# OFA-Sys/ONE-PEACE

Hardware: AMD Instinct MI355X
Metric: pretrain samples/s (tri-modal global batch) ONE-PEACE-4B (higher is better)
Workload: dtype bf16

## Files before the change

### include/onepeace_hip.h

```cpp
#ifndef ONEPEACE_HIP_H
#define ONEPEACE_HIP_H

#include <stdint.h>

#ifdef __cplusplus
extern "C" {
#endif

int op_abi_version(void);
const char* op_last_error(void);

int op_prof_enable(int on);
int op_prof_reserve(int events);
int op_prof_collect(double* ms, int64_t* count, double* work, int n_families);

int op_layernorm_fwd(const void* x, const void* w, const void* b, void* y, float* mean, float* rstd, int64_t rows,
                     int64_t cols, float eps, int act_gelu, int dtype, const int* x_rows, void* stream);
int64_t op_layernorm_bwd_workspace_bytes(int64_t rows, int64_t cols);
int op_layernorm_bwd(const void* dy, const void* x, const void* w, const void* b, const float* mean, const float* rstd,
                     const void* add, void* dx, void* dw, void* db, void* workspace, int64_t rows, int64_t cols,
                     int act_gelu, int accumulate, int dtype, const int* x_rows, void* stream);

int op_gemm_nt(const void* A, int64_t lda, const void* B0, const void* B1, const void* B2, int64_t ldb, int64_t n_seg,
               const void* bias0, const void* bias1, const void* bias2, void* C, int64_t ldc, void* h0, void* h1,
               const void* resid, int64_t ldr, const void* gamma, const float* rowscale, int64_t rows_per_sample,
               const float* alpha, int64_t M, int64_t N, int64_t K, int epilogue, void* workspace, int64_t workspace_bytes,
               int64_t tune, const int* resid_rows, int64_t resid_rows_total, void* stream);
int op_gemm_tn(const void* A, int64_t lda, const void* B, int64_t ldb, void* C, int64_t ldc, int64_t M, int64_t N, int64_t K,
               int accumulate, void* workspace, int64_t workspace_bytes, int64_t tune, void* stream);
int op_gemm_nt_grouped(int64_t nprob, const void* const* A, const int64_t* M, int64_t lda, const void* const* B, int64_t ldb,
                       const void* const* bias, void* const* C, int64_t ldc, void* const* h0, void* const* h1,
                       const void* const* resid, int64_t ldr, const void* const* gamma, const float* const* rowscale,
                       const int64_t* rows_per_sample, int64_t N, int64_t K, int epilogue, int64_t tune, const int* const* resid_rows,
                       int64_t resid_rows_total, void* stream);
int op_gemm_nt_batched(const void* A, int64_t lda, int64_t stride_a, const void* W, int64_t ldb, int64_t stride_b, const void* bias,
                       int64_t stride_bias, void* C, int64_t ldc, int64_t stride_c, int64_t M, int64_t N, int64_t K, int64_t batch,
                       void* stream);
int op_audio_conv1_ln_gelu_fwd(const void* wav, int64_t stride, const void* w0, const void* b0, const void* lnw, const void* lnb, void* y,
                               float* mean, float* rstd, int64_t rows, int64_t C, float eps, void* stream);
int64_t op_audio_conv1_ln_gelu_bwd_workspace_bytes(int64_t C);
int op_audio_conv1_ln_gelu_bwd(const void* dy, const void* wav, int64_t stride, const void* w0, const void* b0, const void* lnw, const void* lnb,
                               const float* mean, const float* rstd, void* dw0, void* db0, void* dlnw, void* dlnb, void* workspace,
                               int64_t rows, int64_t C, int accumulate, void* stream);
int64_t op_gemm_tn_grouped_counter_bytes(void);
int64_t op_gemm_tn_grouped_plan(int64_t nprob, const int64_t* M, const int64_t* N, const int64_t* K, int64_t workgroups, int64_t tune,
                                int32_t* out, int64_t cap);
int op_gemm_tn_grouped(int64_t nprob, const void* const* A, const int64_t* lda, const void* const* B, const int64_t* ldb, void* const* C,
                       const int64_t* ldc, const int64_t* M, const int64_t* N, const int64_t* K, const int32_t* accumulate,
                       const void* const* W, const int64_t* ldw, float* const* rowdot, const void* const* rscale, void* counters,
                       int64_t tune, void* stream);
int op_gemm_plan(int64_t M, int64_t N, int64_t K, int epilogue, int has_bias, int64_t workspace_bytes, int64_t tune, int* plan);

int op_quant_fp8_rows(const void* x, int64_t ldx, void* q, int64_t ldq, float* scale, int64_t rows, int64_t cols, void* stream);
int op_layernorm_fwd_q8(const void* x, const void* w, const void* b, void* y, float* mean, float* rstd, void* q8, float* q8_scale,
                        int64_t rows, int64_t cols, float eps, void* stream);
int op_ln_geglu_fwd_q8(const void* h0, const void* h1, int64_t ldh, const void* w, const void* b, void* y, float* mean, float* rstd, void* q8,
                       float* q8_scale, int64_t rows, int64_t cols, float eps, void* stream);
int op_gemm_nt_fp8(const void* A8, int64_t lda, const float* sa, const void* B0, const void* B1, int64_t ldb, const float* sb0,
                   const float* sb1, const void* bias, void* C, int64_t ldc, void* h0, void* h1, const void* resid, int64_t ldr,
                   const void* gamma, const float* rowscale, int64_t rows_per_sample, int64_t M, int64_t N, int64_t K, int epilogue,
                   int64_t tune, void* stream);

int op_attn_fwd(const void* q, const void* k, const void* v, int64_t ld, const void* bias, int64_t bias_batch_stride,
                const void* bias_frag, const void* key_pad, void* out, int64_t ldo, float* lse, int64_t lse_ld, int64_t B,
                int64_t S, int64_t Spad, int64_t heads, int64_t head_dim, float scale, int64_t tune, void* stream);
int64_t op_attn_bias_frag_elems(int64_t n_img, int64_t S);
int op_attn_bias_pack(const void* src, void* dst, int64_t n_img, int64_t S, int64_t Spad, void* stream);
int op_attn_bwd_delta(const void* dout, const void* out, int64_t ldo, float* delta, int64_t B, int64_t S, int64_t Spad,
                      int64_t heads, void* stream);
int64_t op_attn_bwd_dbias_slabs(int64_t B, int64_t S, int64_t heads, int64_t tune);
int op_attn_bwd(const void* q, const void* k, const void* v, int64_t ld, const void* dout, const void* out, int64_t ldo,
                const void* bias, const void* biasT, const void* bias_frag, int64_t bias_batch_stride, const void* key_pad,
                const float* lse, float* delta, void* dq,
                void* dk, void* dv, int64_t ldg, float* dbias, int64_t B, int64_t S, int64_t Spad, int64_t heads,
                int64_t head_dim, float scale, int64_t tune, void* stream);

int op_relpos_bias_build(const void* table, const int* bucket, int64_t bucket_ld, void* out, int64_t heads, int64_t S,
                         int64_t Spad, int transposed, void* stream);
int op_relpos_bias_bwd(const float* dbias, int64_t S, int64_t Spad, const int* pos, const int* seg, int64_t nseg, const int* bucket_seg,
                       int64_t num_rel, float* partial_ws, float* dtable, int64_t heads, void* stream);
int op_relpos_bias_build_ids(const void* table, const int* bucket, int64_t bucket_ld, const int* ids, void* out, int64_t B,
                             int64_t heads, int64_t K, int64_t Kpad, int transposed, void* stream);
int op_relpos_bias_fold_ids(const float* dbias, const int* ids, float* dense_ws, int64_t Sfull, int64_t B, int64_t heads, int64_t K,
                            int64_t Kpad, void* stream);

int op_transpose(const void* in, void* out, int64_t rows, int64_t cols, int64_t ld_in, int64_t ld_out, void* stream);
int op_transpose_scaled(const void* in, void* out, int64_t rows, int64_t cols, int64_t ld_in, int64_t ld_out, const void* scale,
                        void* stream);
int op_transpose_batched(const void* table, int64_t n, int64_t total_tiles, void* stream);
int64_t op_transpose_desc_bytes(void);
int64_t op_colsum_workspace_bytes(int64_t N);
int op_colsum_segments(const void* x, void* out0, void* out1, void* out2, void* workspace, int64_t M, int64_t n_seg,
                       int64_t seg_cols, int accumulate, void* stream);
int64_t op_resid_bwd_workspace_bytes(int64_t N);
int op_resid_bwd(const void* dout, const void* y, const void* gamma, const float* rowscale, int64_t rows_per_sample,
                 void* dbranch, void* dgamma, void* dbias, float* g0, void* workspace, int64_t M, int64_t N, int accumulate,
                 const int* dout_rows, void* stream);
int op_gamma_grad_finish(const float* rowdot, int64_t slots, const void* b0, const float* g00, const void* b1, const float* g01,
                         const void* b2, const float* g02, void* dgamma, int64_t N, int accumulate, void* stream);
int op_ln_geglu_bwd(const void* dy, const void* h0, const void* h1, const void* w, const float* mean, const float* rstd,
                    void* dh0, void* dh1, int64_t ldd, int64_t ldh, void* dw, void* db, void* workspace, int64_t rows,
                    int64_t cols, int accumulate, void* stream);
int op_ln_geglu_fwd(const void* h0, const void* h1, int64_t ldh, const void* w, const void* b, void* y, float* mean, float* rstd,
                    int64_t rows, int64_t cols, float eps, void* stream);
int op_colsum(const void* x, const void* y, const float* rowscale, int64_t rows_per_sample, const void* mul, void* out,
              void* workspace, int64_t M, int64_t N, int accumulate, int out_dtype, void* stream);
int op_geglu_bwd(const void* dg, const void* h0, const void* h1, void* dh0, void* dh1, int64_t numel, void* stream);
int op_scale_rows(const void* dout, const void* gamma, const float* rowscale, int64_t rows_per_sample, void* dbranch,
                  int64_t M, int64_t N, void* stream);

int op_l2norm_fwd(const void* x, void* y, float* inv_norm, int64_t rows, int64_t cols, float eps, int out_dtype, void* stream);
int op_l2norm_bwd(const void* dy, const void* y, const float* inv_norm, void* dx, int64_t rows, int64_t cols, int y_dtype,
                  void* stream);
int op_infonce_rows(float* sim, int64_t rows, int64_t n, int64_t ld, int64_t target0, float label_smoothing, float gscale,
                    float* row_loss, float* row_hit, float* row_dot, int write_grad, void* stream);

int op_adamw_step(void* p, const void* g, float* m, float* v, int64_t numel, float lr, float beta1, float beta2, float eps,
                  float weight_decay, int64_t step, float grad_scale, const float* grad_sqnorm, float clip_norm,
                  void* stream);
int op_adamw_step_groups(void* p, const void* g, float* m, float* v, int64_t numel, const int64_t* group_end8,
                         const float* group_lr_scale, const float* group_weight_decay, int64_t n_groups, float lr, float beta1,
                         float beta2, float eps, int64_t step, float grad_scale, const float* grad_sqnorm, float clip_norm,
                         void* stream);
int op_sqnorm(const void* x, int64_t numel, float* workspace, float* out, void* stream);

int op_rows_gather(const void* src, void* dst, const int* list, int64_t nseg, const int64_t* src_row0, const int64_t* dst_row0,
                   const int64_t* S, const int64_t* n_kept, const int64_t* dst_rows, const int64_t* n_samples, const int64_t* list_off,
                   int64_t dst_total, int64_t cols, void* stream);
int op_rows_merge(const void* base, const void* upd, void* out, const int* list, int64_t nseg, const int64_t* src_row0,
                  const int64_t* dst_row0, const int64_t* S, const int64_t* n_kept, const int64_t* dst_rows, const int64_t* n_samples,
                  const int64_t* list_off, int64_t total, int64_t cols, void* stream);
int op_rows_map(int* map, const int* list, int64_t nseg, const int64_t* src_row0, const int64_t* dst_row0, const int64_t* S,
                const int64_t* n_kept, const int64_t* dst_rows, const int64_t* n_samples, const int64_t* list_off, int64_t dst_total,
                void* stream);

int64_t op_sim_topk_splits(int64_t M, int64_t N, int64_t splits);
int64_t op_sim_topk_workspace_bytes(int64_t M, int64_t N, int64_t k, int64_t splits);
int op_sim_topk(const void* Q, int64_t ldq, const void* G, int64_t ldg, int64_t M, int64_t N, int64_t D, int64_t k, float* vals, int* idx,
                void* workspace, int64_t workspace_bytes, int64_t splits, void* stream);

int op_image_resize_normalize(const void* src, int64_t src_bytes, const int64_t* desc, const int64_t* desc_host, int64_t B,
                              const int* coef, int64_t coef_count, int64_t S, const float* mean, const float* stdev, void* out,
                              int out_dtype, void* workspace, int64_t workspace_bytes, void* stream);

int op_audio_normalize_pad(const void* src, int64_t src_bytes, const int64_t* desc, const int64_t* desc_host, int64_t B, int64_t max_len,
                           int64_t min_len, void* out, int64_t T, int out_dtype, void* workspace, int64_t workspace_bytes, void* stream);

#ifdef __cplusplus
}
#endif
#endif
```

### one-peace_amd/csrc/elementwise.hip

```cpp
#include "common.h"
#include <string.h>

namespace {

constexpr int CS_MAX_PARTS = 256;

__device__ __forceinline__ void transpose_tile(int bx, int by, const bf16_t* __restrict__ in, bf16_t* __restrict__ out,
                                                        int rows, int cols, int64_t ld_in, int64_t ld_out,
                                                        const bf16_t* __restrict__ scale = nullptr) {
  __shared__ bf16_t tile[64][64 + 2];
  const int r0 = by * 64, c0 = bx * 64;
  const int tx = threadIdx.x & 15, ty = threadIdx.x >> 4;
#pragma unroll
  for (int k = 0; k < 4; ++k) {
    const int r = r0 + ty + k * 16, c = c0 + tx * 4;
    if (r < rows) {
      const float sc = scale ? (float)scale[r] : 1.f;
      if (c + 3 < cols && (ld_in & 3) == 0) {
        bf16x4 v = *reinterpret_cast<const bf16x4*>(in + (int64_t)r * ld_in + c);
#pragma unroll
        for (int j = 0; j < 4; ++j) tile[ty + k * 16][tx * 4 + j] = scale ? (bf16_t)(sc * (float)v[j]) : v[j];
      } else {
        for (int j = 0; j < 4; ++j)
          if (c + j < cols) tile[ty + k * 16][tx * 4 + j] = scale ? (bf16_t)(sc * (float)in[(int64_t)r * ld_in + c + j]) : in[(int64_t)r * ld_in + c + j];
      }
    }
  }
  __syncthreads();
#pragma unroll
  for (int k = 0; k < 4; ++k) {
    const int c = c0 + ty + k * 16, r = r0 + tx * 4;
    if (c < cols) {
      if (r + 3 < rows && (ld_out & 3) == 0) {
        bf16x4 v;
#pragma unroll
        for (int j = 0; j < 4; ++j) v[j] = tile[tx * 4 + j][ty + k * 16];
        *reinterpret_cast<bf16x4*>(out + (int64_t)c * ld_out + r) = v;
      } else {
        for (int j = 0; j < 4; ++j)
          if (r + j < rows) out[(int64_t)c * ld_out + r + j] = tile[tx * 4 + j][ty + k * 16];
      }
    }
  }
}


__global__ __launch_bounds__(256) void transpose_kernel(const bf16_t* __restrict__ in, bf16_t* __restrict__ out, int rows, int cols,
                                                        int64_t ld_in, int64_t ld_out, const bf16_t* __restrict__ scale) {
  transpose_tile(blockIdx.x, blockIdx.y, in, out, rows, cols, ld_in, ld_out, scale);
}

struct TransposeDesc { const bf16_t* in; bf16_t* out; int rows, cols; int64_t ld_in, ld_out; int tile0, tiles_x; const bf16_t* scale; };
__global__ __launch_bounds__(256) void transpose_batched_kernel(const TransposeDesc* __restrict__ table, int n) {
  const int b = blockIdx.x;
  int lo = 0, hi = n - 1;
  while (lo < hi) {
    const int mid = (lo + hi + 1) >> 1;
    if (table[mid].tile0 <= b) lo = mid; else hi = mid - 1;
  }
  const TransposeDesc d = table[lo];
  const int local = b - d.tile0;
  transpose_tile(local % d.tiles_x, local / d.tiles_x, d.in, d.out, d.rows, d.cols, d.ld_in, d.ld_out, d.scale);
}

__global__ __launch_bounds__(256) void colsum_partial_kernel(const bf16_t* __restrict__ x, const bf16_t* __restrict__ y,
                                                             const float* __restrict__ rowscale, int rps,
                                                             float* __restrict__ part, int64_t M, int N, int64_t ld) {
  __shared__ float red[4][512];
  const int lane = threadIdx.x & 63, wid = threadIdx.x >> 6;
  const int c = blockIdx.x * 512 + lane * 8;
  float a[8] = {0, 0, 0, 0, 0, 0, 0, 0};
  if (c < N) {
    const int64_t m0 = (int64_t)blockIdx.y * 4 + wid, step = (int64_t)gridDim.y * 4;
    if (!y && !rowscale) {
      int64_t m = m0;
      for (; m + 3 * step < M; m += 4 * step) {
        typename Vec8<bf16_t>::raw_t r0 = Vec8<bf16_t>::ldraw(x + m * ld + c), r1 = Vec8<bf16_t>::ldraw(x + (m + step) * ld + c),
                                     r2 = Vec8<bf16_t>::ldraw(x + (m + 2 * step) * ld + c), r3 = Vec8<bf16_t>::ldraw(x + (m + 3 * step) * ld + c);
        float v0[8], v1[8], v2[8], v3[8];
        Vec8<bf16_t>::cvt(r0, v0);
        Vec8<bf16_t>::cvt(r1, v1);
        Vec8<bf16_t>::cvt(r2, v2);
        Vec8<bf16_t>::cvt(r3, v3);
#pragma unroll
        for (int j = 0; j < 8; ++j) a[j] = (((a[j] + v0[j]) + v1[j]) + v2[j]) + v3[j];
      }
      for (; m < M; m += step) {
        float xv[8];
        Vec8<bf16_t>::load(x + m * ld + c, xv);
#pragma unroll
        for (int j = 0; j < 8; ++j) a[j] += xv[j];
      }
    } else {
      for (int64_t m = m0; m < M; m += step) {
        float xv[8];
        Vec8<bf16_t>::load(x + m * ld + c, xv);
        float s = rowscale ? rowscale[m / rps] : 1.f;
        if (y) {
          float yv[8];
          Vec8<bf16_t>::load(y + m * ld + c, yv);
#pragma unroll
          for (int j = 0; j < 8; ++j) a[j] += s * xv[j] * yv[j];
        } else {
#pragma unroll
          for (int j = 0; j < 8; ++j) a[j] += s * xv[j];
        }
      }
    }
  }
#pragma unroll
  for (int j = 0; j < 8; ++j) red[wid][lane * 8 + j] = a[j];
  __syncthreads();
  for (int i = threadIdx.x; i < 512; i += 256) {
    const int cc = blockIdx.x * 512 + i;
    if (cc < N) part[(int64_t)blockIdx.y * N + cc] = red[0][i] + red[1][i] + red[2][i] + red[3][i];
  }
}

__global__ __launch_bounds__(256) void gamma_grad_finish_kernel(const float* __restrict__ rowdot, int slots,
                                                                const bf16_t* __restrict__ b0, const float* __restrict__ g00,
                                                                const bf16_t* __restrict__ b1, const float* __restrict__ g01,
                                                                const bf16_t* __restrict__ b2, const float* __restrict__ g02,
                                                                bf16_t* __restrict__ dgamma, int N, int accumulate) {
  __shared__ float part[4][64];
  const int lane = threadIdx.x & 63, w = threadIdx.x >> 6;
  const int n = blockIdx.x * 64 + lane;
  float a0 = 0.f, a1 = 0.f, a2 = 0.f, a3 = 0.f;
  if (n < N) {
    int s = w;
    for (; s + 12 < slots; s += 16) {
      a0 += rowdot[(int64_t)s * N + n];
      a1 += rowdot[(int64_t)(s + 4) * N + n];
      a2 += rowdot[(int64_t)(s + 8) * N + n];
      a3 += rowdot[(int64_t)(s + 12) * N + n];
    }
    for (; s < slots; s += 4) a0 += rowdot[(int64_t)s * N + n];
  }
  part[w][lane] = (a0 + a1) + (a2 + a3);
  __syncthreads();
  if (w != 0 || n >= N) return;
  float t = (part[0][lane] + part[1][lane]) + (part[2][lane] + part[3][lane]);
  if (g00) t += (b0 ? (float)b0[n] : 0.f) * g00[n];
  if (g01) t += (b1 ? (float)b1[n] : 0.f) * g01[n];
  if (g02) t += (b2 ? (float)b2[n] : 0.f) * g02[n];
  dgamma[n] = (bf16_t)(t + (accumulate ? (float)dgamma[n] : 0.f));
}

__global__ __launch_bounds__(256) void resid_bwd_kernel(const bf16_t* __restrict__ dout, const bf16_t* __restrict__ y,
                                                        const bf16_t* __restrict__ gamma, const float* __restrict__ rowscale,
                                                        int rps, bf16_t* __restrict__ dbranch, float* __restrict__ part,
                                                        int64_t M, int N, const int* __restrict__ rows) {
  __shared__ float red[4][512];
  const int lane = threadIdx.x & 63, wid = threadIdx.x >> 6;
  const int c = blockIdx.x * 512 + lane * 8;
  float ag[8] = {0, 0, 0, 0, 0, 0, 0, 0}, ab[8] = {0, 0, 0, 0, 0, 0, 0, 0};
  float gv[8] = {1, 1, 1, 1, 1, 1, 1, 1};
  if (c < N) {
    if (gamma) Vec8<bf16_t>::load(gamma + c, gv);
    const int64_t step = (int64_t)gridDim.y * 4;
    const int64_t mfirst = (int64_t)blockIdx.y * 4 + wid;
    int64_t e0 = (rows && mfirst < M) ? rows[mfirst] : mfirst, e1 = (rows && mfirst + step < M) ? rows[mfirst + step] : mfirst + step;
    for (int64_t m = mfirst; m < M; m += 2 * step) {
      const int64_t m2 = m + step;
      const bool two = m2 < M;
      const int64_t s0 = e0, s1 = two ? e1 : -1;
      const int64_t mn = m + 2 * step;
      if (rows) {
        if (mn < M) e0 = rows[mn];
        if (mn + step < M) e1 = rows[mn + step];
      } else {
        e0 = mn;
        e1 = mn + step;
      }
      const bf16x8 zero8 = {(bf16_t)0.f, (bf16_t)0.f, (bf16_t)0.f, (bf16_t)0.f, (bf16_t)0.f, (bf16_t)0.f, (bf16_t)0.f, (bf16_t)0.f};
      bf16x8 d0 = s0 >= 0 ? Vec8<bf16_t>::ldraw(dout + s0 * N + c) : zero8, d1, y0, y1;
      if (y) y0 = Vec8<bf16_t>::ldraw(y + m * N + c);
      if (two) {
        d1 = s1 >= 0 ? Vec8<bf16_t>::ldraw(dout + s1 * N + c) : zero8;
        if (y) y1 = Vec8<bf16_t>::ldraw(y + m2 * N + c);
      }
#pragma unroll
      for (int h = 0; h < 2; ++h) {
        if (h == 1 && !two) break;
        const int64_t mm = h == 0 ? m : m2;
        float d[8], o[8];
        Vec8<bf16_t>::cvt(h == 0 ? d0 : d1, d);
        const float sc = rowscale ? rowscale[mm / rps] : 1.f;
        if (y) {
          float yv[8];
          Vec8<bf16_t>::cvt(h == 0 ? y0 : y1, yv);
#pragma unroll
          for (int j = 0; j < 8; ++j) ag[j] += sc * d[j] * yv[j];
        }
#pragma unroll
        for (int j = 0; j < 8; ++j) {
          const float t = sc * d[j];
          ab[j] += t;
          o[j] = t * gv[j];
        }
        Vec8<bf16_t>::store(dbranch + mm * N + c, o);
      }
    }
  }
  if (part == nullptr) return;
#pragma unroll
  for (int pass = 0; pass < 2; ++pass) {
    if (pass == 0 && y == nullptr) continue;
    __syncthreads();
#pragma unroll
    for (int j = 0; j < 8; ++j) red[wid][lane * 8 + j] = pass == 0 ? ag[j] : ab[j];
    __syncthreads();
    float* dst = part + ((int64_t)pass * gridDim.y + blockIdx.y) * N;
    for (int i = threadIdx.x; i < 512; i += 256) {
      const int cc = blockIdx.x * 512 + i;
      if (cc < N) dst[cc] = red[0][i] + red[1][i] + red[2][i] + red[3][i];
    }
  }
}

__global__ __launch_bounds__(256) void geglu_bwd_kernel(const bf16_t* __restrict__ dg, const bf16_t* __restrict__ h0,
                                                        const bf16_t* __restrict__ h1, bf16_t* __restrict__ dh0,
                                                        bf16_t* __restrict__ dh1, int64_t n8) {
  for (int64_t i = (int64_t)blockIdx.x * 256 + threadIdx.x; i < n8; i += (int64_t)gridDim.x * 256) {
    float g[8], a[8], b[8], o0[8], o1[8];
    Vec8<bf16_t>::load(dg + i * 8, g);
    Vec8<bf16_t>::load(h0 + i * 8, a);
    Vec8<bf16_t>::load(h1 + i * 8, b);
#pragma unroll
    for (int j = 0; j < 8; ++j) {
      float cdf, pdf;
      gelu_parts(a[j], cdf, pdf);
      o0[j] = g[j] * b[j] * (cdf + a[j] * pdf);
      o1[j] = g[j] * a[j] * cdf;
    }
    Vec8<bf16_t>::store(dh0 + i * 8, o0);
    Vec8<bf16_t>::store(dh1 + i * 8, o1);
  }
}

__global__ __launch_bounds__(256) void scale_rows_kernel(const bf16_t* __restrict__ dout, const bf16_t* __restrict__ gamma,
                                                         const float* __restrict__ rowscale, int rps,
                                                         bf16_t* __restrict__ dbranch, int64_t M, int N) {
  const int n8 = N / 8;
  const int64_t total = M * n8;
  for (int64_t i = (int64_t)blockIdx.x * 256 + threadIdx.x; i < total; i += (int64_t)gridDim.x * 256) {
    const int64_t m = i / n8;
    const int c = (int)(i - m * n8) * 8;
    float d[8], gv[8];
    Vec8<bf16_t>::load(dout + m * N + c, d);
    const float s = rowscale ? rowscale[m / rps] : 1.f;
    if (gamma) {
      Vec8<bf16_t>::load(gamma + c, gv);
#pragma unroll
      for (int j = 0; j < 8; ++j) d[j] *= s * gv[j];
    } else {
#pragma unroll
      for (int j = 0; j < 8; ++j) d[j] *= s;
    }
    Vec8<bf16_t>::store(dbranch + m * N + c, d);
  }
}

template <typename TO>
__global__ __launch_bounds__(256) void l2norm_fwd_kernel(const bf16_t* __restrict__ x, TO* __restrict__ y,
                                                         float* __restrict__ inv_norm, int rows, int cols, float eps) {
  const int lane = threadIdx.x & 63;
  const int row = blockIdx.x * 4 + (threadIdx.x >> 6);
  if (row >= rows) return;
  float ss = 0.f;
  for (int c = lane * 8; c < cols; c += 512) {
    float v[8];
    Vec8<bf16_t>::load(x + (int64_t)row * cols + c, v);
#pragma unroll
    for (int j = 0; j < 8; ++j) ss += v[j] * v[j];
  }
  ss = wave_sum(ss);
  const float nrm = sqrtf(ss);
  const float inv = 1.f / fmaxf(nrm, eps);
  for (int c = lane * 8; c < cols; c += 512) {
    float v[8];
    Vec8<bf16_t>::load(x + (int64_t)row * cols + c, v);
#pragma unroll
    for (int j = 0; j < 8; ++j) v[j] *= inv;
    Vec8<TO>::store(y + (int64_t)row * cols + c, v);
  }
  if (lane == 0 && inv_norm) inv_norm[row] = nrm < eps ? -inv : inv;
}

template <typename TY>
__global__ __launch_bounds__(256) void l2norm_bwd_kernel(const TY* __restrict__ dy, const TY* __restrict__ y,
                                                         const float* __restrict__ inv_norm, bf16_t* __restrict__ dx,
                                                         int rows, int cols) {
  const int lane = threadIdx.x & 63;
  const int row = blockIdx.x * 4 + (threadIdx.x >> 6);
  if (row >= rows) return;
  float dot = 0.f;
  for (int c = lane * 8; c < cols; c += 512) {
    float a[8], b[8];
// ... 284 lines not shown
#pragma unroll
    for (int i = 0; i < 4; ++i) {
      if (i < d.nseg && rc >= d.seg[i].dst_row0 && rc < d.seg[i].dst_row0 + d.seg[i].dst_rows) {
        const int local = (int)(rc - d.seg[i].dst_row0);
        const int j = local / d.seg[i].S;
        if (j < d.seg[i].n_kept) from = d.seg[i].src_row0 + (int64_t)list[d.seg[i].list_off + j] * d.seg[i].S + (local - j * d.seg[i].S);
      }
    }
    bf16x8* o = reinterpret_cast<bf16x8*>(dst + rc * cols);
    if (from >= 0) {
      const bf16x8* in = reinterpret_cast<const bf16x8*>(src + from * cols);
      for (int c = lane; c < n8; c += 64) o[c] = in[c];
    } else {
      bf16x8 z;
#pragma unroll
      for (int k = 0; k < 8; ++k) z[k] = (bf16_t)0.f;
      for (int c = lane; c < n8; c += 64) o[c] = z;
    }
  }
}

__global__ __launch_bounds__(256) void rows_merge_kernel(const bf16_t* __restrict__ base, const bf16_t* __restrict__ upd,
                                                         bf16_t* __restrict__ out, const int* __restrict__ list, const RowsSegs d,
                                                         int64_t total, int cols) {
  const int lane = threadIdx.x & 63;
  const int n8 = cols / 8;
  for (int64_t r = (int64_t)blockIdx.x * 4 + (threadIdx.x >> 6); r < total; r += (int64_t)gridDim.x * 4) {
    int64_t from = -1;
#pragma unroll
    for (int i = 0; i < 4; ++i) {
      if (i < d.nseg && r >= d.seg[i].src_row0 && r < d.seg[i].src_row0 + (int64_t)d.seg[i].n_samples * d.seg[i].S) {
        const int local = (int)(r - d.seg[i].src_row0);
        const int smp = local / d.seg[i].S;
        const int j = list[d.seg[i].list_off + smp];
        if (j >= 0) from = d.seg[i].dst_row0 + (int64_t)j * d.seg[i].S + (local - smp * d.seg[i].S);
      }
    }
    if (from < 0 && out == base) continue;
    if (from >= 0 && upd == nullptr) continue;
    const bf16x8* in = reinterpret_cast<const bf16x8*>(from >= 0 ? upd + from * cols : base + r * cols);
    bf16x8* o = reinterpret_cast<bf16x8*>(out + r * cols);
    for (int c = lane; c < n8; c += 64) o[c] = in[c];
  }
}

__global__ __launch_bounds__(256) void rows_map_kernel(int* __restrict__ map, const int* __restrict__ list, const RowsSegs d, int64_t dst_total) {
  const int64_t rc = (int64_t)blockIdx.x * 256 + threadIdx.x;
  if (rc >= dst_total) return;
  int64_t from = -1;
#pragma unroll
  for (int i = 0; i < 4; ++i) {
    if (i < d.nseg && rc >= d.seg[i].dst_row0 && rc < d.seg[i].dst_row0 + d.seg[i].dst_rows) {
      const int local = (int)(rc - d.seg[i].dst_row0);
      const int j = local / d.seg[i].S;
      if (j < d.seg[i].n_kept) from = d.seg[i].src_row0 + (int64_t)list[d.seg[i].list_off + j] * d.seg[i].S + (local - j * d.seg[i].S);
    }
  }
  map[rc] = (int)from;
}

}

extern "C" {

int op_transpose_scaled(const void* in, void* out, int64_t rows, int64_t cols, int64_t ld_in, int64_t ld_out, const void* scale,
                        void* stream) {
  OP_CHECK_ARG(in && out && rows >= 0 && cols >= 0, "transpose: bad args");
  if (rows == 0 || cols == 0) return OP_OK;
  dim3 grid(ceil_div(cols, 64), ceil_div(rows, 64));
  hipLaunchKernelGGL(transpose_kernel, grid, dim3(256), 0, (hipStream_t)stream, (const bf16_t*)in, (bf16_t*)out, (int)rows,
                     (int)cols, ld_in, ld_out, (const bf16_t*)scale);
  OP_LAUNCH_CHECK();
  return OP_OK;
}
int op_transpose(const void* in, void* out, int64_t rows, int64_t cols, int64_t ld_in, int64_t ld_out, void* stream) {
  return op_transpose_scaled(in, out, rows, cols, ld_in, ld_out, nullptr, stream);
}

int op_transpose_batched(const void* table, int64_t n, int64_t total_tiles, void* stream) {
  OP_CHECK_ARG(table && n > 0 && total_tiles > 0, "transpose_batched: bad args");
  hipLaunchKernelGGL(transpose_batched_kernel, dim3((unsigned)total_tiles), dim3(256), 0, (hipStream_t)stream,
                     (const TransposeDesc*)table, (int)n);
  OP_LAUNCH_CHECK();
  return OP_OK;
}
int64_t op_transpose_desc_bytes(void) { return (int64_t)sizeof(TransposeDesc); }

int64_t op_colsum_workspace_bytes(int64_t N) { return (int64_t)CS_MAX_PARTS * N * (int64_t)sizeof(float); }

int op_colsum(const void* x, const void* y, const float* rowscale, int64_t rows_per_sample, const void* mul, void* out,
              void* workspace, int64_t M, int64_t N, int accumulate, int out_dtype, void* stream) {
  OP_CHECK_ARG(x && out && workspace, "colsum: null pointer");
  OP_CHECK_ARG(N > 0 && N % 8 == 0, "colsum: N must be a multiple of 8");
  hipStream_t s = (hipStream_t)stream;
  int parts = (int)((M + 63) / 64);
  if (parts > CS_MAX_PARTS) parts = CS_MAX_PARTS;
  if (parts < 1) parts = 1;
  dim3 grid(ceil_div(N, 512), parts);
  hipLaunchKernelGGL(colsum_partial_kernel, grid, dim3(256), 0, s, (const bf16_t*)x, (const bf16_t*)y, rowscale,
                     (int)(rows_per_sample > 0 ? rows_per_sample : 1), (float*)workspace, M, (int)N, N);
  OP_LAUNCH_CHECK();
  if (out_dtype == OP_DT_BF16)
    hipLaunchKernelGGL((partials_reduce_kernel<bf16_t>), dim3(ceil_div(N, 32)), dim3(256), 0, s, (const float*)workspace, parts,
                       N, (int)N, (const bf16_t*)mul, (bf16_t*)out, accumulate);
  else
    hipLaunchKernelGGL((partials_reduce_kernel<float>), dim3(ceil_div(N, 32)), dim3(256), 0, s, (const float*)workspace, parts,
                       N, (int)N, (const bf16_t*)mul, (float*)out, accumulate);
  OP_LAUNCH_CHECK();
  return OP_OK;
}

int64_t op_resid_bwd_workspace_bytes(int64_t N) { return 2 * (int64_t)CS_MAX_PARTS * N * (int64_t)sizeof(float); }

int op_resid_bwd(const void* dout, const void* y, const void* gamma, const float* rowscale, int64_t rows_per_sample,
                 void* dbranch, void* dgamma, void* dbias, float* g0, void* workspace, int64_t M, int64_t N, int accumulate,
                 const int* dout_rows, void* stream) {
  OP_CHECK_ARG(dout && dbranch, "resid_bwd: null pointer");
  OP_CHECK_ARG(N > 0 && N % 8 == 0, "resid_bwd: N must be a multiple of 8");
  OP_CHECK_ARG(!dgamma || y, "resid_bwd: dgamma needs y");
  OP_CHECK_ARG(!(dgamma && g0), "resid_bwd: g0 (dbranch without gamma) and dgamma (from y) are alternatives");
  OP_CHECK_ARG(!(dgamma || dbias || g0) || workspace, "resid_bwd: dgamma/dbias/g0 requested without workspace");
  if (M == 0) {
    if (g0) (void)hipMemsetAsync(g0, 0, (size_t)N * sizeof(float), (hipStream_t)stream);
    return OP_OK;
  }
  hipStream_t s = (hipStream_t)stream;
  int parts = (int)((M + 63) / 64);
  if (parts > CS_MAX_PARTS) parts = CS_MAX_PARTS;
  if (parts < 1) parts = 1;
  float* ws = (dgamma || dbias || g0) ? (float*)workspace : nullptr;
  hipLaunchKernelGGL(resid_bwd_kernel, dim3(ceil_div(N, 512), parts), dim3(256), 0, s, (const bf16_t*)dout,
                     (const bf16_t*)(dgamma ? y : nullptr), (const bf16_t*)(g0 ? nullptr : gamma), rowscale,
                     (int)(rows_per_sample > 0 ? rows_per_sample : 1), (bf16_t*)dbranch, ws, M, (int)N, dout_rows);
  OP_LAUNCH_CHECK();
  if (ws) {
    hipLaunchKernelGGL((partials_reduce3_kernel<bf16_t>), dim3(ceil_div(N, 32), g0 ? 3 : 2), dim3(256), 0, s, ws,
                       ws + (int64_t)parts * N, ws + (int64_t)parts * N, (const bf16_t*)nullptr, (const bf16_t*)gamma,
                       (const bf16_t*)nullptr, (bf16_t*)dgamma, (bf16_t*)dbias, (bf16_t*)nullptr, parts, N, (int)N,
                       accumulate, g0);
    OP_LAUNCH_CHECK();
  }
  return OP_OK;
}

int op_gamma_grad_finish(const float* rowdot, int64_t slots, const void* b0, const float* g00, const void* b1, const float* g01,
                         const void* b2, const float* g02, void* dgamma, int64_t N, int accumulate, void* stream) {
  OP_CHECK_ARG(rowdot && dgamma && N > 0 && slots > 0, "gamma_grad_finish: null pointer");
  hipLaunchKernelGGL(gamma_grad_finish_kernel, dim3(ceil_div(N, 64)), dim3(256), 0, (hipStream_t)stream, rowdot, (int)slots,
                     (const bf16_t*)b0, g00, (const bf16_t*)b1, g01, (const bf16_t*)b2, g02, (bf16_t*)dgamma, (int)N, accumulate);
  OP_LAUNCH_CHECK();
  return OP_OK;
}

int op_colsum_segments(const void* x, void* out0, void* out1, void* out2, void* workspace, int64_t M, int64_t n_seg,
                       int64_t seg_cols, int accumulate, void* stream) {
  OP_CHECK_ARG(x && workspace, "colsum_segments: null pointer");
  OP_CHECK_ARG(n_seg >= 1 && n_seg <= 3 && seg_cols > 0 && seg_cols % 8 == 0, "colsum_segments: bad segments");
  hipStream_t s = (hipStream_t)stream;
  const int64_t N = n_seg * seg_cols;
  int parts = (int)((M + 63) / 64);
  if (parts > CS_MAX_PARTS) parts = CS_MAX_PARTS;
  if (parts < 1) parts = 1;
  void* outs[3] = {out0, out1, out2};
  const float* ws = (const float*)workspace;
  for (int i = 0; i < (int)n_seg; ++i) {
    if (outs[i] == nullptr) continue;
    hipLaunchKernelGGL(colsum_partial_kernel, dim3(ceil_div(seg_cols, 512), parts), dim3(256), 0, s,
                       (const bf16_t*)x + i * seg_cols, (const bf16_t*)nullptr, (const float*)nullptr, 1,
                       (float*)workspace + (int64_t)i * parts * seg_cols, M, (int)seg_cols, N);
    OP_LAUNCH_CHECK();
  }
  const int64_t st = (int64_t)parts * seg_cols;
  hipLaunchKernelGGL((partials_reduce3_kernel<bf16_t>), dim3(ceil_div(seg_cols, 32), (int)n_seg), dim3(256), 0, s, ws, ws + st,
                     ws + 2 * st, (const bf16_t*)nullptr, (const bf16_t*)nullptr, (const bf16_t*)nullptr, (bf16_t*)out0,
                     (bf16_t*)out1, (bf16_t*)out2, parts, seg_cols, (int)seg_cols, accumulate);
  OP_LAUNCH_CHECK();
  return OP_OK;
}

int op_geglu_bwd(const void* dg, const void* h0, const void* h1, void* dh0, void* dh1, int64_t numel, void* stream) {
  OP_CHECK_ARG(dg && h0 && h1 && dh0 && dh1, "geglu_bwd: null pointer");
  OP_CHECK_ARG(numel % 8 == 0, "geglu_bwd: numel must be a multiple of 8");
  if (numel == 0) return OP_OK;
  hipLaunchKernelGGL(geglu_bwd_kernel, dim3(ew_grid(numel / 8)), dim3(256), 0, (hipStream_t)stream, (const bf16_t*)dg,
                     (const bf16_t*)h0, (const bf16_t*)h1, (bf16_t*)dh0, (bf16_t*)dh1, numel / 8);
  OP_LAUNCH_CHECK();
  return OP_OK;
}

int op_scale_rows(const void* dout, const void* gamma, const float* rowscale, int64_t rows_per_sample, void* dbranch,
                  int64_t M, int64_t N, void* stream) {
  OP_CHECK_ARG(dout && dbranch, "scale_rows: null pointer");
  OP_CHECK_ARG(N % 8 == 0, "scale_rows: N must be a multiple of 8");
  if (M == 0) return OP_OK;
  hipLaunchKernelGGL(scale_rows_kernel, dim3(ew_grid(M * (N / 8))), dim3(256), 0, (hipStream_t)stream, (const bf16_t*)dout,
                     (const bf16_t*)gamma, rowscale, (int)(rows_per_sample > 0 ? rows_per_sample : 1), (bf16_t*)dbranch, M,
                     (int)N);
  OP_LAUNCH_CHECK();
  return OP_OK;
}

int op_l2norm_fwd(const void* x, void* y, float* inv_norm, int64_t rows, int64_t cols, float eps, int out_dtype, void* stream) {
  OP_CHECK_ARG(x && y && cols % 8 == 0, "l2norm_fwd: bad args");
  if (rows == 0) return OP_OK;
  if (out_dtype == OP_DT_BF16)
    hipLaunchKernelGGL((l2norm_fwd_kernel<bf16_t>), dim3(ceil_div(rows, 4)), dim3(256), 0, (hipStream_t)stream,
                       (const bf16_t*)x, (bf16_t*)y, inv_norm, (int)rows, (int)cols, eps);
  else
    hipLaunchKernelGGL((l2norm_fwd_kernel<float>), dim3(ceil_div(rows, 4)), dim3(256), 0, (hipStream_t)stream,
                       (const bf16_t*)x, (float*)y, inv_norm, (int)rows, (int)cols, eps);
  OP_LAUNCH_CHECK();
  return OP_OK;
}

int op_l2norm_bwd(const void* dy, const void* y, const float* inv_norm, void* dx, int64_t rows, int64_t cols, int y_dtype,
                  void* stream) {
  OP_CHECK_ARG(dy && y && inv_norm && dx && cols % 8 == 0, "l2norm_bwd: bad args");
  if (rows == 0) return OP_OK;
  if (y_dtype == OP_DT_BF16)
    hipLaunchKernelGGL((l2norm_bwd_kernel<bf16_t>), dim3(ceil_div(rows, 4)), dim3(256), 0, (hipStream_t)stream,
                       (const bf16_t*)dy, (const bf16_t*)y, inv_norm, (bf16_t*)dx, (int)rows, (int)cols);
  else
    hipLaunchKernelGGL((l2norm_bwd_kernel<float>), dim3(ceil_div(rows, 4)), dim3(256), 0, (hipStream_t)stream,
                       (const float*)dy, (const float*)y, inv_norm, (bf16_t*)dx, (int)rows, (int)cols);
  OP_LAUNCH_CHECK();
  return OP_OK;
}

int op_infonce_rows(float* sim, int64_t rows, int64_t n, int64_t ld, int64_t target0, float label_smoothing, float gscale,
                    float* row_loss, float* row_hit, float* row_dot, int write_grad, void* stream) {
  OP_CHECK_ARG(sim && row_loss && row_hit && row_dot, "infonce_rows: null pointer");
  OP_CHECK_ARG(n >= 2 && target0 >= 0 && target0 + rows <= n, "infonce_rows: targets out of range");
  if (rows == 0) return OP_OK;
  hipLaunchKernelGGL(infonce_rows_kernel, dim3((int)rows), dim3(256), 0, (hipStream_t)stream, sim, (int)n, ld, (int)target0,
                     label_smoothing, gscale, row_loss, row_hit, row_dot, write_grad);
  OP_LAUNCH_CHECK();
  return OP_OK;
}

int op_sqnorm(const void* x, int64_t numel, float* workspace, float* out, void* stream) {
  OP_CHECK_ARG(x && workspace && out && numel % 8 == 0, "sqnorm: bad args");
  hipStream_t s = (hipStream_t)stream;
  hipLaunchKernelGGL(sqnorm_partial_kernel, dim3(1024), dim3(256), 0, s, (const bf16_t*)x, numel / 8, workspace);
  OP_LAUNCH_CHECK();
  hipLaunchKernelGGL(sqnorm_final_kernel, dim3(1), dim3(256), 0, s, (const float*)workspace, 1024, out);
  OP_LAUNCH_CHECK();
  return OP_OK;
}

int op_adamw_step(void* p, const void* g, float* m, float* v, int64_t numel, float lr, float beta1, float beta2, float eps,
                  float weight_decay, int64_t step, float grad_scale, const float* grad_sqnorm, float clip_norm,
                  void* stream) {
  OP_CHECK_ARG(p && g && m && v, "adamw: null pointer");
  OP_CHECK_ARG(numel % 8 == 0 && step >= 1, "adamw: numel must be a multiple of 8 and step >= 1");
  if (numel == 0) return OP_OK;
  const double bc1 = 1.0 - pow((double)beta1, (double)step);
  const double bc2 = 1.0 - pow((double)beta2, (double)step);
  const float step_size = (float)((double)lr * sqrt(bc2) / bc1);
  const float decay_mul = 1.f - weight_decay * lr;
  hipLaunchKernelGGL(adamw_kernel, dim3(ew_grid(numel / 8)), dim3(256), 0, (hipStream_t)stream, (bf16_t*)p, (const bf16_t*)g,
                     m, v, numel / 8, beta1, beta2, eps, step_size, decay_mul, grad_scale, grad_sqnorm, clip_norm);
  OP_LAUNCH_CHECK();
  return OP_OK;
}

int op_adamw_step_groups(void* p, const void* g, float* m, float* v, int64_t numel, const int64_t* group_end8,
                         const float* group_lr_scale, const float* group_weight_decay, int64_t n_groups, float lr, float beta1,
                         float beta2, float eps, int64_t step, float grad_scale, const float* grad_sqnorm, float clip_norm,
                         void* stream) {
  OP_CHECK_ARG(p && g && m && v && group_end8 && group_lr_scale && group_weight_decay, "adamw_groups: null pointer");
  OP_CHECK_ARG(numel % 8 == 0 && step >= 1 && n_groups >= 1 && n_groups <= ADAM_MAX_GROUPS,
               "adamw_groups: numel %% 8 == 0, step >= 1, 1 <= n_groups <= %d required", ADAM_MAX_GROUPS);
  if (numel == 0) return OP_OK;
  const double bc1 = 1.0 - pow((double)beta1, (double)step);
  const double bc2 = 1.0 - pow((double)beta2, (double)step);
  hipLaunchKernelGGL(adamw_groups_kernel, dim3(ew_grid(numel / 8)), dim3(256), 0, (hipStream_t)stream, (bf16_t*)p,
                     (const bf16_t*)g, m, v, numel / 8, group_end8, group_lr_scale, group_weight_decay, (int)n_groups, lr, beta1,
                     beta2, eps, (float)(sqrt(bc2) / bc1), grad_scale, grad_sqnorm, clip_norm);
  OP_LAUNCH_CHECK();
  return OP_OK;
}

int op_relpos_bias_build(const void* table, const int* bucket, int64_t bucket_ld, void* out, int64_t heads, int64_t S,
                         int64_t Spad, int transposed, void* stream) {
  OP_CHECK_ARG(table && bucket && out && Spad >= S && Spad % 8 == 0, "relpos_bias_build: bad args");
  hipLaunchKernelGGL(relpos_build_kernel, dim3(ew_grid(S * Spad)), dim3(256), 0, (hipStream_t)stream, (const bf16_t*)table,
                     bucket, bucket_ld, (bf16_t*)out, (int)heads, (int)S, (int)Spad, transposed);
  OP_LAUNCH_CHECK();
  return OP_OK;
}

int op_relpos_bias_build_ids(const void* table, const int* bucket, int64_t bucket_ld, const int* ids, void* out, int64_t B,
                             int64_t heads, int64_t K, int64_t Kpad, int transposed, void* stream) {
  OP_CHECK_ARG(table && bucket && ids && out && B > 0 && K > 0 && Kpad >= K && Kpad % 8 == 0, "relpos_bias_build_ids: bad args");
  hipLaunchKernelGGL(relpos_build_ids_kernel, dim3(ew_grid(B * K * Kpad)), dim3(256), 0, (hipStream_t)stream, (const bf16_t*)table,
                     bucket, bucket_ld, ids, (bf16_t*)out, (int)B, (int)heads, (int)K, (int)Kpad, transposed);
  OP_LAUNCH_CHECK();
  return OP_OK;
}

int op_relpos_bias_fold_ids(const float* dbias, const int* ids, float* dense_ws, int64_t Sfull, int64_t B, int64_t heads, int64_t K,
                            int64_t Kpad, void* stream) {
  OP_CHECK_ARG(dbias && ids && dense_ws && B > 0 && K > 0 && Sfull > 0, "relpos_bias_fold_ids: bad args");
  hipLaunchKernelGGL(relpos_fold_ids_kernel, dim3(ew_grid(B * heads * K * K)), dim3(256), 0, (hipStream_t)stream, dbias, ids, dense_ws,
                     (int)B, (int)heads, (int)K, (int)Kpad, (int)Sfull);
  OP_LAUNCH_CHECK();
// ... 75 lines not shown
```

### one-peace_amd/csrc/layernorm.hip

```cpp
#include "common.h"

namespace {

constexpr int LN_MAX_BLOCKS = 4096;
constexpr int g_ln_blocks_fwd = 512, g_ln_blocks_bwd = 512;
#ifndef OP_LN_GEGLU_BLOCKS_FWD
#define OP_LN_GEGLU_BLOCKS_FWD 2048
#endif
#ifndef OP_LN_GEGLU_BLOCKS_BWD
#define OP_LN_GEGLU_BLOCKS_BWD 512
#endif

template <int NW>
__device__ __forceinline__ float group_sum(float v, float* red) {
  v = wave_sum(v);
  if (NW == 1) return v;
  const int wid = threadIdx.x >> 6;
  __syncthreads();
  if ((threadIdx.x & 63) == 0) red[wid] = v;
  __syncthreads();
  float t = 0.f;
#pragma unroll
  for (int i = 0; i < NW; ++i) t += red[i];
  return t;
// ... 97 lines not shown
    }
    const float rstd = rsqrtf(group_sum<NW>(ss, red) * inv + eps);
    T* yr = y + row * (int64_t)cols;
    int amax = 0;
#pragma unroll
    for (int i = 0; i < CH; ++i) {
      const int c = (tig + G * i) * 8;
      if (c < cols) {
        float o[8];
#pragma unroll
        for (int j = 0; j < 8; ++j) {
          float t = (v[i][j] - mean) * rstd * wv[i][j] + bv[i][j];
          o[j] = GELU ? gelu_erf(t) : t;
        }
        store_sel<T, NT>(yr + c, o);
        if constexpr (Q8) {
#pragma unroll
          for (int j = 0; j < 8; ++j) { v[i][j] = (float)(T)o[j]; amax = fp8_amax_acc(amax, v[i][j]); }
        }
      }
    }
    if constexpr (Q8) {
      float qinv;
      const float sc = fp8_row_scale(group_amax<NW>(amax, red), qinv);
      uint8_t* qr = q8 + row * (int64_t)cols;
#pragma unroll
      for (int i = 0; i < CH; ++i) {
        const int c = (tig + G * i) * 8;
        if (c < cols) *reinterpret_cast<u32x2*>(qr + c) = fp8_pack8(v[i], qinv);
      }
      if (tig == 0) q8_scale[row] = sc;
    }
    if (tig == 0) {
      if (mean_out) mean_out[row] = mean;
      if (rstd_out) rstd_out[row] = rstd;
    }
#pragma unroll
    for (int i = 0; i < CH; ++i) cur[i] = nxt[i];
  }
}

template <int CH, int NW, bool Q8 = false>
__global__ __launch_bounds__(NW == 1 ? 256 : 64 * NW) void ln_geglu_fwd_kernel(const bf16_t* __restrict__ h0, const bf16_t* __restrict__ h1,
                                                           int64_t ldh, const bf16_t* __restrict__ w, const bf16_t* __restrict__ b,
                                                           bf16_t* __restrict__ y, float* __restrict__ mean_out,
                                                           float* __restrict__ rstd_out, int64_t rows, int cols, float eps,
                                                           uint8_t* __restrict__ q8 = nullptr, float* __restrict__ q8_scale = nullptr) {
  __shared__ float red[4];
  constexpr int G = 64 * NW;
  const int tig = (NW == 1) ? (threadIdx.x & 63) : threadIdx.x;
  const int64_t row0 = (NW == 1) ? ((int64_t)blockIdx.x * 4 + (threadIdx.x >> 6)) : blockIdx.x;
  const int64_t rstep = (NW == 1) ? (int64_t)gridDim.x * 4 : gridDim.x;
  const float inv = 1.0f / (float)cols;
  float wv[CH][8], bv[CH][8];
#pragma unroll
  for (int i = 0; i < CH; ++i) {
    const int c = (tig + G * i) * 8;
#pragma unroll
    for (int j = 0; j < 8; ++j) { wv[i][j] = 1.f; bv[i][j] = 0.f; }
    if (c < cols) {
      if (w) Vec8<bf16_t>::load(w + c, wv[i]);
      if (b) Vec8<bf16_t>::load(b + c, bv[i]);
    }
  }
  bf16x8 c0[CH], c1[CH], n0[CH], n1[CH];
  if (row0 < rows) {
#pragma unroll
    for (int i = 0; i < CH; ++i) {
      const int c = (tig + G * i) * 8;
      if (c < cols) {
        c0[i] = Vec8<bf16_t>::ldraw_nt(h0 + row0 * ldh + c);
        c1[i] = Vec8<bf16_t>::ldraw_nt(h1 + row0 * ldh + c);
      }
    }
  }
  for (int64_t row = row0; row < rows; row += rstep) {
    const int64_t nrow = row + rstep;
    if (nrow < rows) {
#pragma unroll
      for (int i = 0; i < CH; ++i) {
        const int c = (tig + G * i) * 8;
        if (c < cols) {
          n0[i] = Vec8<bf16_t>::ldraw_nt(h0 + nrow * ldh + c);
          n1[i] = Vec8<bf16_t>::ldraw_nt(h1 + nrow * ldh + c);
        }
      }
    }
    float v[CH][8];
    float s = 0.f;
#pragma unroll
    for (int i = 0; i < CH; ++i) {
      const int c = (tig + G * i) * 8;
      if (c < cols) {
        float a[8], bb[8];
        Vec8<bf16_t>::cvt(c0[i], a);
        Vec8<bf16_t>::cvt(c1[i], bb);
#pragma unroll
        for (int j = 0; j < 8; ++j) {
          v[i][j] = (float)(bf16_t)(gelu_erf(a[j]) * bb[j]);
          s += v[i][j];
        }
      } else {
#pragma unroll
        for (int j = 0; j < 8; ++j) v[i][j] = 0.f;
      }
    }
    const float mean = group_sum<NW>(s, red) * inv;
    float ss = 0.f;
#pragma unroll
    for (int i = 0; i < CH; ++i) {
      const int c = (tig + G * i) * 8;
      if (c < cols) {
#pragma unroll
        for (int j = 0; j < 8; ++j) { const float d = v[i][j] - mean; ss += d * d; }
      }
    }
    const float rstd = rsqrtf(group_sum<NW>(ss, red) * inv + eps);
    bf16_t* yr = y + row * (int64_t)cols;
    int amax = 0;
#pragma unroll
    for (int i = 0; i < CH; ++i) {
      const int c = (tig + G * i) * 8;
      if (c < cols) {
        float o[8];
#pragma unroll
        for (int j = 0; j < 8; ++j) o[j] = (v[i][j] - mean) * rstd * wv[i][j] + bv[i][j];
        Vec8<bf16_t>::store_nt(yr + c, o);
        if constexpr (Q8) {
#pragma unroll
          for (int j = 0; j < 8; ++j) { v[i][j] = (float)(bf16_t)o[j]; amax = fp8_amax_acc(amax, v[i][j]); }
        }
      }
    }
    if constexpr (Q8) {
      float qinv;
      const float sc = fp8_row_scale(group_amax<NW>(amax, red), qinv);
      uint8_t* qr = q8 + row * (int64_t)cols;
#pragma unroll
      for (int i = 0; i < CH; ++i) {
        const int c = (tig + G * i) * 8;
        if (c < cols) *reinterpret_cast<u32x2*>(qr + c) = fp8_pack8(v[i], qinv);
      }
      if (tig == 0) q8_scale[row] = sc;
    }
    if (tig == 0) {
      if (mean_out) mean_out[row] = mean;
      if (rstd_out) rstd_out[row] = rstd;
    }
#pragma unroll
    for (int i = 0; i < CH; ++i) { c0[i] = n0[i]; c1[i] = n1[i]; }
  }
}

template <typename T, int CH, int NW, bool GELU, bool NT>
__global__ __launch_bounds__(256) void ln_bwd_kernel(const T* __restrict__ dy, const T* __restrict__ x,
                                                     const T* __restrict__ w, const T* __restrict__ b,
                                                     const float* __restrict__ mean_in,
                                                     const float* __restrict__ rstd_in, const T* __restrict__ add,
                                                     T* __restrict__ dx, float* __restrict__ ws, int64_t rows, int cols,
                                                     const int* __restrict__ xmap = nullptr) {
  extern __shared__ __attribute__((aligned(16))) float smem[];
  float* red = smem;
  constexpr int G = 64 * NW;
  const int tig = (NW == 1) ? (threadIdx.x & 63) : threadIdx.x;
  const int wid = threadIdx.x >> 6;
  const int64_t row0 = (NW == 1) ? ((int64_t)blockIdx.x * 4 + wid) : blockIdx.x;
  const int64_t rstep = (NW == 1) ? (int64_t)gridDim.x * 4 : gridDim.x;
  const float inv = 1.0f / (float)cols;

  float wv[CH][8], bv[CH][8], dwa[CH][8], dba[CH][8];
#pragma unroll
  for (int i = 0; i < CH; ++i) {
    const int c = (tig + G * i) * 8;
#pragma unroll
    for (int j = 0; j < 8; ++j) { wv[i][j] = 1.f; bv[i][j] = 0.f; dwa[i][j] = 0.f; dba[i][j] = 0.f; }
    if (c < cols) {
      if (w) Vec8<T>::load(w + c, wv[i]);
      if (GELU && b) Vec8<T>::load(b + c, bv[i]);
    }
  }
  typedef typename Vec8<T>::raw_t raw_t;
  raw_t curx[CH], curg[CH], nxtx[CH], nxtg[CH], addv[CH];
  int64_t src = row0 < rows ? (xmap ? (int64_t)xmap[row0] : row0) : -1;
  int64_t nsrc = row0 + rstep < rows ? (xmap ? (int64_t)xmap[row0 + rstep] : row0 + rstep) : -1, nnsrc = -1;
  if (row0 < rows) {
#pragma unroll
    for (int i = 0; i < CH; ++i) {
      const int c = (tig + G * i) * 8;
      if (c < cols) {
        if (src >= 0) curx[i] = ldraw_sel<T, NT>(x + src * (int64_t)cols + c);
        else curx[i] = raw_t{};
        curg[i] = ldraw_sel<T, NT>(dy + row0 * (int64_t)cols + c);
      }
    }
  }
  for (int64_t row = row0; row < rows; row += rstep) {
    const float mean = mean_in[row], rstd = rstd_in[row];
    const int64_t nrow = row + rstep, nnrow = nrow + rstep;
    if (nnrow < rows) nnsrc = xmap ? (int64_t)xmap[nnrow] : nnrow;
#pragma unroll
    for (int i = 0; i < CH; ++i) {
      const int c = (tig + G * i) * 8;
      if (c < cols) {
        if (add && src >= 0) addv[i] = ldraw_sel<T, NT>(add + src * (int64_t)cols + c);
        if (nrow < rows) {
          if (nsrc >= 0) nxtx[i] = ldraw_sel<T, NT>(x + nsrc * (int64_t)cols + c);
          else nxtx[i] = raw_t{};
          nxtg[i] = ldraw_sel<T, NT>(dy + nrow * (int64_t)cols + c);
        }
      }
    }
    float xh[CH][8], g[CH][8];
    float s1 = 0.f, s2 = 0.f;
#pragma unroll
    for (int i = 0; i < CH; ++i) {
      const int c = (tig + G * i) * 8;
      if (c < cols) {
        Vec8<T>::cvt(curx[i], xh[i]);
        Vec8<T>::cvt(curg[i], g[i]);
#pragma unroll
        for (int j = 0; j < 8; ++j) {
          xh[i][j] = (xh[i][j] - mean) * rstd;
          if (GELU) g[i][j] *= gelu_erf_grad(xh[i][j] * wv[i][j] + bv[i][j]);
          dwa[i][j] += g[i][j] * xh[i][j];
          dba[i][j] += g[i][j];
          const float gw = g[i][j] * wv[i][j];
          g[i][j] = gw;
          s1 += gw;
          s2 += gw * xh[i][j];
        }
      }
    }
    group_sum2<NW>(s1, s2, red);
    const float c1 = s1 * inv, c2 = s2 * inv;
    T* dr = dx + (src >= 0 ? src : 0) * (int64_t)cols;
#pragma unroll
    for (int i = 0; i < CH; ++i) {
      const int c = (tig + G * i) * 8;
      if (c < cols && src >= 0) {
        float o[8];
#pragma unroll
        for (int j = 0; j < 8; ++j) o[j] = rstd * (g[i][j] - c1 - xh[i][j] * c2);
        if (add) {
          float av[8];
          Vec8<T>::cvt(addv[i], av);
#pragma unroll
          for (int j = 0; j < 8; ++j) o[j] += av[j];
        }
        store_sel<T, NT>(dr + c, o);
      }
    }
#pragma unroll
    for (int i = 0; i < CH; ++i) { curx[i] = nxtx[i]; curg[i] = nxtg[i]; }
    src = nsrc;
    nsrc = nnsrc;
  }
  if (ws == nullptr) return;
  float* wsb = ws + (int64_t)blockIdx.x * 2 * cols;
  if (NW == 1) {
#pragma unroll
    for (int pass = 0; pass < 2; ++pass) {
      __syncthreads();
#pragma unroll
      for (int i = 0; i < CH; ++i) {
        const int c = (tig + G * i) * 8;
        if (c < cols) {
#pragma unroll
          for (int j = 0; j < 8; ++j) smem[wid * cols + c + j] = pass == 0 ? dwa[i][j] : dba[i][j];
        }
      }
      __syncthreads();
      for (int c = threadIdx.x; c < cols; c += 256)
        wsb[pass * cols + c] = smem[c] + smem[cols + c] + smem[2 * cols + c] + smem[3 * cols + c];
    }
  } else {
#pragma unroll
    for (int i = 0; i < CH; ++i) {
      const int c = (tig + G * i) * 8;
      if (c < cols) {
#pragma unroll
        for (int j = 0; j < 8; ++j) { wsb[c + j] = dwa[i][j]; wsb[cols + c + j] = dba[i][j]; }
      }
    }
  }
}

template <int CH, int NW>
__global__ __launch_bounds__(NW == 1 ? 256 : 64 * NW) void ln_geglu_bwd_kernel(const bf16_t* __restrict__ dy, const bf16_t* __restrict__ h0,
                                                           const bf16_t* __restrict__ h1, const bf16_t* __restrict__ w,
                                                           const float* __restrict__ mean_in,
                                                           const float* __restrict__ rstd_in, bf16_t* __restrict__ dh0,
                                                           bf16_t* __restrict__ dh1, int64_t ldd, int64_t ldh, float* __restrict__ ws,
                                                           int64_t rows, int cols) {
  extern __shared__ __attribute__((aligned(16))) float smem[];
  float* red = smem;
  constexpr int G = 64 * NW;
  const int tig = (NW == 1) ? (threadIdx.x & 63) : threadIdx.x;
  const int wid = threadIdx.x >> 6;
  const int64_t row0 = (NW == 1) ? ((int64_t)blockIdx.x * 4 + wid) : blockIdx.x;
  const int64_t rstep = (NW == 1) ? (int64_t)gridDim.x * 4 : gridDim.x;
  const float inv = 1.0f / (float)cols;
  float dwa[CH][8], dba[CH][8];
  bf16x8 wraw[CH];
#pragma unroll
  for (int i = 0; i < CH; ++i) {
    const int c = (tig + G * i) * 8;
#pragma unroll
    for (int j = 0; j < 8; ++j) { dwa[i][j] = 0.f; dba[i][j] = 0.f; }
#pragma unroll
    for (int j = 0; j < 8; ++j) wraw[i][j] = (bf16_t)1.0f;
    if (c < cols && w) wraw[i] = Vec8<bf16_t>::ldraw(w + c);
  }
  bf16x8 r0[CH], r1[CH], rg[CH], n0[CH], n1[CH], ng[CH];
  if (row0 < rows) {
#pragma unroll
    for (int i = 0; i < CH; ++i) {
      const int c = (tig + G * i) * 8;
      if (c < cols) {
        r0[i] = Vec8<bf16_t>::ldraw_nt(h0 + row0 * ldh + c);
        r1[i] = Vec8<bf16_t>::ldraw_nt(h1 + row0 * ldh + c);
        rg[i] = Vec8<bf16_t>::ldraw_nt(dy + row0 * (int64_t)cols + c);
      }
    }
  }
  for (int64_t row = row0; row < rows; row += rstep) {
    const float mean = mean_in[row], rstd = rstd_in[row];
    const int64_t base = row * (int64_t)cols;
    const int64_t nrow = row + rstep;
    if (nrow < rows) {
#pragma unroll
      for (int i = 0; i < CH; ++i) {
        const int c = (tig + G * i) * 8;
        if (c < cols) {
          n0[i] = Vec8<bf16_t>::ldraw_nt(h0 + nrow * ldh + c);
          n1[i] = Vec8<bf16_t>::ldraw_nt(h1 + nrow * ldh + c);
          ng[i] = Vec8<bf16_t>::ldraw_nt(dy + nrow * (int64_t)cols + c);
        }
      }
    }
    float gw[CH][8], cdfs[CH][8], gps[CH][8];
    float s1 = 0.f, s2 = 0.f;
#pragma unroll
    for (int i = 0; i < CH; ++i) {
      const int c = (tig + G * i) * 8;
      if (c < cols) {
        float a[8], b[8];
        Vec8<bf16_t>::cvt(r0[i], a);
        Vec8<bf16_t>::cvt(r1[i], b);
        Vec8<bf16_t>::cvt(rg[i], gw[i]);
        float wv[8];
        asm volatile("" : "+v"(wraw[i]));
        Vec8<bf16_t>::cvt(wraw[i], wv);
#pragma unroll
        for (int j = 0; j < 8; ++j) {
          float cdf, pdf;
          gelu_parts(a[j], cdf, pdf);
          cdfs[i][j] = cdf;
          gps[i][j] = cdf + a[j] * pdf;
          const float gval = (float)(bf16_t)(a[j] * cdf * b[j]);
          const float xh = (gval - mean) * rstd;
          const float d = gw[i][j];
          dwa[i][j] += d * xh;
          dba[i][j] += d;
          const float t = d * wv[j];
          gw[i][j] = t;
          s1 += t;
          s2 += t * xh;
        }
      }
    }
    group_sum2<NW>(s1, s2, red);
    const float c1 = s1 * inv, c2 = s2 * inv;
#pragma unroll
    for (int i = 0; i < CH; ++i) {
      const int c = (tig + G * i) * 8;
      if (c < cols) {
        float a[8], b[8], o0[8], o1[8];
        Vec8<bf16_t>::cvt(r0[i], a);
        Vec8<bf16_t>::cvt(r1[i], b);
#pragma unroll
        for (int j = 0; j < 8; ++j) {
          const float ge = a[j] * cdfs[i][j];
          const float xh = ((float)(bf16_t)(ge * b[j]) - mean) * rstd;
          const float dg = rstd * (gw[i][j] - c1 - xh * c2);
          o0[j] = dg * b[j] * gps[i][j];
          o1[j] = dg * ge;
        }
        Vec8<bf16_t>::store_nt(dh0 + row * ldd + c, o0);
        Vec8<bf16_t>::store_nt(dh1 + row * ldd + c, o1);
      }
    }
#pragma unroll
    for (int i = 0; i < CH; ++i) { r0[i] = n0[i]; r1[i] = n1[i]; rg[i] = ng[i]; }
  }
  if (ws == nullptr) return;
  float* wsb = ws + (int64_t)blockIdx.x * 2 * cols;
  if (NW == 1) {
#pragma unroll
    for (int pass = 0; pass < 2; ++pass) {
      __syncthreads();
#pragma unroll
      for (int i = 0; i < CH; ++i) {
        const int c = (tig + G * i) * 8;
        if (c < cols) {
#pragma unroll
          for (int j = 0; j < 8; ++j) smem[wid * cols + c + j] = pass == 0 ? dwa[i][j] : dba[i][j];
        }
      }
      __syncthreads();
      for (int c = threadIdx.x; c < cols; c += 256)
        wsb[pass * cols + c] = smem[c] + smem[cols + c] + smem[2 * cols + c] + smem[3 * cols + c];
    }
  } else {
#pragma unroll
    for (int i = 0; i < CH; ++i) {
      const int c = (tig + G * i) * 8;
      if (c < cols) {
#pragma unroll
        for (int j = 0; j < 8; ++j) { wsb[c + j] = dwa[i][j]; wsb[cols + c + j] = dba[i][j]; }
      }
    }
  }
}

inline int ln_grid(int64_t rows, int nw, int cap) {
  int64_t blocks = nw == 1 ? (rows + 3) / 4 : rows;
  if (blocks > cap) blocks = cap;
  if (blocks < 1) blocks = 1;
  return (int)blocks;
}

template <typename T, bool GELU>
int ln_fwd_dispatch(const void* x, const void* w, const void* b, void* y, float* mean, float* rstd, int64_t rows,
                    int cols, float eps, hipStream_t s, const int* xmap = nullptr) {
  const T* X = (const T*)x; const T* W = (const T*)w; const T* B = (const T*)b; T* Y = (T*)y;
  const bool nt = mean != nullptr && (int64_t)rows * cols * (int64_t)sizeof(T) >= ((int64_t)64 << 20);
#define LN_F(CH, NW)                                                                                                                      \
  do {                                                                                                                                    \
    if (nt) hipLaunchKernelGGL((ln_fwd_kernel<T, CH, NW, GELU, true>), dim3(ln_grid(rows, NW, g_ln_blocks_fwd)), dim3(256), 0, s, X, W, B, Y, mean, rstd, rows, cols, eps, (uint8_t*)nullptr, (float*)nullptr, xmap); \
    else hipLaunchKernelGGL((ln_fwd_kernel<T, CH, NW, GELU, false>), dim3(ln_grid(rows, NW, g_ln_blocks_fwd)), dim3(256), 0, s, X, W, B, Y, mean, rstd, rows, cols, eps, (uint8_t*)nullptr, (float*)nullptr, xmap); \
  } while (0)
  if (cols <= 512) LN_F(1, 1);
  else if (cols <= 1024) LN_F(2, 1);
  else if (cols <= 1536) LN_F(3, 1);
  else if (cols <= 2048) LN_F(4, 1);
  else if (cols <= 4096) LN_F(2, 4);
  else if (cols <= 6144) LN_F(3, 4);
  else if (cols <= 8192) LN_F(4, 4);
  else { op_set_error("layernorm: cols %d > 8192 unsupported", cols); return OP_ENOTSUP; }
#undef LN_F
  OP_LAUNCH_CHECK();
  return OP_OK;
}

template <typename T, bool GELU>
int ln_bwd_dispatch(const void* dy, const void* x, const void* w, const void* b, const float* mean, const float* rstd,
                    const void* add, void* dx, void* dw, void* db, float* ws, int64_t rows, int cols, int accumulate,
                    hipStream_t s, const int* xmap = nullptr) {
  const T* DY = (const T*)dy; const T* X = (const T*)x; const T* W = (const T*)w; const T* B = (const T*)b; T* DX = (T*)dx;
  const T* ADD = (const T*)add;
  int grid = 0;
  float* wsk = (dw || db) ? ws : nullptr;
  const bool nt = (int64_t)rows * cols * (int64_t)sizeof(T) >= ((int64_t)64 << 20);
#define LN_B(CH, NW)                                                                                        \
  do {                                                                                                      \
    grid = ln_grid(rows, NW, g_ln_blocks_bwd);                                                                               \
    size_t sh = (NW == 1) ? (size_t)4 * cols * sizeof(float) : 64;                                          \
    if (nt) hipLaunchKernelGGL((ln_bwd_kernel<T, CH, NW, GELU, true>), dim3(grid), dim3(256), sh, s, DY, X, W, B, mean,   \
                       rstd, ADD, DX, wsk, rows, cols, xmap);                                                    \
    else hipLaunchKernelGGL((ln_bwd_kernel<T, CH, NW, GELU, false>), dim3(grid), dim3(256), sh, s, DY, X, W, B, mean,   \
                       rstd, ADD, DX, wsk, rows, cols, xmap);                                                    \
  } while (0)
  if (cols <= 512) LN_B(1, 1);
  else if (cols <= 1024) LN_B(2, 1);
  else if (cols <= 1536) LN_B(3, 1);
  else if (cols <= 2048) LN_B(4, 1);
  else if (cols <= 4096) LN_B(2, 4);
  else if (cols <= 6144) LN_B(3, 4);
  else if (cols <= 8192) LN_B(4, 4);
  else { op_set_error("layernorm: cols %d > 8192 unsupported", cols); return OP_ENOTSUP; }
#undef LN_B
  OP_LAUNCH_CHECK();
  if (wsk) {
    hipLaunchKernelGGL((partials_reduce3_kernel<T>), dim3(ceil_div(cols, 32), 2), dim3(256), 0, s, ws, ws + cols,
                       (const float*)nullptr, (const bf16_t*)nullptr, (const bf16_t*)nullptr, (const bf16_t*)nullptr, (T*)dw,
                       (T*)db, (T*)nullptr, grid, (int64_t)2 * cols, cols, accumulate);
    OP_LAUNCH_CHECK();
  }
  return OP_OK;
}

}

extern "C" {


int64_t op_layernorm_bwd_workspace_bytes(int64_t rows, int64_t cols) {
  (void)rows;
  return (int64_t)LN_MAX_BLOCKS * 2 * cols * (int64_t)sizeof(float);
}

int op_layernorm_fwd(const void* x, const void* w, const void* b, void* y, float* mean, float* rstd, int64_t rows,
                     int64_t cols, float eps, int act_gelu, int dtype, const int* x_rows, void* stream) {
  OP_CHECK_ARG(x && y, "layernorm_fwd: null x/y");
  OP_CHECK_ARG(rows >= 0 && cols > 0 && cols % 8 == 0, "layernorm_fwd: cols=%lld must be a positive multiple of 8",
               (long long)cols);
  if (rows == 0) return OP_OK;
  hipStream_t s = (hipStream_t)stream;
  if (dtype == OP_DT_BF16)
    return act_gelu ? ln_fwd_dispatch<bf16_t, true>(x, w, b, y, mean, rstd, rows, (int)cols, eps, s, x_rows)
                    : ln_fwd_dispatch<bf16_t, false>(x, w, b, y, mean, rstd, rows, (int)cols, eps, s, x_rows);
  if (dtype == OP_DT_F32)
    return act_gelu ? ln_fwd_dispatch<float, true>(x, w, b, y, mean, rstd, rows, (int)cols, eps, s, x_rows)
                    : ln_fwd_dispatch<float, false>(x, w, b, y, mean, rstd, rows, (int)cols, eps, s, x_rows);
  op_set_error("layernorm_fwd: bad dtype %d", dtype);
  return OP_EINVAL;
}

int op_layernorm_fwd_q8(const void* x, const void* w, const void* b, void* y, float* mean, float* rstd, void* q8, float* q8_scale,
                        int64_t rows, int64_t cols, float eps, void* stream) {
  OP_CHECK_ARG(x && y && q8 && q8_scale, "layernorm_fwd_q8: null pointer");
  OP_CHECK_ARG(rows >= 0 && cols > 0 && cols % 8 == 0 && cols <= 8192, "layernorm_fwd_q8: cols=%lld unsupported", (long long)cols);
  if (rows == 0) return OP_OK;
  hipStream_t s = (hipStream_t)stream;
#define LN_Q(CH, NW)                                                                                                                         \
  hipLaunchKernelGGL((ln_fwd_kernel<bf16_t, CH, NW, false, false, true>), dim3(ln_grid(rows, NW, g_ln_blocks_fwd)), dim3(256), 0, s,        \
                     (const bf16_t*)x, (const bf16_t*)w, (const bf16_t*)b, (bf16_t*)y, mean, rstd, rows, (int)cols, eps, (uint8_t*)q8, q8_scale)
  if (cols <= 512) LN_Q(1, 1);
  else if (cols <= 1024) LN_Q(2, 1);
  else if (cols <= 1536) LN_Q(3, 1);
  else if (cols <= 2048) LN_Q(4, 1);
  else if (cols <= 4096) LN_Q(2, 4);
  else if (cols <= 6144) LN_Q(3, 4);
  else LN_Q(4, 4);
#undef LN_Q
  OP_LAUNCH_CHECK();
  return OP_OK;
}

int op_layernorm_bwd(const void* dy, const void* x, const void* w, const void* b, const float* mean, const float* rstd,
                     const void* add, void* dx, void* dw, void* db, void* workspace, int64_t rows, int64_t cols,
                     int act_gelu, int accumulate, int dtype, const int* x_rows, void* stream) {
  OP_CHECK_ARG(dy && x && dx && mean && rstd, "layernorm_bwd: null pointer");
  OP_CHECK_ARG(rows >= 0 && cols > 0 && cols % 8 == 0, "layernorm_bwd: cols=%lld must be a positive multiple of 8",
               (long long)cols);
  OP_CHECK_ARG(!(dw || db) || workspace, "layernorm_bwd: dw/db requested without workspace");
  if (rows == 0) return OP_OK;
  hipStream_t s = (hipStream_t)stream;
  if (dtype == OP_DT_BF16)
    return act_gelu ? ln_bwd_dispatch<bf16_t, true>(dy, x, w, b, mean, rstd, add, dx, dw, db, (float*)workspace, rows,
                                                    (int)cols, accumulate, s, x_rows)
                    : ln_bwd_dispatch<bf16_t, false>(dy, x, w, b, mean, rstd, add, dx, dw, db, (float*)workspace, rows,
                                                     (int)cols, accumulate, s, x_rows);
  if (dtype == OP_DT_F32)
    return act_gelu ? ln_bwd_dispatch<float, true>(dy, x, w, b, mean, rstd, add, dx, dw, db, (float*)workspace, rows,
                                                   (int)cols, accumulate, s, x_rows)
                    : ln_bwd_dispatch<float, false>(dy, x, w, b, mean, rstd, add, dx, dw, db, (float*)workspace, rows,
                                                    (int)cols, accumulate, s, x_rows);
  op_set_error("layernorm_bwd: bad dtype %d", dtype);
  return OP_EINVAL;
}

int op_ln_geglu_fwd(const void* h0, const void* h1, int64_t ldh, const void* w, const void* b, void* y, float* mean, float* rstd,
                    int64_t rows, int64_t cols, float eps, void* stream) {
  OP_CHECK_ARG(h0 && h1 && y, "ln_geglu_fwd: null pointer");
  if (ldh <= 0) ldh = cols;
  OP_CHECK_ARG(rows >= 0 && cols > 0 && cols % 8 == 0 && cols <= 8192 && ldh >= cols && ldh % 8 == 0, "ln_geglu_fwd: cols=%lld ldh=%lld unsupported",
               (long long)cols, (long long)ldh);
  if (rows == 0) return OP_OK;
  hipStream_t s = (hipStream_t)stream;
#define LNG_F(CH, NW)                                                                                                       \
  hipLaunchKernelGGL((ln_geglu_fwd_kernel<CH, NW>), dim3(ln_grid(rows, NW, OP_LN_GEGLU_BLOCKS_FWD)), dim3(NW == 1 ? 256 : 64 * NW), 0, s, \
                     (const bf16_t*)h0, (const bf16_t*)h1, ldh, (const bf16_t*)w, (const bf16_t*)b, (bf16_t*)y, mean, rstd, rows, \
                     (int)cols, eps)
  if (cols <= 512) LNG_F(1, 1);
  else if (cols <= 1024) LNG_F(2, 1);
  else if (cols <= 1536) LNG_F(3, 1);
  else if (cols <= 2048) LNG_F(4, 1);
  else if (cols <= 4096) LNG_F(2, 4);
  else if (cols <= 6144) LNG_F(3, 4);
  else LNG_F(4, 4);
#undef LNG_F
  OP_LAUNCH_CHECK();
  return OP_OK;
}

int op_ln_geglu_fwd_q8(const void* h0, const void* h1, int64_t ldh, const void* w, const void* b, void* y, float* mean, float* rstd, void* q8,
                       float* q8_scale, int64_t rows, int64_t cols, float eps, void* stream) {
  OP_CHECK_ARG(h0 && h1 && y && q8 && q8_scale, "ln_geglu_fwd_q8: null pointer");
  if (ldh <= 0) ldh = cols;
  OP_CHECK_ARG(rows >= 0 && cols > 0 && cols % 8 == 0 && cols <= 8192 && ldh >= cols && ldh % 8 == 0, "ln_geglu_fwd_q8: cols=%lld ldh=%lld unsupported",
               (long long)cols, (long long)ldh);
  if (rows == 0) return OP_OK;
  hipStream_t s = (hipStream_t)stream;
#define LNG_Q(CH, NW)                                                                                                       \
  hipLaunchKernelGGL((ln_geglu_fwd_kernel<CH, NW, true>), dim3(ln_grid(rows, NW, OP_LN_GEGLU_BLOCKS_FWD)), dim3(NW == 1 ? 256 : 64 * NW), 0, s, \
                     (const bf16_t*)h0, (const bf16_t*)h1, ldh, (const bf16_t*)w, (const bf16_t*)b, (bf16_t*)y, mean, rstd, rows, \
                     (int)cols, eps, (uint8_t*)q8, q8_scale)
  if (cols <= 512) LNG_Q(1, 1);
  else if (cols <= 1024) LNG_Q(2, 1);
  else if (cols <= 1536) LNG_Q(3, 1);
  else if (cols <= 2048) LNG_Q(4, 1);
  else if (cols <= 4096) LNG_Q(2, 4);
  else if (cols <= 6144) LNG_Q(3, 4);
  else LNG_Q(4, 4);
#undef LNG_Q
  OP_LAUNCH_CHECK();
  return OP_OK;
}

int op_ln_geglu_bwd(const void* dy, const void* h0, const void* h1, const void* w, const float* mean, const float* rstd,
                    void* dh0, void* dh1, int64_t ldd, int64_t ldh, void* dw, void* db, void* workspace, int64_t rows, int64_t cols,
                    int accumulate, void* stream) {
  OP_CHECK_ARG(dy && h0 && h1 && dh0 && dh1 && mean && rstd, "ln_geglu_bwd: null pointer");
  if (ldd <= 0) ldd = cols;
  if (ldh <= 0) ldh = cols;
  OP_CHECK_ARG(ldd >= cols && ldd % 8 == 0 && ldh >= cols && ldh % 8 == 0, "ln_geglu_bwd: row strides %lld / %lld", (long long)ldd, (long long)ldh);
  OP_CHECK_ARG(rows >= 0 && cols > 0 && cols % 8 == 0 && cols <= 8192, "ln_geglu_bwd: cols=%lld unsupported", (long long)cols);
  OP_CHECK_ARG(!(dw || db) || workspace, "ln_geglu_bwd: dw/db requested without workspace");
  if (rows == 0) return OP_OK;
  hipStream_t s = (hipStream_t)stream;
  float* wsk = (dw || db) ? (float*)workspace : nullptr;
  int grid = 0;
#define LNG_B(CH, NW)                                                                                              \
  do {                                                                                                             \
    grid = ln_grid(rows, NW, OP_LN_GEGLU_BLOCKS_BWD);                                                                     \
    size_t sh = (NW == 1) ? (size_t)4 * cols * sizeof(float) : 64;                                                 \
    hipLaunchKernelGGL((ln_geglu_bwd_kernel<CH, NW>), dim3(grid), dim3(NW == 1 ? 256 : 64 * NW), sh, s,           \
                       (const bf16_t*)dy, (const bf16_t*)h0, (const bf16_t*)h1, (const bf16_t*)w, mean, rstd,      \
                       (bf16_t*)dh0, (bf16_t*)dh1, ldd, ldh, wsk, rows, (int)cols);                                \
  } while (0)
  if (cols <= 512) LNG_B(1, 1);
  else if (cols <= 1024) LNG_B(2, 1);
  else if (cols <= 1536) LNG_B(3, 1);
  else if (cols <= 2048) LNG_B(4, 1);
  else if (cols <= 4096) LNG_B(2, 4);
  else if (cols <= 6144) LNG_B(3, 4);
  else LNG_B(4, 4);
#undef LNG_B
  OP_LAUNCH_CHECK();
  if (wsk) {
    hipLaunchKernelGGL((partials_reduce3_kernel<bf16_t>), dim3(ceil_div(cols, 32), 2), dim3(256), 0, s, wsk, wsk + cols,
                       (const float*)nullptr, (const bf16_t*)nullptr, (const bf16_t*)nullptr, (const bf16_t*)nullptr,
                       (bf16_t*)dw, (bf16_t*)db, (bf16_t*)nullptr, grid, (int64_t)2 * cols, (int)cols, accumulate);
    OP_LAUNCH_CHECK();
  }
  return OP_OK;
}

}
```

### one-peace_amd/hip.py

```python
import ctypes
import os
from ctypes import c_double, c_float, c_int, c_int64, c_void_p

import torch

_HERE = os.path.dirname(os.path.abspath(__file__))
LIB_PATH = os.environ.get("ONEPEACE_HIP_LIB") or os.path.join(_HERE, "lib", "libonepeace_hip.so")
_lib = None

DT_BF16, DT_F32 = 0, 1
EPI_BIAS, EPI_F32, EPI_GEGLU, EPI_RESID = 0, 1, 2, 3
PROF_GEMM, PROF_ATTN = 0, 1
ATTN_RESIDENT_MAX_S = 320

P = c_void_p
I64 = c_int64

SIGNATURES = {
    "op_abi_version": (c_int, []),
    "op_last_error": (ctypes.c_char_p, []),
    "op_prof_enable": (c_int, [c_int]),
    "op_prof_reserve": (c_int, [c_int]),
    "op_prof_collect": (c_int, [P, P, P, c_int]),
    "op_layernorm_fwd": (c_int, [P, P, P, P, P, P, I64, I64, c_float, c_int, c_int, P, P]),
    "op_layernorm_bwd_workspace_bytes": (I64, [I64, I64]),
    "op_attn_bwd_dbias_slabs": (I64, [I64, I64, I64, I64]),
    "op_layernorm_bwd": (c_int, [P, P, P, P, P, P, P, P, P, P, P, I64, I64, c_int, c_int, c_int, P, P]),
    "op_gemm_plan": (c_int, [c_int64, c_int64, c_int64, c_int, c_int, c_int64, I64, P]),
    "op_gemm_nt": (c_int, [P, I64, P, P, P, I64, I64, P, P, P, P, I64, P, P, P, I64, P, P, I64, P, I64, I64, I64,
                           c_int, P, I64, I64, P, I64, P]),
    "op_gemm_nt_grouped": (c_int, [I64, P, P, I64, P, I64, P, P, I64, P, P, P, I64, P, P, P, I64, I64, c_int, I64, P, I64, P]),
    "op_gemm_tn": (c_int, [P, I64, P, I64, P, I64, I64, I64, I64, c_int, P, I64, I64, P]),
    "op_gemm_tn_grouped_counter_bytes": (I64, []),
    "op_gemm_tn_grouped_plan": (I64, [I64, P, P, P, I64, I64, P, I64]),
    "op_gemm_tn_grouped": (c_int, [I64, P, P, P, P, P, P, P, P, P, P, P, P, P, P, P, I64, P]),
    "op_gemm_nt_batched": (c_int, [P, I64, I64, P, I64, I64, P, I64, P, I64, I64, I64, I64, I64, I64, P]),
    "op_audio_conv1_ln_gelu_fwd": (c_int, [P, I64, P, P, P, P, P, P, P, I64, I64, c_float, P]),
    "op_audio_conv1_ln_gelu_bwd_workspace_bytes": (I64, [I64]),
    "op_audio_conv1_ln_gelu_bwd": (c_int, [P, P, I64, P, P, P, P, P, P, P, P, P, P, P, I64, I64, c_int, P]),
    "op_transpose": (c_int, [P, P, I64, I64, I64, I64, P]),
    "op_transpose_scaled": (c_int, [P, P, I64, I64, I64, I64, P, P]),
    "op_transpose_batched": (c_int, [P, I64, I64, P]),
    "op_transpose_desc_bytes": (I64, []),
    "op_colsum_workspace_bytes": (I64, [I64]),
    "op_colsum_segments": (c_int, [P, P, P, P, P, I64, I64, I64, c_int, P]),
    "op_resid_bwd_workspace_bytes": (I64, [I64]),
    "op_resid_bwd": (c_int, [P, P, P, P, I64, P, P, P, P, P, I64, I64, c_int, P, P]),
    "op_gamma_grad_finish": (c_int, [P, I64, P, P, P, P, P, P, P, I64, c_int, P]),
    "op_ln_geglu_bwd": (c_int, [P, P, P, P, P, P, P, P, I64, I64, P, P, P, I64, I64, c_int, P]),
    "op_ln_geglu_fwd": (c_int, [P, P, I64, P, P, P, P, P, I64, I64, c_float, P]),
    "op_colsum": (c_int, [P, P, P, I64, P, P, P, I64, I64, c_int, c_int, P]),
    "op_geglu_bwd": (c_int, [P, P, P, P, P, I64, P]),
    "op_scale_rows": (c_int, [P, P, P, I64, P, I64, I64, P]),
    "op_l2norm_fwd": (c_int, [P, P, P, I64, I64, c_float, c_int, P]),
    "op_l2norm_bwd": (c_int, [P, P, P, P, I64, I64, c_int, P]),
    "op_infonce_rows": (c_int, [P, I64, I64, I64, I64, c_float, c_float, P, P, P, c_int, P]),
    "op_adamw_step": (c_int, [P, P, P, P, I64, c_float, c_float, c_float, c_float, c_float, I64, c_float, P, c_float, P]),
    "op_adamw_step_groups": (c_int, [P, P, P, P, I64, P, P, P, I64, c_float, c_float, c_float, c_float, I64, c_float, P, c_float, P]),
    "op_sqnorm": (c_int, [P, I64, P, P, P]),
    "op_relpos_bias_build": (c_int, [P, P, I64, P, I64, I64, I64, c_int, P]),
    "op_relpos_bias_bwd": (c_int, [P, I64, I64, P, P, I64, P, I64, P, P, I64, P]),
    "op_relpos_bias_build_ids": (c_int, [P, P, I64, P, P, I64, I64, I64, I64, c_int, P]),
    "op_relpos_bias_fold_ids": (c_int, [P, P, P, I64, I64, I64, I64, I64, P]),
    "op_attn_fwd": (c_int, [P, P, P, I64, P, I64, P, P, P, I64, P, I64, I64, I64, I64, I64, I64, c_float, I64, P]),
    "op_attn_bias_frag_elems": (I64, [I64, I64]),
    "op_attn_bias_pack": (c_int, [P, P, I64, I64, I64, P]),
    "op_attn_bwd_delta": (c_int, [P, P, I64, P, I64, I64, I64, I64, P]),
    "op_attn_bwd": (c_int, [P, P, P, I64, P, P, I64, P, P, P, I64, P, P, P, P, P, P, I64, P, I64, I64, I64, I64, I64, c_float, I64, P]),
    "op_quant_fp8_rows": (c_int, [P, I64, P, I64, P, I64, I64, P]),
    "op_layernorm_fwd_q8": (c_int, [P, P, P, P, P, P, P, P, I64, I64, c_float, P]),
    "op_ln_geglu_fwd_q8": (c_int, [P, P, I64, P, P, P, P, P, P, P, I64, I64, c_float, P]),
    "op_gemm_nt_fp8": (c_int, [P, I64, P, P, P, I64, P, P, P, P, I64, P, P, P, I64, P, P, I64, I64, I64, I64, c_int, I64, P]),
    "op_rows_gather": (c_int, [P, P, P, I64, P, P, P, P, P, P, P, I64, I64, P]),
    "op_rows_merge": (c_int, [P, P, P, P, I64, P, P, P, P, P, P, P, I64, I64, P]),
    "op_rows_map": (c_int, [P, P, I64, P, P, P, P, P, P, P, I64, P]),
    "op_sim_topk_splits": (I64, [I64, I64, I64]),
    "op_sim_topk_workspace_bytes": (I64, [I64, I64, I64, I64]),
    "op_sim_topk": (c_int, [P, I64, P, I64, I64, I64, I64, I64, P, P, P, I64, I64, P]),
    "op_image_resize_normalize": (c_int, [P, I64, P, P, I64, P, I64, I64, P, P, P, c_int, P, I64, P]),
    "op_audio_normalize_pad": (c_int, [P, I64, P, P, I64, I64, I64, P, I64, c_int, P, I64, P]),
}


PROBE_SIGNATURES = {
    "op_last_error": (ctypes.c_char_p, []),
    "op_probe_mfma16": (c_int, [P, P, P, c_int, P]),
    "op_probe_mfma32": (c_int, [P, P, P, c_int, P]),
    "op_probe_tr16": (c_int, [P, P, P, c_int, P]),
    "op_probe_glds": (c_int, [P, P, c_int, P, P]),
    "op_probe_mfma_f8": (c_int, [P, P, P, P, P, c_int, P]),
    "op_probe_mfma_rate": (c_int, [P, P, P, c_int, c_int, P]),
    "op_probe_lds_atomic": (c_int, [P, P, c_int, c_int, c_int, P]),
    "op_probe_occupy": (c_int, [P, ctypes.c_longlong, c_int, ctypes.c_longlong, P, P]),
}


class Tuning:

    def __init__(self):
        self.reset()

    def reset(self):
        self.tile_mode = 0
        self.fullline = 2
        self.tail_rows = 1
        self.gm = 0
        self.force_splits = 0
        self.glds = 1
        self.sched = int(os.environ.get("ONEPEACE_TUNE_SCHED", "0"))
        self.fp8_small = 0
        self.merge_dbias = 1
        self.resident = 1
        self.attn_waves = 0
        self.attn_pers = 1
        self.dbias_chunks_r2 = 0
        self.dkdv_keys = 0
        self.dbias_chunks = 0
        self.attn_pers_dkdv = 1
        self.attn_lone_keys = 1
        self.attn_pers_bwd = 1

    def gemm(self):
        fl = {2: 0, 0: 1, 1: 2, 3: 3}.get(self.fullline, 0)
        tr = 0 if self.tail_rows == 1 else self.tail_rows + 1
        return (self.tile_mode | fl << 2 | tr << 4 | (self.gm & 31) << 7 | (self.force_splits & 15) << 15
                | (0 if self.glds else 1) << 19 | (self.sched & 7) << 20)

    def attn_fwd(self):
        return (0 if self.resident & 1 else 1) | ((self.resident >> 1) & 3) << 1 | (self.attn_waves & 15) << 3 | (0 if self.attn_pers else 128)

    def attn_bwd(self):
        return ((0 if self.merge_dbias else 1) | (2 if self.dbias_chunks_r2 else 0) | (self.dkdv_keys & 3) << 2 | (self.dbias_chunks & 63) << 4
                | (0 if self.attn_pers_bwd else 1024) | (0 if self.attn_lone_keys else 2048) | (0 if self.attn_pers_dkdv else 4096))


TUNE = Tuning()


class _LibProxy:

    def __init__(self, cdll):
        self._cdll = cdll

    def __getattr__(self, name):
        return getattr(self._cdll, name)

    @staticmethod
    def op_gemm_set_tile(mode):
        old = TUNE.tile_mode
        if mode >= 60:
            TUNE.force_splits = mode - 60
        elif mode >= 50:
            TUNE.tail_rows = mode - 50
        elif mode >= 40:
            TUNE.gm = mode - 40
        elif mode >= 20:
            if 0 <= mode - 20 <= 3:
                TUNE.fullline = mode - 20
        elif mode >= 10:
            pass
        else:
            TUNE.tile_mode = mode
        return old

    @staticmethod
    def op_gemm_set_staging(glds):
        old, TUNE.glds = TUNE.glds, 1 if glds else 0
        return old

    @staticmethod
    def op_attn_set_merge_dbias(on):
        old, TUNE.merge_dbias = TUNE.merge_dbias, 1 if on else 0
        return old

    @staticmethod
    def op_attn_set_resident(mode):
        old, TUNE.resident = TUNE.resident, int(mode)
        return old


def lib():
    global _lib
    if _lib is None:
        if not os.path.exists(LIB_PATH):
            raise RuntimeError(
                "%s not found: build it with `python one-peace_amd/build.py` (hipcc, gfx950). "
                "There is no CPU fallback for the HIP path." % LIB_PATH)
        L = ctypes.CDLL(LIB_PATH)
        for name, (res, args) in SIGNATURES.items():
            fn = getattr(L, name)
            fn.restype = res
            fn.argtypes = args
        _lib = _LibProxy(L)
    return _lib


_probe_lib = None


def probe_lib():
    global _probe_lib
    if _probe_lib is None:
        path = os.path.join(os.path.dirname(LIB_PATH), "libonepeace_probe.so")
        if not os.path.exists(path):
            raise RuntimeError("%s not found: build it with `python one-peace_amd/build.py`" % path)
        L = ctypes.CDLL(path)
        for name, (res, args) in PROBE_SIGNATURES.items():
            fn = getattr(L, name)
            fn.restype = res
            fn.argtypes = args
        _probe_lib = L
    return _probe_lib


def _check_probe(rc, what):
    if rc != 0:
        msg = probe_lib().op_last_error()
        raise RuntimeError("%s failed (rc=%d): %s" % (what, rc, msg.decode() if msg else ""))


def available():
    return os.path.exists(LIB_PATH) and torch.cuda.is_available()


def _check(rc, what):
    if rc != 0:
        msg = lib().op_last_error()
        raise RuntimeError("%s failed (rc=%d): %s" % (what, rc, msg.decode() if msg else ""))


def ptr(t):
    return None if t is None else c_void_p(t.data_ptr())


def stream():
    return c_void_p(torch.cuda.current_stream().cuda_stream)


def _dt(t):
    if t.dtype == torch.bfloat16:
        return DT_BF16
    if t.dtype == torch.float32:
        return DT_F32
    raise TypeError("unsupported dtype %s" % t.dtype)


def _req(t, name, dtype=None):
    if t is None:
        return
    if not t.is_cuda:
        raise RuntimeError("%s must be a CUDA(HIP) tensor" % name)
    if not t.is_contiguous():
        raise RuntimeError("%s must be contiguous" % name)
    if dtype is not None and t.dtype != dtype:
        raise TypeError("%s must be %s, got %s" % (name, dtype, t.dtype))


def layernorm_fwd(x2d, w, b, eps=1e-5, gelu=False, want_stats=True, q8=False, x_rows=None):
    _req(x2d, "x")
    rows, cols = x2d.shape
    if x_rows is not None:
        assert not q8 and x_rows.dtype == torch.int32 and x_rows.is_contiguous()
        rows = x_rows.numel()
    y = torch.empty(rows, cols, dtype=x2d.dtype, device=x2d.device)
    mean = rstd = None
    if want_stats:
        mean = torch.empty(rows, dtype=torch.float32, device=x2d.device)
        rstd = torch.empty(rows, dtype=torch.float32, device=x2d.device)
    if q8:
        assert not gelu and x2d.dtype == torch.bfloat16
        q = torch.empty(rows, cols, dtype=torch.uint8, device=x2d.device)
        qs = torch.empty(rows, dtype=torch.float32, device=x2d.device)
        _check(lib().op_layernorm_fwd_q8(ptr(x2d), ptr(w), ptr(b), ptr(y), ptr(mean), ptr(rstd), ptr(q), ptr(qs), rows, cols, eps, stream()),
               "op_layernorm_fwd_q8")
        return y, mean, rstd, (q, qs)
    _check(lib().op_layernorm_fwd(ptr(x2d), ptr(w), ptr(b), ptr(y), ptr(mean), ptr(rstd), rows, cols, eps,
                                  int(gelu), _dt(x2d), ptr(x_rows), stream()), "op_layernorm_fwd")
    return y, mean, rstd


_ws_cache = {}


def workspace(nbytes, device, tag="ws"):
    key = (device, tag, torch.cuda.current_stream(device).cuda_stream)
    buf = _ws_cache.get(key)
    if buf is None or buf.numel() < nbytes:
        buf = torch.empty(max(int(nbytes), 1 << 20), dtype=torch.uint8, device=device)
        _ws_cache[key] = buf
    return buf


def layernorm_bwd(dy, x, w, b, mean, rstd, gelu=False, need_wgrad=True, dw=None, db=None, accumulate=False, add=None,
                  dx=None, x_rows=None):
    rows, cols = x.shape
    if x_rows is not None:
        assert dx is not None and dx.shape == x.shape and (add is None or add.shape == x.shape) and x_rows.dtype == torch.int32
        rows = x_rows.numel()
        assert dy.shape[0] == rows
    if dx is None:
        dx = torch.empty_like(x)
    ws = None
    if need_wgrad and w is not None:
        if dw is None:
            dw = torch.empty_like(w)
            db = torch.empty_like(w)
            accumulate = False
        ws = workspace(lib().op_layernorm_bwd_workspace_bytes(rows, cols), x.device, "ln")
    else:
        dw = db = None
    _check(lib().op_layernorm_bwd(ptr(dy), ptr(x), ptr(w), ptr(b), ptr(mean), ptr(rstd), ptr(add), ptr(dx), ptr(dw), ptr(db),
                                  ptr(ws), rows, cols, int(gelu), int(accumulate), _dt(x), ptr(x_rows), stream()), "op_layernorm_bwd")
    return dx, dw, db


SPLITK_WS_BYTES = 768 << 20
GEMM_ALGO_BYTES = [0, 0]


def gemm_nt(A, Bs, biases=None, out=None, epilogue=EPI_BIAS, n_seg=0, h0=None, h1=None, resid=None, gamma=None,
            rowscale=None, rows_per_sample=0, alpha=None, N=None, ldc=None, splitk=True, resid_rows=None):
    M, K = A.shape
    if resid_rows is not None:
        assert epilogue == EPI_RESID and out is not None and resid is not None and out.shape == resid.shape and resid_rows.numel() == M
        assert resid_rows.dtype == torch.int32 and resid_rows.is_contiguous()
    Bs = list(Bs) + [None] * (3 - len(Bs))
    biases = list(biases or []) + [None] * (3 - len(biases or []))
    if epilogue == EPI_GEGLU:
        Nn = Bs[0].shape[0]
    else:
        Nn = N if N is not None else sum(b.shape[0] for b in Bs if b is not None)
        if n_seg == 0:
            n_seg = Bs[0].shape[0]
    if out is None:
        out = torch.empty(M, Nn, dtype=torch.float32 if epilogue == EPI_F32 else torch.bfloat16, device=A.device)
    ldc_ = ldc if ldc is not None else out.stride(0)
    ws, ws_bytes = None, 0
    if splitk and epilogue in (EPI_BIAS, EPI_RESID) and (K >= 2048 or M <= 1024):
        ws = workspace(min(SPLITK_WS_BYTES, 32 * M * Nn), A.device, "gemm_splitk")
        ws_bytes = ws.numel()
    outs = 1 + (2 if h1 is not None else (1 if h0 is not None else 0))
    GEMM_ALGO_BYTES[0] += 2 * (M * K + Nn * K * (2 if epilogue == EPI_GEGLU else 1) + (M * Nn if resid is not None else 0)) \
        + out.element_size() * M * Nn * outs
    GEMM_ALGO_BYTES[1] += 1
    _check(lib().op_gemm_nt(ptr(A), A.stride(0), ptr(Bs[0]), ptr(Bs[1]), ptr(Bs[2]), Bs[0].stride(0), n_seg,
                            ptr(biases[0]), ptr(biases[1]), ptr(biases[2]), ptr(out), ldc_, ptr(h0), ptr(h1),
                            ptr(resid), resid.stride(0) if resid is not None else 0, ptr(gamma), ptr(rowscale),
                            rows_per_sample, ptr(alpha), M, Nn, K, epilogue, ptr(ws), ws_bytes, TUNE.gemm(), ptr(resid_rows),
                            out.shape[0] if resid_rows is not None else 0, stream()), "op_gemm_nt")
    return out


def _ptr_array(items, n):
    arr = (c_void_p * n)()
    for i, t in enumerate(items or ()):
        arr[i] = None if t is None else t.data_ptr()
    return arr


def gemm_nt_grouped(As, Ws, biases=None, outs=None, epilogue=EPI_BIAS, h0s=None, h1s=None, resids=None, gammas=None,
                    rowscales=None, rows_per_sample=None, resid_rows=None):
    n = len(As)
    K = As[0].shape[1]
    pairs = [w if isinstance(w, (tuple, list)) else (w, None) for w in Ws]
    N = pairs[0][0].shape[0]
    if outs is None:
        outs = [torch.empty(a.shape[0], N, dtype=torch.bfloat16, device=a.device) for a in As]
    lda, ldb, ldc = As[0].stride(0), pairs[0][0].stride(0), outs[0].stride(0)
    ldr = resids[0].stride(0) if resids and resids[0] is not None else 0
    if any(a.stride(0) != lda or a.shape[1] != K for a in As) or any(w[0].stride(0) != ldb or w[0].shape != (N, K) for w in pairs) \
            or any(o.stride(0) != ldc for o in outs) or (ldr and any(r.stride(0) != ldr for r in resids)):
        return None
    flatB, flatb = [], []
    for i, (w0, w1) in enumerate(pairs):
        flatB += [w0, w1]
        flatb += [biases[i] if biases else None, None]
    Ms = (c_int64 * n)(*[a.shape[0] for a in As])
    rps = (c_int64 * n)(*[(rows_per_sample[i] if rows_per_sample else 0) for i in range(n)])
    for i, a in enumerate(As):
        outs_n = 1 + (2 if h1s and h1s[i] is not None else (1 if h0s and h0s[i] is not None else 0))
        GEMM_ALGO_BYTES[0] += 2 * (a.shape[0] * K + N * K * (2 if epilogue == EPI_GEGLU else 1)
                                   + (a.shape[0] * N if resids and resids[i] is not None else 0)) + 2 * a.shape[0] * N * outs_n
    GEMM_ALGO_BYTES[1] += 1
    rc = lib().op_gemm_nt_grouped(n, _ptr_array(As, n), Ms, lda, _ptr_array(flatB, 2 * n), ldb, _ptr_array(flatb, 2 * n),
                                  _ptr_array(outs, n), ldc, _ptr_array(h0s, n), _ptr_array(h1s, n), _ptr_array(resids, n), ldr,
                                  _ptr_array(gammas, n), _ptr_array(rowscales, n), rps, N, K, epilogue, TUNE.gemm(),
                                  _ptr_array(resid_rows, n) if resid_rows is not None else None,
                                  outs[0].shape[0] if resid_rows is not None else 0, stream())
    if rc == -95:
        return None
    _check(rc, "op_gemm_nt_grouped")
    return outs


def quant_fp8_rows(x2d, out=None):
    rows, cols = x2d.shape
    if out is not None:
        q, scale = out
    else:
        q = torch.empty(rows, cols, dtype=torch.uint8, device=x2d.device)
        scale = torch.empty(rows, dtype=torch.float32, device=x2d.device)
    _check(lib().op_quant_fp8_rows(ptr(x2d), x2d.stride(0), ptr(q), q.stride(0), ptr(scale), rows, cols, stream()), "op_quant_fp8_rows")
    return q, scale


def gemm_nt_fp8(A8, sa, B8s, sbs, bias=None, out=None, epilogue=EPI_BIAS, h0=None, h1=None, resid=None, gamma=None, rowscale=None,
                rows_per_sample=0):
    M, K = A8.shape
    N = B8s[0].shape[0]
    if out is None:
        out = torch.empty(M, N, dtype=torch.bfloat16, device=A8.device)
    B1, sb1 = (B8s[1], sbs[1]) if len(B8s) > 1 else (None, None)
    _check(lib().op_gemm_nt_fp8(ptr(A8), A8.stride(0), ptr(sa), ptr(B8s[0]), ptr(B1), B8s[0].stride(0), ptr(sbs[0]), ptr(sb1),
                                ptr(bias), ptr(out), out.stride(0), ptr(h0), ptr(h1), ptr(resid),
                                resid.stride(0) if resid is not None else 0, ptr(gamma), ptr(rowscale), rows_per_sample, M, N, K,
                                epilogue, int(TUNE.fp8_small), stream()), "op_gemm_nt_fp8")
    return out


def gemm_plan(M, N, K, epilogue=EPI_BIAS, has_bias=True, workspace_bytes=SPLITK_WS_BYTES):
    out = (ctypes.c_int * 4)()
    _check(lib().op_gemm_plan(M, N, K, epilogue, int(has_bias), workspace_bytes, TUNE.gemm(), ctypes.cast(out, P)), "op_gemm_plan")
    return out[0], out[1], bool(out[2]), out[3]


def gemm_tn_supported(K, M, N, lda, ldb):
    return (K % 64 == 0 and M % 8 == 0 and N % 8 == 0 and lda % 8 == 0 and ldb % 8 == 0 and M >= 8 and N >= 8
            and 31 * lda + M < (1 << 30) and 31 * ldb + N < (1 << 30))


def gemm_nt_batched(A, W, bias, out, rows, K):
    G, N = W.shape[0], W.shape[1]
    assert W.is_contiguous() and out.is_contiguous() and out.shape == (G, rows, N) and A.stride(2) == 1
    GEMM_ALGO_BYTES[0] += 2 * G * (rows * K + N * K + rows * N)
    GEMM_ALGO_BYTES[1] += 1
    _check(lib().op_gemm_nt_batched(ptr(A), A.stride(1), A.stride(0), ptr(W), K, N * K, ptr(bias), N if bias is not None else 0, ptr(out), N,
                                    rows * N, rows, N, K, G, stream()), "op_gemm_nt_batched")
    return out


def audio_conv1_ln_gelu_fwd(wav, stride, w0, b0, lnw, lnb, rows, eps, slack_rows=0):
    C = w0.shape[0]
    assert w0.is_contiguous() and w0.numel() == C * 10 and wav.is_contiguous() and wav.numel() >= stride * (rows - 1) + 10
    y = torch.empty(rows + slack_rows, C, dtype=torch.bfloat16, device=wav.device)
    if slack_rows:
        y[rows:].zero_()
    mean = torch.empty(rows, dtype=torch.float32, device=wav.device)
    rstd = torch.empty(rows, dtype=torch.float32, device=wav.device)
    _check(lib().op_audio_conv1_ln_gelu_fwd(ptr(wav), stride, ptr(w0), ptr(b0), ptr(lnw), ptr(lnb), ptr(y), ptr(mean), ptr(rstd), rows, C, eps,
                                            stream()), "op_audio_conv1_ln_gelu_fwd")
    return y, mean, rstd


def audio_conv1_ln_gelu_bwd(dy, wav, stride, w0, b0, lnw, lnb, mean, rstd):
    rows, C = dy.shape
    mk = lambda ref, shape: torch.empty(shape, dtype=torch.bfloat16, device=dy.device) if ref is not None else None
    dw0, db0, dlw, dlb = torch.empty(C, 10, dtype=torch.bfloat16, device=dy.device), mk(b0, C), mk(lnw, C), mk(lnb, C)
    ws = workspace(lib().op_audio_conv1_ln_gelu_bwd_workspace_bytes(C), dy.device, "audio_conv1")
    _check(lib().op_audio_conv1_ln_gelu_bwd(ptr(dy), ptr(wav), stride, ptr(w0), ptr(b0), ptr(lnw), ptr(lnb), ptr(mean), ptr(rstd), ptr(dw0), ptr(db0),
                                            ptr(dlw), ptr(dlb), ptr(ws), rows, C, 0, stream()), "op_audio_conv1_ln_gelu_bwd")
    return dw0, db0, dlw, dlb


def gemm_tn_grouped_plan(sizes, workgroups=256, tune=0):
    n = len(sizes)
    cap = sum(((m + 255) // 256) * ((nn + 255) // 256) for m, nn, _ in sizes)
    out = (ctypes.c_int32 * (4 * cap))()
    arr = lambda j: (c_int64 * n)(*[q[j] for q in sizes])
    cnt = lib().op_gemm_tn_grouped_plan(n, arr(0), arr(1), arr(2), int(workgroups), int(tune), ctypes.cast(out, P), cap)
    if cnt < 0:
        raise RuntimeError("op_gemm_tn_grouped_plan failed (%d)" % cnt)
    return [tuple(out[4 * i:4 * i + 4]) for i in range(cnt)]


def gemm_tn(A_km, B_kn, out=None, accumulate=False, splitk=True):
    K, M = A_km.shape
    N = B_kn.shape[1]
    if out is None:
        out = torch.empty(M, N, dtype=torch.bfloat16, device=A_km.device)
        accumulate = False
    ws = workspace(SPLITK_WS_BYTES, A_km.device, "gemm_splitk") if splitk else None
    GEMM_ALGO_BYTES[0] += 2 * (K * M + K * N + M * N * (2 if accumulate else 1))
    GEMM_ALGO_BYTES[1] += 1
    _check(lib().op_gemm_tn(ptr(A_km), A_km.stride(0), ptr(B_kn), B_kn.stride(0), ptr(out), out.stride(0), M, N, K,
                            int(accumulate), ptr(ws), ws.numel() if ws is not None else 0, TUNE.gemm(), stream()), "op_gemm_tn")
    return out


_tn_counters = {}
TN_GROUP_MAX = 16


def gemm_tn_grouped(problems, tune=0):
    n = len(problems)
    dev = problems[0][0].device
    key = (dev, torch.cuda.current_stream(dev).cuda_stream)
    ctr = _tn_counters.get(key)
    if ctr is None:
        ctr = _tn_counters[key] = torch.zeros(int(lib().op_gemm_tn_grouped_counter_bytes()), dtype=torch.uint8, device=dev)
    arr = lambda vals: (c_int64 * n)(*vals)
    As, Bs, Cs = [q[0] for q in problems], [q[1] for q in problems], [q[2] for q in problems]
    acc = (ctypes.c_int32 * n)(*[int(bool(q[3])) for q in problems])
    side = [tuple(q[4]) + (None,) * (3 - len(q[4])) if len(q) > 4 and q[4] is not None else (None, None, None) for q in problems]
    Ws, Rs, Ss = [x[0] for x in side], [x[1] for x in side], [x[2] for x in side]
    has_side = any(r is not None for r in Rs)
    for sc, r, a, b in zip(Ss, Rs, As, Bs):
        assert sc is None or (sc.dtype == torch.bfloat16 and sc.is_contiguous() and sc.numel() == a.shape[1])
        assert r is None or (r.dtype == torch.float32 and r.is_contiguous() and r.shape == (b.shape[1] // 128, a.shape[1])), "rowdot: fp32 [N / 128, M]"
    rc = lib().op_gemm_tn_grouped(n, _ptr_array(As, n), arr([a.stride(0) for a in As]), _ptr_array(Bs, n), arr([b.stride(0) for b in Bs]),
                                  _ptr_array(Cs, n), arr([c.stride(0) for c in Cs]), arr([a.shape[1] for a in As]),
                                  arr([b.shape[1] for b in Bs]), arr([a.shape[0] for a in As]), acc,
                                  _ptr_array(Ws, n) if has_side else None, arr([w.stride(0) if w is not None else 0 for w in Ws]) if has_side else None,
                                  _ptr_array(Rs, n) if has_side else None, _ptr_array(Ss, n) if any(x is not None for x in Ss) else None,
                                  ptr(ctr), int(tune), stream())
    if rc == -95:
        return False
    _check(rc, "op_gemm_tn_grouped")
    for a, b, c, ac in [q[:4] for q in problems]:
        K, M = a.shape
        GEMM_ALGO_BYTES[0] += 2 * (K * M + K * b.shape[1] + M * b.shape[1] * (2 if ac else 1))
    GEMM_ALGO_BYTES[1] += 1
    return True


def transpose(x2d, out=None, scale=None):
    rows, cols = x2d.shape
    if out is None:
        out = torch.empty(cols, rows, dtype=x2d.dtype, device=x2d.device)
    assert scale is None or (scale.dtype == torch.bfloat16 and scale.is_contiguous() and scale.numel() == rows)
    _check(lib().op_transpose_scaled(ptr(x2d), ptr(out), rows, cols, x2d.stride(0), out.stride(0), ptr(scale), stream()), "op_transpose")
    return out


def transpose_table(jobs, device):
    import struct
    assert lib().op_transpose_desc_bytes() == 56
    raw, tile0 = b"", 0
    for job in jobs:
        src, dst = job[:2]
        scale = job[2] if len(job) > 2 else None
        rows, cols = src.shape
        tx, ty = (cols + 63) // 64, (rows + 63) // 64
        raw += struct.pack("<QQiiqqiiQ", src.data_ptr(), dst.data_ptr(), rows, cols, src.stride(0), dst.stride(0), tile0, tx,
                           scale.data_ptr() if scale is not None else 0)
        tile0 += tx * ty
    table = torch.frombuffer(bytearray(raw), dtype=torch.uint8).to(device)
    return table, tile0


def transpose_batched(table, n, total_tiles):
    _check(lib().op_transpose_batched(ptr(table), n, total_tiles, stream()), "op_transpose_batched")


def colsum(x, y=None, rowscale=None, rows_per_sample=0, mul=None, out=None, accumulate=False, out_dtype=torch.bfloat16):
    M, N = x.shape
    if out is None:
        out = torch.empty(N, dtype=out_dtype, device=x.device)
        accumulate = False
    ws = workspace(lib().op_colsum_workspace_bytes(N), x.device, "colsum")
    _check(lib().op_colsum(ptr(x), ptr(y), ptr(rowscale), rows_per_sample, ptr(mul), ptr(out), ptr(ws), M, N,
                           int(accumulate), _dt(out), stream()), "op_colsum")
    return out


def colsum_segments(x, seg_cols, outs=None, accumulate=False):
    M, N = x.shape
    n_seg = N // seg_cols
    if outs is None:
        outs = [torch.empty(seg_cols, dtype=x.dtype, device=x.device) for _ in range(n_seg)]
        accumulate = False
    o = list(outs) + [None] * (3 - len(outs))
    ws = workspace(lib().op_colsum_workspace_bytes(N), x.device, "colsum")
    _check(lib().op_colsum_segments(ptr(x), ptr(o[0]), ptr(o[1]), ptr(o[2]), ptr(ws), M, n_seg, seg_cols, int(accumulate),
                                    stream()), "op_colsum_segments")
    return outs


def resid_bwd(dout, y=None, gamma=None, rowscale=None, rows_per_sample=0, dgamma=None, dbias=None, accumulate=False, g0=None,
              dout_rows=None):
    M, N = dout.shape
    if dout_rows is not None:
        assert dout_rows.dtype == torch.int32 and dout_rows.is_contiguous() and dout.is_contiguous()
        M = dout_rows.numel()
    out = torch.empty(M, N, dtype=dout.dtype, device=dout.device)
    if dgamma is True:
        dgamma = torch.empty(N, dtype=dout.dtype, device=dout.device)
    if dbias is True:
        dbias = torch.empty(N, dtype=dout.dtype, device=dout.device)
    ws = None
    if dgamma is not None or dbias is not None or g0 is not None:
        ws = workspace(lib().op_resid_bwd_workspace_bytes(N), dout.device, "resid")
    assert g0 is None or (g0.dtype == torch.float32 and g0.is_contiguous() and g0.numel() == N)
    _check(lib().op_resid_bwd(ptr(dout), ptr(y if dgamma is not None else None), ptr(gamma), ptr(rowscale), rows_per_sample,
                              ptr(out), ptr(dgamma), ptr(dbias), ptr(g0), ptr(ws), M, N, int(accumulate), ptr(dout_rows), stream()),
           "op_resid_bwd")
    return out, dgamma, dbias


def gamma_grad_finish(rowdot, pairs, dgamma, accumulate):
    assert rowdot.dtype == torch.float32 and rowdot.dim() == 2 and rowdot.is_contiguous() and len(pairs) <= 3 and dgamma.dtype == torch.bfloat16
    assert rowdot.shape[1] == dgamma.numel()
    flat = []
    for b, g0 in list(pairs) + [(None, None)] * (3 - len(pairs)):
        flat += [ptr(b), ptr(g0)]
    _check(lib().op_gamma_grad_finish(ptr(rowdot), rowdot.shape[0], *flat, ptr(dgamma), rowdot.shape[1], int(accumulate), stream()),
           "op_gamma_grad_finish")
    return dgamma


def ln_geglu_bwd(dy, h0, h1, w, mean, rstd, dw=None, db=None, accumulate=False, need_wgrad=True, dh0=None, dh1=None):
    rows, cols = h0.shape
    if dh0 is None:
        dh0, dh1 = torch.empty_like(h0), torch.empty_like(h1)
    assert dh0.stride(0) == dh1.stride(0) and dh0.stride(1) == 1 and dh1.stride(1) == 1
    assert h0.stride(0) == h1.stride(0) and h0.stride(1) == 1 and h1.stride(1) == 1
    ws = None
    if need_wgrad:
        if dw is None:
            dw, db, accumulate = torch.empty_like(w), torch.empty_like(w), False
        ws = workspace(lib().op_layernorm_bwd_workspace_bytes(rows, cols), h0.device, "ln")
    else:
        dw = db = None
    _check(lib().op_ln_geglu_bwd(ptr(dy), ptr(h0), ptr(h1), ptr(w), ptr(mean), ptr(rstd), ptr(dh0), ptr(dh1), dh0.stride(0),
                                 h0.stride(0), ptr(dw), ptr(db), ptr(ws), rows, cols, int(accumulate), stream()), "op_ln_geglu_bwd")
    return dh0, dh1, dw, db


def ln_geglu_fwd(h0, h1, w, b, eps=1e-5, want_stats=True, out=None, mean=None, rstd=None, q8=None):
    rows, cols = h0.shape
    assert h0.stride(0) == h1.stride(0) and h0.stride(1) == 1 and h1.stride(1) == 1
    y = out if out is not None else torch.empty(rows, cols, dtype=h0.dtype, device=h0.device)
    if want_stats and mean is None:
        mean = torch.empty(rows, dtype=torch.float32, device=h0.device)
        rstd = torch.empty(rows, dtype=torch.float32, device=h0.device)
    if q8 is not None:
        assert q8[0].is_contiguous() and q8[0].shape == (rows, cols) and y.is_contiguous()
        _check(lib().op_ln_geglu_fwd_q8(ptr(h0), ptr(h1), h0.stride(0), ptr(w), ptr(b), ptr(y), ptr(mean), ptr(rstd), ptr(q8[0]), ptr(q8[1]),
                                        rows, cols, eps, stream()), "op_ln_geglu_fwd_q8")
        return y, mean, rstd
    _check(lib().op_ln_geglu_fwd(ptr(h0), ptr(h1), h0.stride(0), ptr(w), ptr(b), ptr(y), ptr(mean), ptr(rstd), rows, cols, eps, stream()),
           "op_ln_geglu_fwd")
    return y, mean, rstd


def geglu_bwd(dg, h0, h1):
    dh0, dh1 = torch.empty_like(h0), torch.empty_like(h1)
    _check(lib().op_geglu_bwd(ptr(dg), ptr(h0), ptr(h1), ptr(dh0), ptr(dh1), dg.numel(), stream()), "op_geglu_bwd")
    return dh0, dh1


def scale_rows(dout, gamma=None, rowscale=None, rows_per_sample=0):
    M, N = dout.shape
    out = torch.empty_like(dout)
    _check(lib().op_scale_rows(ptr(dout), ptr(gamma), ptr(rowscale), rows_per_sample, ptr(out), M, N, stream()),
           "op_scale_rows")
    return out


def l2norm_fwd(x, out_dtype=torch.bfloat16, eps=1e-12):
    rows, cols = x.shape
    y = torch.empty(rows, cols, dtype=out_dtype, device=x.device)
    inv = torch.empty(rows, dtype=torch.float32, device=x.device)
    _check(lib().op_l2norm_fwd(ptr(x), ptr(y), ptr(inv), rows, cols, eps, _dt(y), stream()), "op_l2norm_fwd")
    return y, inv


def l2norm_bwd(dy, y, inv):
    rows, cols = y.shape
    dx = torch.empty(rows, cols, dtype=torch.bfloat16, device=y.device)
    _check(lib().op_l2norm_bwd(ptr(dy), ptr(y), ptr(inv), ptr(dx), rows, cols, _dt(y), stream()), "op_l2norm_bwd")
    return dx


def infonce_rows(sim, target0, label_smoothing=0.0, gscale=1.0, write_grad=True):
    rows, n = sim.shape
    dev = sim.device
    loss = torch.empty(rows, dtype=torch.float32, device=dev)
    hit = torch.empty(rows, dtype=torch.float32, device=dev)
    dot = torch.empty(rows, dtype=torch.float32, device=dev)
    _check(lib().op_infonce_rows(ptr(sim), rows, n, sim.stride(0), target0, label_smoothing, gscale, ptr(loss), ptr(hit),
                                 ptr(dot), int(write_grad), stream()), "op_infonce_rows")
    return loss, hit, dot


def adamw_step(p, g, m, v, lr, beta1, beta2, eps, weight_decay, step, grad_scale=1.0, grad_sqnorm=None, clip_norm=0.0):
    _check(lib().op_adamw_step(ptr(p), ptr(g), ptr(m), ptr(v), p.numel(), lr, beta1, beta2, eps, weight_decay, step,
                               grad_scale, ptr(grad_sqnorm), clip_norm, stream()), "op_adamw_step")


def adamw_step_groups(p, g, m, v, group_end8, group_lr_scale, group_wd, lr, beta1, beta2, eps, step, grad_scale=1.0,
                      grad_sqnorm=None, clip_norm=0.0):
    _check(lib().op_adamw_step_groups(ptr(p), ptr(g), ptr(m), ptr(v), p.numel(), ptr(group_end8), ptr(group_lr_scale),
                                      ptr(group_wd), group_end8.numel(), lr, beta1, beta2, eps, step, grad_scale, ptr(grad_sqnorm),
                                      clip_norm, stream()), "op_adamw_step_groups")


def sqnorm(x, out=None):
    if out is None:
        out = torch.empty(1, dtype=torch.float32, device=x.device)
    ws = workspace(4096, x.device, "sqnorm")
    _check(lib().op_sqnorm(ptr(x), x.numel(), ptr(ws), ptr(out), stream()), "op_sqnorm")
    return out


def relpos_bias_build(table, bucket_i32, S, Spad, transposed=False):
    heads = table.shape[1]
    out = torch.empty(heads, S, Spad, dtype=torch.bfloat16, device=table.device)
    _check(lib().op_relpos_bias_build(ptr(table), ptr(bucket_i32), bucket_i32.stride(0), ptr(out), heads, S, Spad,
                                      int(transposed), stream()), "op_relpos_bias_build")
    return out


PAIR_SEG = 32


def relpos_pairs(bucket_i32, S, num_rel):
    key = (S, num_rel, bucket_i32._version)
    cached = getattr(bucket_i32, "_op_pairs", None)
    if cached is not None and cached[0] == key:
        return cached[1]
    dev = bucket_i32.device
    vals, order = torch.sort(bucket_i32[:S, :S].reshape(-1).long(), stable=True)
    pair_off = torch.searchsorted(vals, torch.arange(num_rel + 1, device=dev))
    bucket_seg = torch.zeros(num_rel + 1, dtype=torch.int64, device=dev)
    bucket_seg[1:] = ((pair_off[1:] - pair_off[:-1] + PAIR_SEG - 1) // PAIR_SEG).cumsum(0)
    nseg = S * S // PAIR_SEG + num_rel
    t = torch.arange(nseg, device=dev)
    r = torch.searchsorted(bucket_seg[1:], t, right=True)
    rc = r.clamp(max=num_rel - 1)
    seg = torch.full((nseg + 1,), S * S, dtype=torch.int64, device=dev)
    seg[:nseg] = torch.where(r < num_rel, pair_off[rc] + (t - bucket_seg[rc]) * PAIR_SEG, S * S)
    res = (order.to(torch.int32), seg.to(torch.int32), bucket_seg.to(torch.int32), nseg)
    bucket_i32._op_pairs = (key, res)
    return res


def relpos_bias_bwd(dbias_f32, bucket_i32, num_rel, S, Spad):
    heads = dbias_f32.shape[0]
    pos, seg, bucket_seg, nseg = relpos_pairs(bucket_i32, S, num_rel)
    dtable = torch.empty(num_rel, heads, dtype=torch.float32, device=dbias_f32.device)
    partial = torch.empty(nseg, heads, dtype=torch.float32, device=dbias_f32.device)
    _check(lib().op_relpos_bias_bwd(ptr(dbias_f32), S, Spad, ptr(pos), ptr(seg), nseg, ptr(bucket_seg), num_rel, ptr(partial), ptr(dtable),
                                    heads, stream()), "op_relpos_bias_bwd")
    return dtable


def relpos_bias_build_ids(table, bucket_i32, ids_i32, Kpad, transposed=False):
    B, K = ids_i32.shape
    heads = table.shape[1]
    out = torch.empty(B, heads, K, Kpad, dtype=torch.bfloat16, device=table.device)
    _check(lib().op_relpos_bias_build_ids(ptr(table), ptr(bucket_i32), bucket_i32.stride(0), ptr(ids_i32), ptr(out), B, heads, K, Kpad,
                                          int(transposed), stream()), "op_relpos_bias_build_ids")
    return out


def relpos_bias_bwd_ids(dbias_f32, bucket_i32, ids_i32, num_rel):
    B, heads, K, Kpad = dbias_f32.shape
# ... 258 lines not shown
```

### one-peace_amd/ops.py

```python
import math
import os
import weakref

import torch

from . import hip

_wt_cache = {}
_cache_epoch = 0


_refresh_plan = None


def invalidate_weight_cache():
    global _cache_epoch
    _cache_epoch += 1


def refresh_weight_cache():
    global _cache_epoch, _refresh_plan
    _cache_epoch += 1
    if not FP8_FFN and (_fp8_cache or _fp8_derived_cache):
        _fp8_cache.clear()
# ... 549 lines not shown
            return torch.zeros(_unused.shape[:-1] + (ctx.S,), dtype=_unused.dtype, device=_unused.device), None
        g = h.acc[..., : ctx.S].to(_unused.dtype)
        h.acc = None
        return g, None


class _RelPosImageFn(torch.autograd.Function):
    @staticmethod
    def forward(ctx, table, handle):
        ctx.handle_ref = weakref.ref(handle)
        ctx.shape = tuple(table.shape)
        if handle.ids is not None:
            return hip.relpos_bias_build_ids(table, handle.bucket, handle.ids, handle.Spad)
        return hip.relpos_bias_build(table, handle.bucket, handle.S, handle.Spad)

    @staticmethod
    def backward(ctx, _unused):
        h = ctx.handle_ref()
        if h is None or h.acc is None:
            return torch.zeros(ctx.shape, dtype=torch.bfloat16, device=_unused.device), None
        if h.ids is not None:
            dtable = hip.relpos_bias_bwd_ids(h.acc, h.bucket, h.ids, h.num_rel)
        else:
            dtable = hip.relpos_bias_bwd(h.acc.sum(0), h.bucket, h.num_rel, h.S, h.Spad)
        h.acc = None
        return dtable.to(torch.bfloat16), None


_DIRECT_WEIGHTS = ("wq", "wk", "wv", "wo", "w0", "w1", "w2")
ATTN_PARAMS = ("ln1_w", "ln1_b", "wq", "bq", "wk", "wv", "bv", "aln_w", "aln_b", "wo", "bo", "g1")
FFN_PARAMS = ("ln2_w", "ln2_b", "w0", "w1", "fln_w", "fln_b", "w2", "b2", "g2")
LAYER_PARAMS = ATTN_PARAMS + FFN_PARAMS


class StreamSeg:
    __slots__ = ("name", "B", "S", "row0", "bias", "key_pad", "pad")

    def __init__(self, name, B, S, row0, bias=None, key_pad=None, pad=0):
        self.name, self.B, self.S, self.row0, self.bias, self.key_pad, self.pad = name, B, S, row0, bias, key_pad, pad

    @property
    def tokens(self):
        return self.B * self.S

    @property
    def rows(self):
        return self.B * self.S + self.pad

    @property
    def end(self):
        return self.row0 + self.B * self.S + self.pad

    def frag(self, limit):
        return self.bias.frag if self.bias is not None and self.S <= limit else None


def _attn_forward(x2, P, segs, heads, scale, rowscale, rps, keep, want_y=True, xmap=None, out=None):
    H = x2.shape[1]
    xln1, mean1, rstd1 = hip.layernorm_fwd(x2, P["ln1_w"], P["ln1_b"], want_stats=keep, x_rows=xmap)
    if H % 128 == 0:
        Nr = xln1.shape[0]
        full = _qkv_rows_that_fill_whole_rounds(Nr, 3 * H) if QKV_ROUND_SPLIT else Nr
        if full < Nr:
            qkv = torch.empty(Nr, 3 * H, dtype=x2.dtype, device=x2.device)
            for lo, hi in ((0, full), (full, Nr)):
                hip.gemm_nt(xln1[lo:hi], [P["wq"], P["wk"], P["wv"]], [P["bq"], None, P["bv"]], n_seg=H, N=3 * H, out=qkv[lo:hi])
        else:
            qkv = hip.gemm_nt(xln1, [P["wq"], P["wk"], P["wv"]], [P["bq"], None, P["bv"]], n_seg=H, N=3 * H)
    else:
        qkv = torch.empty(xln1.shape[0], 3 * H, dtype=x2.dtype, device=x2.device)
        for i, (w, b) in enumerate(((P["wq"], P["bq"]), (P["wk"], None), (P["wv"], P["bv"]))):
            hip.gemm_nt(xln1, [w], [b] if b is not None else None, out=qkv[:, i * H:(i + 1) * H], ldc=3 * H)
    attn = torch.empty_like(xln1)
    lses = []
    for sg in segs:
        r = slice(sg.row0, sg.end)
        _, lse = hip.attn_fwd(qkv[r, :H], qkv[r, H:2 * H], qkv[r, 2 * H:], 3 * H, sg.B, sg.S, heads, scale,
                              sg.bias.image.detach() if sg.bias is not None else None, sg.key_pad, hip.attn_spad(sg.S), out=attn[r],
                              want_lse=keep, bias_frag=sg.frag(hip.ATTN_RESIDENT_MAX_S))
        lses.append(lse)
        if sg.pad:
            attn[sg.end - sg.pad:sg.end].zero_()
    if P["aln_w"] is not None:
        aln, mean_a, rstd_a = hip.layernorm_fwd(attn, P["aln_w"], P["aln_b"], want_stats=keep)
    else:
        aln, mean_a, rstd_a = attn, None, None
    y1 = torch.empty_like(xln1) if keep and want_y else None
    x_mid = hip.gemm_nt(aln, [P["wo"]], [P["bo"]], epilogue=hip.EPI_RESID, resid=x2, gamma=P["g1"], rowscale=rowscale,
                        rows_per_sample=rps, h0=y1, out=out, resid_rows=xmap)
    if not keep:
        return x_mid, None
    acts = dict(xln1=xln1, mean1=mean1, rstd1=rstd1, qkv=qkv, attn=attn, aln=aln, mean_a=mean_a, rstd_a=rstd_a, y1=y1)
    for i, lse in enumerate(lses):
        acts["lse%d" % i] = lse
    return x_mid, acts


QKV_ROUND_SPLIT = os.environ.get("ONEPEACE_QKV_ROUND_SPLIT", "1") != "0"
SKIP_ROW_TABLES = os.environ.get("ONEPEACE_SKIP_ROW_TABLES", "1") != "0"


def _row_tables(kept):
    return kept is not None and SKIP_ROW_TABLES and not FP8_FFN


def _qkv_rows_that_fill_whole_rounds(rows, n_out, cus=256, max_tail=512):
    tn, tm = (n_out + 255) // 256, (rows + 255) // 256
    rounds = -(-tm * tn // cus)
    tm_main = (rounds - 1) * cus // tn
    full = tm_main * 256
    return full if 0 < rows - full <= max_tail and tm_main > 0 else rows


GEGLU_SPLIT = os.environ.get("ONEPEACE_GEGLU_SPLIT", "1") != "0"
SEPARATE_DELTA = os.environ.get("ONEPEACE_SEPARATE_DELTA", "0") == "1"


def _geglu_split(Fd, fln_w):
    return GEGLU_SPLIT and fln_w is not None and Fd % 256 == 0


def _register_direct(ctx, names, params, needs):
    ctx.direct = tuple((n, q) for n, q, ng in zip(names, params, needs) if ng and q is not None and _direct_grad(q))
    for _, q in ctx.direct:
        q._op_pending = getattr(q, "_op_pending", 0) + 1


def _targets(direct, *names):
    if all(n in direct for n in names):
        return [direct[n].grad for n in names], True
    return [None] * len(names), False


def _finish(direct, G, names, values, accumulated):
    for n, v in zip(names, values):
        if accumulated:
            _direct_grad_done(direct[n])
        else:
            G[n] = v


def _return_grads(names, params, G, direct):
    out = []
    for n, q in zip(names, params):
        g = G.get(n) if q is not None else None
        if g is not None and n in direct:
            direct[n].grad.add_(g.view_as(direct[n].grad))
            _direct_grad_done(direct[n])
            g = None
        out.append(g)
    return out


def _resid_backward(dout, y, gamma, ps, S, gname, bname, direct, G, needs, g0=None, rows=None, fold=None):
    names = tuple(n for n, present in ((gname, gamma is not None and g0 is None), (bname, True)) if present and needs.get(n))
    tgt, acc = _targets(direct, *names) if names else ([], False)
    t = dict(zip(names, tgt))
    dgamma = (t[gname] if acc else True) if gname in t else None
    dbias = (t[bname] if acc else True) if bname in t else None
    dy, dg, db = hip.resid_bwd(dout, y if dgamma is not None else None, gamma, ps, S, dgamma=dgamma, dbias=dbias, accumulate=acc, g0=g0,
                               dout_rows=rows)
    if fold is not None and gname in t:
        if not acc:
            fold[gname] = fold[gname] + dg.float() if gname in fold else dg.float()
        names = tuple(n for n in names if n != gname)
    _finish(direct, G, names, tuple({gname: dg, bname: db}[n] for n in names), acc)
    return dy


def _adjacent_grads(direct, names):
    if not all(n in direct for n in names):
        return None
    order = sorted(names, key=lambda n: direct[n].grad.data_ptr())
    for a, b in zip(order, order[1:]):
        ga, gb = direct[a].grad, direct[b].grad
        if not ga.is_contiguous() or ga.data_ptr() + ga.numel() * ga.element_size() != gb.data_ptr() or ga.shape[1:] != gb.shape[1:]:
            return None
    return order


def _span(direct, order):
    g0 = direct[order[0]].grad
    return torch.as_strided(g0, (sum(direct[n].grad.shape[0] for n in order), g0.shape[1]), (g0.shape[1], 1))


def _weight_grad_fn(ctx, G):
    direct = dict(ctx.direct)

    def weight_grad(name, dyv, xv, side=None, after=None):
        target = direct.get(name)
        if target is not None:
            wgrad_into(dyv, xv, target.grad, (target,), side, after)
        else:
            assert side is None and after is None
            G[name] = wgrad(dyv, xv)
    return weight_grad, direct


def _gamma_finish_hook(rowdot, gamma_param, pairs, done):
    def run():
        hip.gamma_grad_finish(rowdot, pairs, gamma_param.grad, True)
        if done:
            _direct_grad_done(gamma_param)
    return run


def _save(ctx, keep, acts, *tensors):
    if keep:
        ctx.act_names = [k for k, v in acts.items() if v is not None]
        ctx.save_for_backward(*tensors, *[acts[k] for k in ctx.act_names])
    else:
        ctx.act_names = None
        ctx.save_for_backward(*tensors)


def _restore(ctx, saved_acts, optional):
    A = dict(zip(ctx.act_names, saved_acts))
    for k in optional:
        A.setdefault(k, None)
    return A


class AttnBranchFn(torch.autograd.Function):

    @staticmethod
    def forward(ctx, x2, segs, rowscale, rps, heads, save_acts, kept, *rest):
        nseg = len(segs)
        params = rest[nseg:]
        P = dict(zip(ATTN_PARAMS, params))
        need_grad = any(ctx.needs_input_grad) and bool(int(save_acts) & 2)
        keep = bool(int(save_acts) & 1) and need_grad
        first_param = 7 + nseg
        needs = dict(zip(ATTN_PARAMS, ctx.needs_input_grad[first_param:]))
        x_full = x2
        mapped = _row_tables(kept)
        if kept is not None and not mapped:
            x2 = hip.rows_gather(x_full, kept)
        H = x2.shape[1]
        N = kept.total if mapped else x2.shape[0]
        scale = (H // heads) ** -0.5
        ctx.dg_fused = need_grad and dgamma_from_wgrad_ok([N], P["g1"], [P["wo"]], [P["bo"]], needs["g1"], [needs["wo"]])
        if mapped:
            x_mid = torch.empty_like(x_full)
            _, acts = _attn_forward(x_full, P, segs, heads, scale, rowscale, rps, keep, want_y=needs["g1"] and not ctx.dg_fused,
                                    xmap=kept.rowmap(), out=x_mid)
            hip.rows_merge(x_full, None, kept, out=x_mid)
        else:
            x_mid, acts = _attn_forward(x2, P, segs, heads, scale, rowscale, rps, keep, want_y=needs["g1"] and not ctx.dg_fused)
            if kept is not None:
                x_mid = hip.rows_merge(x_full, x_mid, kept)
        ctx.kept, ctx.mapped = kept, mapped
        ctx.segs, ctx.dims, ctx.n_params, ctx.first_param = segs, (N, H, heads, scale, rps), len(params), first_param
        ctx.direct = ()
        if need_grad:
            _register_direct(ctx, ATTN_PARAMS, params, ctx.needs_input_grad[first_param:])
        if keep:
            if not needs["wo"]:
                acts["aln"] = None if P["aln_w"] is not None else acts["aln"]
            if not (needs["wq"] or needs["wk"] or needs["wv"]):
                acts["xln1"] = None
        ctx.cheap = keep and bool(int(save_acts) & 4)
        if ctx.cheap:
            acts["xln1"] = None
            if P["aln_w"] is not None:
                acts["aln"] = None
        _save(ctx, keep, acts, x2, rowscale, *params)
        return x_mid

    @staticmethod
    def backward(ctx, dx_mid):
        x2, rowscale, *rest = ctx.saved_tensors
        params, saved_acts = rest[:ctx.n_params], rest[ctx.n_params:]
        N, H, heads, scale, rps = ctx.dims
        segs = ctx.segs
        nseg = len(segs)
        P = dict(zip(ATTN_PARAMS, params))
        needs = {n: bool(ng) and q is not None for n, q, ng in zip(ATTN_PARAMS, params, ctx.needs_input_grad[ctx.first_param:])}
        need_x = bool(ctx.needs_input_grad[0])
        want_dbias = [sg.bias is not None and sg.bias.image.requires_grad for sg in segs]
        kept, mapped = ctx.kept, ctx.mapped
        xmap = kept.rowmap() if mapped else None
        if ctx.act_names is not None:
            A = _restore(ctx, saved_acts, ("mean_a", "rstd_a", "y1", "xln1", "aln"))
            if ctx.cheap:
                if needs["wq"] or needs["wk"] or needs["wv"]:
                    A["xln1"] = hip.layernorm_fwd(x2, P["ln1_w"], P["ln1_b"], x_rows=xmap)[0]
                if needs["wo"] and P["aln_w"] is not None:
                    A["aln"] = hip.layernorm_fwd(A["attn"], P["aln_w"], P["aln_b"])[0]
        else:
            _, A = _attn_forward(x2, P, segs, heads, scale, rowscale, rps, True, want_y=not ctx.dg_fused, xmap=xmap,
                                 out=torch.empty_like(x2) if mapped else None)
        if not dx_mid.is_contiguous():
            dx_mid = dx_mid.contiguous()
        dx_full = dx_mid
        if kept is not None and not mapped:
            dx_mid = hip.rows_gather(dx_full, kept)
        G = {}
        weight_grad, direct = _weight_grad_fn(ctx, G)
        if ctx.dg_fused:
            g0 = torch.empty(H, dtype=torch.float32, device=dx_mid.device)
            dy1 = _resid_backward(dx_mid, None, P["g1"], rowscale, rps, "g1", "bo", direct, G, needs, g0=g0, rows=xmap)
            rowdot, (rd_wo,) = _rowdot_slots(dx_mid.device, [P["wo"]])
            weight_grad("wo", dy1, A["aln"], side=(P["wo"], rd_wo, P["g1"]),
                        after=_gamma_finish_hook(rowdot, direct["g1"], [(P["bo"], g0)] if P["bo"] is not None else [], True))
            wo_t = _transposed(P["wo"], scale=P["g1"])
        else:
            dy1 = _resid_backward(dx_mid, A["y1"], P["g1"], rowscale, rps, "g1", "bo", direct, G, needs, rows=xmap)
            if needs["wo"]:
                weight_grad("wo", dy1, A["aln"])
            wo_t = None
        upstream = ("ln1_w", "ln1_b", "wq", "bq", "wk", "wv", "bv", "aln_w", "aln_b")
        dx = None
        if need_x or any(want_dbias) or any(needs[n] for n in upstream):
            daln = hip.gemm_nt(dy1, [wo_t if wo_t is not None else _transposed(P["wo"])])
            if P["aln_w"] is not None:
                want = needs["aln_w"] or needs["aln_b"]
                (tw, tb), acc = _targets(direct, "aln_w", "aln_b") if want else ((None, None), False)
                dattn, dw_, db_ = hip.layernorm_bwd(daln, A["attn"], P["aln_w"], P["aln_b"], A["mean_a"], A["rstd_a"], dw=tw, db=tb,
                                                    accumulate=acc, need_wgrad=want)
                if want:
                    _finish(direct, G, ("aln_w", "aln_b"), (dw_, db_), acc)
            else:
                dattn = daln
            qkv_names = ("wq", "wk", "wv")
            order = _adjacent_grads(direct, qkv_names) if all(needs[n] for n in qkv_names) and H % 8 == 0 else None
            cols = tuple(order) if order else qkv_names
            slot = {n: i for i, n in enumerate(cols)}
            qkv = A["qkv"]
            dqkv = torch.empty_like(qkv)
            for i, sg in enumerate(segs):
                r = slice(sg.row0, sg.end)
                if sg.pad:
                    dqkv[sg.end - sg.pad:sg.end].zero_()
                dparts = {n: dqkv[r, slot[n] * H:(slot[n] + 1) * H] for n in qkv_names}
                _attn_backward(qkv[r], dattn[r], A["attn"][r], A["lse%d" % i], sg.B, sg.S, heads, scale,
                               sg.bias.image.detach() if sg.bias is not None else None, sg.bias.imageT if sg.bias is not None else None,
                               sg.key_pad, sg.bias.grad_accumulator(sg.B) if want_dbias[i] else None, sg.frag(384),
                               dparts["wq"], dparts["wk"], dparts["wv"])
            bias_of = {"wq": "bq", "wv": "bv"}
            bnames = tuple(bias_of[n] for n in cols if n in bias_of and needs[bias_of[n]])
            if bnames:
                tgt, acc = _targets(direct, *bnames)
                if H % 8 == 0:
                    outs = [None, None, None]
                    for n, t_ in zip(bnames, tgt):
                        outs[slot["wq" if n == "bq" else "wv"]] = t_ if acc else torch.empty(H, dtype=dqkv.dtype, device=dqkv.device)
                    hip.colsum_segments(dqkv, H, outs, accumulate=acc)
                    _finish(direct, G, bnames, tuple(outs[slot["wq" if n == "bq" else "wv"]] for n in bnames), acc)
                else:
                    sums = hip.colsum(dqkv)
                    for n in bnames:
                        i = slot["wq" if n == "bq" else "wv"]
                        G[n] = sums[i * H:(i + 1) * H]
            if order:
                wgrad_into(dqkv, A["xln1"], _span(direct, order), [direct[n] for n in order])
            elif any(n in direct for n in qkv_names) or not all(needs[n] for n in qkv_names):
                for n in qkv_names:
                    if needs[n]:
                        weight_grad(n, dqkv[:, slot[n] * H:(slot[n] + 1) * H], A["xln1"])
            else:
                dW = wgrad(dqkv, A["xln1"])
                G["wq"], G["wk"], G["wv"] = dW[:H], dW[H:2 * H], dW[2 * H:]
            if need_x or needs["ln1_w"] or needs["ln1_b"]:
                dxln1 = hip.gemm_nt(dqkv, [_transposed(tuple(P[n] for n in cols))])
                want = needs["ln1_w"] or needs["ln1_b"]
                (tw, tb), acc = _targets(direct, "ln1_w", "ln1_b") if want else ((None, None), False)
                dx, dw_, db_ = hip.layernorm_bwd(dxln1, x2, P["ln1_w"], P["ln1_b"], A["mean1"], A["rstd1"], add=dx_mid, dw=tw, db=tb,
                                                 accumulate=acc, need_wgrad=want, dx=torch.empty_like(dx_full) if mapped else None,
                                                 x_rows=xmap)
                if want:
                    _finish(direct, G, ("ln1_w", "ln1_b"), (dw_, db_), acc)
        if dx is None and need_x:
            dx = dx_full
        elif dx is not None and mapped:
            hip.rows_merge(dx_full, None, kept, out=dx)
        elif dx is not None and kept is not None:
            dx = hip.rows_merge(dx_full, dx, kept)
        flush_wgrads()
        grads = _return_grads(ATTN_PARAMS, params, G, direct)
        dimgs = []
        for sg, w in zip(segs, want_dbias):
            if w and not getattr(sg.bias, "_grad_routed", False):
                sg.bias._grad_routed = True
                img = sg.bias.image
                dimgs.append(torch.zeros((), dtype=img.dtype, device=img.device).expand(img.shape))
            else:
                dimgs.append(None)
        return (dx, None, None, None, None, None, None, *dimgs, *grads)


FFN_SHARED = ("ln2_w", "ln2_b", "g2")
FFN_OWN = ("w0", "w1", "fln_w", "fln_b", "w2", "b2")


class FfnBranchMultiFn(torch.autograd.Function):

    @staticmethod
    def _compute(x2, segs, pss, params, keep, want_y, grad=None, xmap=None):
        nseg = len(segs)
        shared = dict(zip(FFN_SHARED, params[:3]))
        own = [dict(zip(FFN_OWN, params[3 + 6 * i:9 + 6 * i])) for i in range(nseg)]
        H = x2.shape[1]
        N = xmap.numel() if xmap is not None else x2.shape[0]
        Fd = own[0]["w0"].shape[0]
        dev, dt = x2.device, x2.dtype
        has_fln = own[0]["fln_w"] is not None
        split = (keep if grad is None else grad) and _geglu_split(Fd, own[0]["fln_w"])
        fp8 = FP8_FFN and H % 128 == 0 and Fd % 128 == 0
        gq = None
        if fp8 and split:
            xln2, mean2, rstd2, (xq, xs) = hip.layernorm_fwd(x2, shared["ln2_w"], shared["ln2_b"], want_stats=keep, q8=True)
            gq, gs = torch.empty(N, Fd, dtype=torch.uint8, device=dev), torch.empty(N, dtype=torch.float32, device=dev)
        else:
            xln2, mean2, rstd2 = hip.layernorm_fwd(x2, shared["ln2_w"], shared["ln2_b"], want_stats=keep, x_rows=xmap)
            if fp8:
                xq, xs = hip.quant_fp8_rows(xln2)
        if split:
            hh = torch.empty(N, 2 * Fd, dtype=dt, device=dev)
            g, h0, h1 = None, hh[:, :Fd], hh[:, Fd:]
        else:
            g = torch.empty(N, Fd, dtype=dt, device=dev)
            h0 = torch.empty(N, Fd, dtype=dt, device=dev) if keep else None
            h1 = torch.empty(N, Fd, dtype=dt, device=dev) if keep else None
        gln = torch.empty(N, Fd, dtype=dt, device=dev) if has_fln else g
        mean_f = torch.empty(N, dtype=torch.float32, device=dev) if (keep or split) and has_fln else None
        rstd_f = torch.empty(N, dtype=torch.float32, device=dev) if (keep or split) and has_fln else None
        L = hip.lib()
        for sg, P in zip(segs, own):
            r = slice(sg.row0, sg.end)
            if split:
                if fp8:
                    w01q, w01s = _fp8_weight_pair(P["w0"], P["w1"])
                    hip.gemm_nt_fp8(xq[r], xs[r], [w01q], [w01s], out=hh[r])
                else:
                    hip.gemm_nt(xln2[r], [P["w0"], P["w1"]], n_seg=Fd, N=2 * Fd, out=hh[r])
                hip.ln_geglu_fwd(h0[r], h1[r], P["fln_w"], P["fln_b"], out=gln[r], mean=mean_f[r], rstd=rstd_f[r],
                                 q8=(gq[r], gs[r]) if fp8 else None)
                continue
            if fp8:
                (w0q, w0s), (w1q, w1s) = _fp8_weight(P["w0"]), _fp8_weight(P["w1"])
                hip.gemm_nt_fp8(xq[r], xs[r], [w0q, w1q], [w0s, w1s], epilogue=hip.EPI_GEGLU, h0=h0[r] if keep else None,
                                h1=h1[r] if keep else None, out=g[r])
            else:
                hip.gemm_nt(xln2[r], [P["w0"], P["w1"]], epilogue=hip.EPI_GEGLU, h0=h0[r] if keep else None, h1=h1[r] if keep else None,
                            out=g[r])
            if has_fln:
                hip._check(L.op_layernorm_fwd(hip.ptr(g[r]), hip.ptr(P["fln_w"]), hip.ptr(P["fln_b"]), hip.ptr(gln[r]),
                                              hip.ptr(mean_f[r]) if keep else None, hip.ptr(rstd_f[r]) if keep else None, sg.rows, Fd, 1e-5, 0,
                                              hip.DT_BF16, None, hip.stream()), "op_layernorm_fwd")
        y2 = torch.empty(N, H, dtype=dt, device=dev) if keep and want_y else None
        out = torch.empty_like(x2)
        rs = [slice(sg.row0, sg.end) for sg in segs]
        if fp8:
            if gq is None:
                gq, gs = hip.quant_fp8_rows(gln)
            for sg, P, r, ps in zip(segs, own, rs, pss):
                w2q, w2s = _fp8_weight(P["w2"])
                hip.gemm_nt_fp8(gq[r], gs[r], [w2q], [w2s], bias=P["b2"], epilogue=hip.EPI_RESID, resid=x2[r], gamma=shared["g2"], rowscale=ps,
                                rows_per_sample=sg.S, h0=y2[r] if y2 is not None else None, out=out[r])
            acts = dict(xln2=xln2, mean2=mean2, rstd2=rstd2, h0=h0, h1=h1, gln=gln, mean_f=mean_f, rstd_f=rstd_f, y2=y2) if keep else None
            return out, acts
        tabs = [xmap[r] for r in rs] if xmap is not None else None
        grouped = nseg > 1 and hip.gemm_nt_grouped(
            [gln[r] for r in rs], [P["w2"] for P in own], biases=[P["b2"] for P in own],
            outs=[out[r] for r in rs] if tabs is None else [out] * nseg, epilogue=hip.EPI_RESID,
            h0s=[y2[r] for r in rs] if y2 is not None else None, resids=[x2[r] for r in rs] if tabs is None else [x2] * nseg,
            gammas=[shared["g2"]] * nseg, rowscales=list(pss), rows_per_sample=[sg.S for sg in segs], resid_rows=tabs) is not None
        if not grouped:
            for i, (sg, P, r, ps) in enumerate(zip(segs, own, rs, pss)):
                hip.gemm_nt(gln[r], [P["w2"]], [P["b2"]], epilogue=hip.EPI_RESID, resid=x2[r] if tabs is None else x2, gamma=shared["g2"],
                            rowscale=ps, rows_per_sample=sg.S, h0=y2[r] if y2 is not None else None, out=out[r] if tabs is None else out,
                            resid_rows=tabs[i] if tabs is not None else None)
        acts = dict(xln2=xln2, mean2=mean2, rstd2=rstd2, h0=h0, h1=h1, gln=gln, mean_f=mean_f, rstd_f=rstd_f, y2=y2) if keep else None
        return out, acts

    @staticmethod
    def forward(ctx, x2, segs, pss, save_acts, kept, *params):
        nseg = len(segs)
        Fd = params[3].shape[0]
        need_grad = any(ctx.needs_input_grad) and bool(int(save_acts) & 2)
        keep = bool(int(save_acts) & 1) and need_grad
        needs = ctx.needs_input_grad[5:]
        has_fln = params[5] is not None
        x_full = x2
        mapped = _row_tables(kept)
        if kept is not None and not mapped:
            x2 = hip.rows_gather(x_full, kept)
        H = x2.shape[1]
        N = kept.total if mapped else x2.shape[0]
        w2s, b2s = [params[3 + 6 * i + 4] for i in range(nseg)], [params[3 + 6 * i + 5] for i in range(nseg)]
        ctx.dg_fused = need_grad and dgamma_from_wgrad_ok([sg.rows for sg in segs], params[2], w2s, b2s, bool(needs[2]),
                                                           [bool(needs[3 + 6 * i + 4]) for i in range(nseg)])
        out, acts = FfnBranchMultiFn._compute(x2, segs, pss, params, keep, bool(needs[2]) and not ctx.dg_fused, grad=bool(int(save_acts) & 2),
                                              xmap=kept.rowmap() if mapped else None)
        if mapped:
            hip.rows_merge(x_full, None, kept, out=out)
        elif kept is not None:
            out = hip.rows_merge(x_full, out, kept)
        ctx.kept, ctx.mapped = kept, mapped
        ctx.segs, ctx.n_params, ctx.dims = segs, len(params), (N, H, Fd)
        ctx.direct = ()
        names = list(FFN_SHARED) + ["%s@%d" % (n, i) for i in range(nseg) for n in FFN_OWN]
        ctx.names = names
        if need_grad:
            _register_direct(ctx, names, params, needs)
        if keep:
            nd = dict(zip(names, needs))
            if not any(nd["w0@%d" % i] or nd["w1@%d" % i] for i in range(nseg)):
                acts["xln2"] = None
            if has_fln and not any(nd["w2@%d" % i] for i in range(nseg)):
                acts["gln"] = None
        ctx.cheap = keep and bool(int(save_acts) & 4)
        if ctx.cheap:
            acts["xln2"] = None
            if _geglu_split(Fd, params[5]):
                acts["gln"] = None
        _save(ctx, keep, acts or {}, x2, *[ps for ps in pss], *params)
        ctx.n_ps = len(pss)
        return out

    @staticmethod
    def backward(ctx, dout):
        x2, *rest = ctx.saved_tensors
        pss, rest = rest[:ctx.n_ps], rest[ctx.n_ps:]
        params, saved_acts = rest[:ctx.n_params], rest[ctx.n_params:]
        segs, names = ctx.segs, ctx.names
        nseg = len(segs)
        N, H, Fd = ctx.dims
        P = dict(zip(names, params))
        needs = {n: bool(ng) and q is not None for n, q, ng in zip(names, params, ctx.needs_input_grad[5:])}
        need_x = bool(ctx.needs_input_grad[0])
        kept, mapped = ctx.kept, ctx.mapped
        xmap = kept.rowmap() if mapped else None
        if ctx.act_names is not None:
            A = _restore(ctx, saved_acts, ("mean_f", "rstd_f", "y2", "gln", "xln2"))
            if ctx.cheap:
                if any(needs["%s@%d" % (n, i)] for i in range(nseg) for n in ("w0", "w1")):
                    A["xln2"] = hip.layernorm_fwd(x2, P["ln2_w"], P["ln2_b"], x_rows=xmap)[0]
                if A["gln"] is None and any(needs["w2@%d" % i] for i in range(nseg)):
                    A["gln"] = torch.empty(N, Fd, dtype=x2.dtype, device=x2.device)
                    for i, sg in enumerate(segs):
                        r = slice(sg.row0, sg.end)
                        hip.ln_geglu_fwd(A["h0"][r], A["h1"][r], P["fln_w@%d" % i], P["fln_b@%d" % i], out=A["gln"][r], want_stats=False)
        else:
            _, A = FfnBranchMultiFn._compute(x2, segs, pss, params, True, not ctx.dg_fused, xmap=xmap)
        if not dout.is_contiguous():
            dout = dout.contiguous()
        dout_full = dout
        if kept is not None and not mapped:
            dout = hip.rows_gather(dout_full, kept)
        G = {}
        weight_grad, direct = _weight_grad_fn(ctx, G)
        has_fln = P["fln_w@0"] is not None
        dev, dt = dout.device, dout.dtype
        upstream = need_x or needs["ln2_w"] or needs["ln2_b"] or any(
            needs["%s@%d" % (n, i)] for i in range(nseg) for n in ("w0", "w1", "fln_w", "fln_b"))
        dh = torch.empty(N, 2 * Fd, dtype=dt, device=dev) if upstream else None
        dgln = torch.empty(N, Fd, dtype=dt, device=dev) if upstream else None
        colsets = []
        fold = {} if nseg > 1 else None
        fused = ctx.dg_fused
        fp8b = FP8_FFN and FP8_FFN_DGRAD and H % 128 == 0 and Fd % 128 == 0
        (rowdot, rd_views), pairs = (_rowdot_slots(dev, [P["w2@%d" % i] for i in range(nseg)]), []) if fused else ((None, None), None)
        for i, sg in enumerate(segs):
            r = slice(sg.row0, sg.end)
            k = lambda n: "%s@%d" % (n, i)
            g0 = None
            if fused:
                g0 = torch.empty(H, dtype=torch.float32, device=dev)
                if P[k("b2")] is not None:
                    pairs.append((P[k("b2")], g0))
            dy2 = _resid_backward(dout_full if mapped else dout[r], A["y2"][r] if A["y2"] is not None else None, P["g2"], pss[i], sg.S,
                                  "g2", k("b2"), direct, G, needs, g0=g0, rows=xmap[r] if mapped else None, fold=fold)
            if fused:
                weight_grad(k("w2"), dy2, A["gln"][r], side=(P[k("w2")], rd_views[i], P["g2"]),
                            after=_gamma_finish_hook(rowdot, direct["g2"], pairs, True) if i == nseg - 1 else None)
            elif needs[k("w2")]:
                weight_grad(k("w2"), dy2, A["gln"][r])
            if not upstream:
                colsets.append(None)
                continue
            w2t = _transposed(P[k("w2")], scale=P["g2"] if fused else None)
            if fp8b:
                hip.gemm_nt_fp8(*hip.quant_fp8_rows(dy2), *[[x] for x in _fp8_derived(w2t)], out=dgln[r])
            else:
                hip.gemm_nt(dy2, [w2t], out=dgln[r])
            pair = (k("w0"), k("w1"))
            order = _adjacent_grads(direct, pair) if needs[pair[0]] and needs[pair[1]] and Fd % 8 == 0 else None
            cols = tuple(order) if order else pair
            colsets.append(cols)
            dpart = {n: dh[r, j * Fd:(j + 1) * Fd] for j, n in enumerate(cols)}
            if has_fln:
                want = needs[k("fln_w")] or needs[k("fln_b")]
                (tw, tb2), acc = _targets(direct, k("fln_w"), k("fln_b")) if want else ((None, None), False)
                _, _, dw_, db2_ = hip.ln_geglu_bwd(dgln[r], A["h0"][r], A["h1"][r], P[k("fln_w")], A["mean_f"][r], A["rstd_f"][r], dw=tw,
                                                   db=tb2, accumulate=acc, need_wgrad=want, dh0=dpart[pair[0]], dh1=dpart[pair[1]])
                if want:
                    _finish(direct, G, (k("fln_w"), k("fln_b")), (dw_, db2_), acc)
            else:
                d0, d1 = hip.geglu_bwd(dgln[r], A["h0"][r], A["h1"][r])
                dpart[pair[0]].copy_(d0)
                dpart[pair[1]].copy_(d1)
            if order:
                wgrad_into(dh[r], A["xln2"][r], _span(direct, order), [direct[n] for n in order])
            else:
                for n in pair:
                    if needs[n]:
                        weight_grad(n, dpart[n], A["xln2"][r])
        if fold is not None and needs["g2"] and not fused:
            if "g2" in fold:
                G["g2"] = fold["g2"].to(dt)
            else:
                _direct_grad_done(direct["g2"])
        dx = None
        if upstream and (need_x or needs["ln2_w"] or needs["ln2_b"]):
            dxln2 = torch.empty(N, H, dtype=dt, device=dev)
            rs = [slice(sg.row0, sg.end) for sg in segs]
            wts = [_transposed(tuple(P[n] for n in cols)) for cols in colsets]
            if fp8b:
                for r, wt in zip(rs, wts):
                    hip.gemm_nt_fp8(*hip.quant_fp8_rows(dh[r]), *[[x] for x in _fp8_derived(wt)], out=dxln2[r])
            elif nseg == 1 or hip.gemm_nt_grouped([dh[r] for r in rs], wts, outs=[dxln2[r] for r in rs]) is None:
                for r, wt in zip(rs, wts):
                    hip.gemm_nt(dh[r], [wt], out=dxln2[r])
            want = needs["ln2_w"] or needs["ln2_b"]
            (tw, tb), acc = _targets(direct, "ln2_w", "ln2_b") if want else ((None, None), False)
            dx, dw_, db_ = hip.layernorm_bwd(dxln2, x2, P["ln2_w"], P["ln2_b"], A["mean2"], A["rstd2"], add=dout, dw=tw, db=tb,
                                             accumulate=acc, need_wgrad=want, dx=torch.empty_like(dout_full) if mapped else None, x_rows=xmap)
            if want:
                _finish(direct, G, ("ln2_w", "ln2_b"), (dw_, db_), acc)
        if dx is None and need_x:
            dx = dout_full
        elif dx is not None and mapped:
            hip.rows_merge(dout_full, None, kept, out=dx)
        elif dx is not None and kept is not None:
            dx = hip.rows_merge(dout_full, dx, kept)
        grads = _return_grads(names, params, G, direct)
        return (dx, None, None, None, None, *grads)


def ffn_branch_multi(x2, segs, pss, shared, own, save_acts=True, kept=None):
    flat = list(shared)
    for o in own:
        flat += list(o)
    return FfnBranchMultiFn.apply(x2, segs, tuple(pss), _save_flags(save_acts), kept, *flat)


_SCALE_ROWS = {}


def kept_segments(kept, segs, device):
    out = []
    for i, sg in enumerate(segs):
        key_pad = sg.key_pad.index_select(0, kept.kept_list(i)) if sg.key_pad is not None else None
        out.append(StreamSeg(sg.name, kept.n_kept[i], sg.S, kept.dst_row0[i], sg.bias, key_pad, pad=kept.dst_rows[i] - kept.n_kept[i] * sg.S))
    key = (device, kept.scale)
    vec = _SCALE_ROWS.get(key)
    if vec is None or vec.numel() < kept.total + 8:
        if len(_SCALE_ROWS) > 256:
            _SCALE_ROWS.clear()
        vec = _SCALE_ROWS[key] = torch.full((max(kept.full_rows, kept.total) + 8,), kept.scale, dtype=torch.float32, device=device)
    return out, vec


def _attn_backward(qkv, dattn, attn, lse, B, S, heads, scale, bias_img, biasT, key_pad, dbias_acc, bias_frag, dq, dk, dv):
    H = heads * 64
    dev = qkv.device
    Spad = hip.attn_spad(S)
    delta = torch.empty(B, heads, Spad, dtype=torch.float32, device=dev)
    if attn.stride(0) != dattn.stride(0) or SEPARATE_DELTA:
        hip._check(hip.lib().op_attn_bwd_delta(hip.ptr(dattn), hip.ptr(attn), dattn.stride(0), hip.ptr(delta), B, S, Spad, heads,
                                               hip.stream()), "op_attn_bwd_delta")
        attn = None
    hip.attn_bwd_launch(qkv[:, :H], qkv[:, H:2 * H], qkv[:, 2 * H:], 3 * H, dattn, bias_img, biasT, key_pad, lse, delta, dq, dk,
                        dv, dq.stride(0), dbias_acc, B, S, Spad, heads, scale, bias_frag, out=attn)


def attn_branch(x, bias, key_pad, ps, heads, params, save_acts=False):
    B, S, H = x.shape
    seg = StreamSeg("x", B, S, 0, bias, key_pad)
    out = AttnBranchFn.apply(x.reshape(B * S, H), [seg], ps, S, heads, _save_flags(save_acts), None, bias.image if bias is not None else None, *params)
    return out.view(B, S, H)


def attn_branch_multi(x2, segs, ps_rows, heads, params, save_acts=False, kept=None):
    return AttnBranchFn.apply(x2, segs, ps_rows, 1, heads, _save_flags(save_acts), kept,
                              *[sg.bias.image if sg.bias is not None else None for sg in segs], *params)


def _save_flags(save_acts):
    return int(bool(save_acts)) | (2 if torch.is_grad_enabled() else 0) | (4 if RECOMPUTE_CHEAP and save_acts else 0)


def ffn_branch(x, ps, params, save_acts=False):
    B, S, H = x.shape
    P = dict(zip(FFN_PARAMS, params))
    out = ffn_branch_multi(x.reshape(B * S, H), [StreamSeg("x", B, S, 0)], [ps], [P[n] for n in FFN_SHARED], [[P[n] for n in FFN_OWN]],
                           save_acts)
    return out.view(B, S, H)


class L2NormalizeFn(torch.autograd.Function):

    @staticmethod
    def forward(ctx, x):
        y, inv = hip.l2norm_fwd(x.contiguous())
        ctx.save_for_backward(y, inv)
        return y

    @staticmethod
    def backward(ctx, dy):
        y, inv = ctx.saved_tensors
        return hip.l2norm_bwd(dy.contiguous(), y, inv)


def l2_normalize(x):
    return L2NormalizeFn.apply(x)


class InfoNCEFn(torch.autograd.Function):

    @staticmethod
    def forward(ctx, a_local, b_local, a_all, b_all, scale, rank, label_smoothing):
        b = a_local.shape[0]
        t0 = rank * b
        scale_f = scale.detach().float().reshape(1)
        sims, rows = [], []
        for loc, allv in ((a_local, b_all), (b_local, a_all)):
            sim = gemm_any(loc.detach(), allv.detach(), out_f32=True, alpha=scale_f)
            loss_r, hit_r, dot_r = hip.infonce_rows(sim, t0, label_smoothing, gscale=0.5 / b, write_grad=True)
            sims.append(sim)
            rows.append((loss_r, hit_r, dot_r))
        loss = 0.5 * (rows[0][0].mean() + rows[1][0].mean())
        ctx.save_for_backward(a_local, b_local, a_all, b_all, scale_f, sims[0], sims[1], rows[0][2], rows[1][2])
        ctx.scale_dtype = scale.dtype
        hits_a, hits_b = rows[0][1].sum(), rows[1][1].sum()
        ctx.mark_non_differentiable(hits_a, hits_b)
        return loss, hits_a, hits_b

    @staticmethod
    def backward(ctx, gl, _ga, _gb):
        a_local, b_local, a_all, b_all, scale_f, ds_ab, ds_ba, dot_ab, dot_ba = ctx.saved_tensors
        g = gl.float()
        coef = (g * scale_f).reshape(1)
        da = gemm_any(ds_ab.to(torch.bfloat16), hip.transpose(b_all.contiguous()), out_f32=True, alpha=coef)
        db = gemm_any(ds_ba.to(torch.bfloat16), hip.transpose(a_all.contiguous()), out_f32=True, alpha=coef)
        dscale = (g * (dot_ab.sum() + dot_ba.sum()) / scale_f).reshape(()).to(ctx.scale_dtype)
        return da.to(a_local.dtype), db.to(b_local.dtype), None, None, dscale, None, None


def info_nce(a_local, b_local, a_all, b_all, scale, rank=0, label_smoothing=0.0):
    return InfoNCEFn.apply(a_local, b_local, a_all, b_all, scale, rank, label_smoothing)


class DclFn(torch.autograd.Function):

    @staticmethod
    def forward(ctx, student, teacher, scale, label_smoothing, block):
        m, H = student.shape
        teacher = teacher.detach().contiguous()
        teacher_t = hip.transpose(teacher)
        alpha = torch.full((1,), float(scale), dtype=torch.float32, device=student.device)
        dstudent = torch.empty(m, H, dtype=torch.float32, device=student.device)
        total = torch.zeros((), dtype=torch.float32, device=student.device)
        for r0 in range(0, m, block):
            rows = student[r0:r0 + block].detach().contiguous()
            sim = gemm_any(rows, teacher, out_f32=True, alpha=alpha)
            loss_r, _, _ = hip.infonce_rows(sim, r0, label_smoothing, gscale=1.0 / m, write_grad=True)
            total += loss_r.sum()
            dstudent[r0:r0 + block] = gemm_any(sim.to(torch.bfloat16), teacher_t, out_f32=True, alpha=alpha)
            del sim
        ctx.save_for_backward(dstudent)
        ctx.dtype = student.dtype
        return total / m

    @staticmethod
    def backward(ctx, g):
        (dstudent,) = ctx.saved_tensors
        return (dstudent * g.float()).to(ctx.dtype), None, None, None, None


# ... 3 lines not shown
```

Before: 185.0.

## Fuse next block's residual-scale backward into layernorm backward via cross-block link

Adds a linked layernorm-backward kernel that, while producing dx, also writes the rowscale-scaled branch gradient and per-segment column partials (g0) that the upstream block's residual backward would otherwise compute in a separate pass. Python-side offer/find link objects pair adjacent attention/FFN autograd functions so the consumer takes the precomputed dy and g0 instead of calling resid_bwd. Bias gradients are then folded into the gamma-grad finish kernel. This saves a full read of dout per block but adds an extra output write, more LDS, and cross-function state coupling.

Result: no change. 185.3, median of 6 (+0.2%).

```diff
diff --git a/include/onepeace_hip.h b/include/onepeace_hip.h
--- a/include/onepeace_hip.h
+++ b/include/onepeace_hip.h
@@ -20,6 +20,9 @@
 int op_layernorm_bwd(const void* dy, const void* x, const void* w, const void* b, const float* mean, const float* rstd,
                      const void* add, void* dx, void* dw, void* db, void* workspace, int64_t rows, int64_t cols,
                      int act_gelu, int accumulate, int dtype, const int* x_rows, void* stream);
+int op_layernorm_bwd_link(const void* dy, const void* x, const void* w, const float* mean, const float* rstd, const void* add, void* dx,
+                          void* dw, void* db, void* workspace, int64_t rows, int64_t cols, int accumulate, void* u, int64_t n_seg,
+                          const int64_t* seg_end, const int64_t* seg_rps, const float* const* rowscale, float* const* g0, void* stream);
 
 int op_gemm_nt(const void* A, int64_t lda, const void* B0, const void* B1, const void* B2, int64_t ldb, int64_t n_seg,
                const void* bias0, const void* bias1, const void* bias2, void* C, int64_t ldc, void* h0, void* h1,
@@ -98,6 +101,9 @@
                  const int* dout_rows, void* stream);
 int op_gamma_grad_finish(const float* rowdot, int64_t slots, const void* b0, const float* g00, const void* b1, const float* g01,
                          const void* b2, const float* g02, void* dgamma, int64_t N, int accumulate, void* stream);
+int op_gamma_grad_finish_bias(const float* rowdot, int64_t slots, const void* b0, const float* g00, const void* b1, const float* g01,
+                              const void* b2, const float* g02, void* dgamma, int64_t N, int accumulate, const void* gamma, void* db0,
+                              void* db1, void* db2, void* stream);
 int op_ln_geglu_bwd(const void* dy, const void* h0, const void* h1, const void* w, const float* mean, const float* rstd,
                     void* dh0, void* dh1, int64_t ldd, int64_t ldh, void* dw, void* db, void* workspace, int64_t rows,
                     int64_t cols, int accumulate, void* stream);
diff --git a/one-peace_amd/csrc/elementwise.hip b/one-peace_amd/csrc/elementwise.hip
--- a/one-peace_amd/csrc/elementwise.hip
+++ b/one-peace_amd/csrc/elementwise.hip
@@ -121,7 +121,9 @@
                                                                 const bf16_t* __restrict__ b0, const float* __restrict__ g00,
                                                                 const bf16_t* __restrict__ b1, const float* __restrict__ g01,
                                                                 const bf16_t* __restrict__ b2, const float* __restrict__ g02,
-                                                                bf16_t* __restrict__ dgamma, int N, int accumulate) {
+                                                                bf16_t* __restrict__ dgamma, int N, int accumulate,
+                                                                const bf16_t* __restrict__ gamma = nullptr, bf16_t* __restrict__ db0 = nullptr,
+                                                                bf16_t* __restrict__ db1 = nullptr, bf16_t* __restrict__ db2 = nullptr) {
   __shared__ float part[4][64];
   const int lane = threadIdx.x & 63, w = threadIdx.x >> 6;
   const int n = blockIdx.x * 64 + lane;
@@ -144,6 +146,10 @@
   if (g01) t += (b1 ? (float)b1[n] : 0.f) * g01[n];
   if (g02) t += (b2 ? (float)b2[n] : 0.f) * g02[n];
   dgamma[n] = (bf16_t)(t + (accumulate ? (float)dgamma[n] : 0.f));
+  const float gm = gamma ? (float)gamma[n] : 1.f;
+  if (db0) db0[n] = (bf16_t)(g00[n] * gm + (float)db0[n]);
+  if (db1) db1[n] = (bf16_t)(g01[n] * gm + (float)db1[n]);
+  if (db2) db2[n] = (bf16_t)(g02[n] * gm + (float)db2[n]);
 }
 
 __global__ __launch_bounds__(256) void resid_bwd_kernel(const bf16_t* __restrict__ dout, const bf16_t* __restrict__ y,
@@ -734,6 +740,18 @@
   return OP_OK;
 }
 
+int op_gamma_grad_finish_bias(const float* rowdot, int64_t slots, const void* b0, const float* g00, const void* b1, const float* g01,
+                              const void* b2, const float* g02, void* dgamma, int64_t N, int accumulate, const void* gamma, void* db0,
+                              void* db1, void* db2, void* stream) {
+  OP_CHECK_ARG(rowdot && dgamma && N > 0 && slots > 0, "gamma_grad_finish_bias: null pointer");
+  OP_CHECK_ARG((!db0 || g00) && (!db1 || g01) && (!db2 || g02), "gamma_grad_finish_bias: a bias gradient without its g0");
+  hipLaunchKernelGGL(gamma_grad_finish_kernel, dim3(ceil_div(N, 64)), dim3(256), 0, (hipStream_t)stream, rowdot, (int)slots,
+                     (const bf16_t*)b0, g00, (const bf16_t*)b1, g01, (const bf16_t*)b2, g02, (bf16_t*)dgamma, (int)N, accumulate,
+                     (const bf16_t*)gamma, (bf16_t*)db0, (bf16_t*)db1, (bf16_t*)db2);
+  OP_LAUNCH_CHECK();
+  return OP_OK;
+}
+
 int op_colsum_segments(const void* x, void* out0, void* out1, void* out2, void* workspace, int64_t M, int64_t n_seg,
                        int64_t seg_cols, int accumulate, void* stream) {
   OP_CHECK_ARG(x && workspace, "colsum_segments: null pointer");
diff --git a/one-peace_amd/csrc/layernorm.hip b/one-peace_amd/csrc/layernorm.hip
--- a/one-peace_amd/csrc/layernorm.hip
+++ b/one-peace_amd/csrc/layernorm.hip
@@ -273,13 +273,23 @@
   }
 }
 
-template <typename T, int CH, int NW, bool GELU, bool NT>
+constexpr int LN_LINK_SEGS = 4;
+struct LnLink {
+  bf16_t* u;
+  float* g0ws;
+  const float* rs[LN_LINK_SEGS];
+  int64_t end[LN_LINK_SEGS];
+  int rps[LN_LINK_SEGS];
+  int nseg;
+};
+
+template <typename T, int CH, int NW, bool GELU, bool NT, bool LINK = false>
 __global__ __launch_bounds__(256) void ln_bwd_kernel(const T* __restrict__ dy, const T* __restrict__ x,
                                                      const T* __restrict__ w, const T* __restrict__ b,
                                                      const float* __restrict__ mean_in,
                                                      const float* __restrict__ rstd_in, const T* __restrict__ add,
                                                      T* __restrict__ dx, float* __restrict__ ws, int64_t rows, int cols,
-                                                     const int* __restrict__ xmap = nullptr) {
+                                                     const int* __restrict__ xmap = nullptr, const LnLink L = LnLink{}) {
   extern __shared__ __attribute__((aligned(16))) float smem[];
   float* red = smem;
   constexpr int G = 64 * NW;
@@ -296,10 +306,34 @@
 #pragma unroll
     for (int j = 0; j < 8; ++j) { wv[i][j] = 1.f; bv[i][j] = 0.f; dwa[i][j] = 0.f; dba[i][j] = 0.f; }
     if (c < cols) {
-      if (w) Vec8<T>::load(w + c, wv[i]);
+      if (w && !LINK) Vec8<T>::load(w + c, wv[i]);
       if (GELU && b) Vec8<T>::load(b + c, bv[i]);
     }
   }
+  float ga[LINK ? CH : 1][8];
+  typename Vec8<T>::raw_t wraw[LINK ? CH : 1];
+  int cur = 0;
+  if constexpr (LINK) {
+#pragma unroll
+    for (int i = 0; i < CH; ++i) {
+      const int c = (tig + G * i) * 8;
+#pragma unroll
+      for (int j = 0; j < 8; ++j) { ga[i][j] = 0.f; wraw[i][j] = (T)1.0f; }
+      if (c < cols && w) wraw[i] = Vec8<T>::ldraw(w + c);
+    }
+  }
+  auto park = [&]() {
+    float* dst = smem + ((int64_t)4 * (1 + cur) + wid) * cols;
+#pragma unroll
+    for (int i = 0; i < CH; ++i) {
+      const int c = (tig + G * i) * 8;
+      if (c < cols) {
+#pragma unroll
+        for (int j = 0; j < 8; ++j) { dst[c + j] = ga[LINK ? i : 0][j]; ga[LINK ? i : 0][j] = 0.f; }
+      }
+    }
+    ++cur;
+  };
   typedef typename Vec8<T>::raw_t raw_t;
   raw_t curx[CH], curg[CH], nxtx[CH], nxtg[CH], addv[CH];
   int64_t src = row0 < rows ? (xmap ? (int64_t)xmap[row0] : row0) : -1;
@@ -317,6 +351,12 @@
   }
   for (int64_t row = row0; row < rows; row += rstep) {
     const float mean = mean_in[row], rstd = rstd_in[row];
+    float usc = 1.f;
+    if constexpr (LINK) {
+      while (cur < L.nseg - 1 && row >= L.end[cur]) park();
+      const float* rs = L.rs[cur];
+      if (rs) usc = rs[(row - (cur ? L.end[cur - 1] : 0)) / L.rps[cur]];
+    }
     const int64_t nrow = row + rstep, nnrow = nrow + rstep;
     if (nnrow < rows) nnsrc = xmap ? (int64_t)xmap[nnrow] : nnrow;
 #pragma unroll
@@ -339,6 +379,10 @@
       if (c < cols) {
         Vec8<T>::cvt(curx[i], xh[i]);
         Vec8<T>::cvt(curg[i], g[i]);
+        if constexpr (LINK) {
+          asm volatile("" : "+v"(wraw[i]));
+          Vec8<T>::cvt(wraw[i], wv[i]);
+        }
 #pragma unroll
         for (int j = 0; j < 8; ++j) {
           xh[i][j] = (xh[i][j] - mean) * rstd;
@@ -369,6 +413,16 @@
           for (int j = 0; j < 8; ++j) o[j] += av[j];
         }
         store_sel<T, NT>(dr + c, o);
+        if constexpr (LINK) {
+          float uo[8];
+#pragma unroll
+          for (int j = 0; j < 8; ++j) {
+            const float t = usc * (float)(T)o[j];
+            ga[i][j] += t;
+            uo[j] = t;
+          }
+          store_sel<T, NT>(L.u + row * (int64_t)cols + c, uo);
+        }
       }
     }
 #pragma unroll
@@ -376,8 +430,44 @@
     src = nsrc;
     nsrc = nnsrc;
   }
-  if (ws == nullptr) return;
+  if (!LINK && ws == nullptr) return;
   float* wsb = ws + (int64_t)blockIdx.x * 2 * cols;
+  if constexpr (LINK) {
+    while (cur < L.nseg - 1) park();
+    if (ws != nullptr) {
+#pragma unroll
+      for (int pass = 0; pass < 2; ++pass) {
+        __syncthreads();
+#pragma unroll
+        for (int i = 0; i < CH; ++i) {
+          const int c = (tig + G * i) * 8;
+          if (c < cols) {
+#pragma unroll
+            for (int j = 0; j < 8; ++j) smem[wid * cols + c + j] = pass == 0 ? dwa[i][j] : dba[i][j];
+          }
+        }
+        __syncthreads();
+        for (int c = threadIdx.x; c < cols; c += 256)
+          wsb[pass * cols + c] = smem[c] + smem[cols + c] + smem[2 * cols + c] + smem[3 * cols + c];
+      }
+    }
+    __syncthreads();
+#pragma unroll
+    for (int i = 0; i < CH; ++i) {
+      const int c = (tig + G * i) * 8;
+      if (c < cols) {
+#pragma unroll
+        for (int j = 0; j < 8; ++j) smem[wid * cols + c + j] = ga[i][j];
+      }
+    }
+    __syncthreads();
+    for (int sg = 0; sg < L.nseg; ++sg) {
+      const float* p = sg == L.nseg - 1 ? smem : smem + (int64_t)4 * (1 + sg) * cols;
+      float* dst = L.g0ws + ((int64_t)sg * gridDim.x + blockIdx.x) * cols;
+      for (int c = threadIdx.x; c < cols; c += 256) dst[c] = p[c] + p[cols + c] + p[2 * cols + c] + p[3 * cols + c];
+    }
+    return;
+  }
   if (NW == 1) {
 #pragma unroll
     for (int pass = 0; pass < 2; ++pass) {
@@ -611,6 +701,67 @@
   return OP_OK;
 }
 
+struct FoldJob { const float* part; bf16_t* out; float* outf; int64_t pstride; };
+struct FoldJobs { FoldJob j[2 + LN_LINK_SEGS]; };
+__global__ __launch_bounds__(256) void partials_reduce_jobs_kernel(const FoldJobs J, int parts, int N, int accumulate) {
+  __shared__ float red[8][33];
+  const FoldJob job = J.j[blockIdx.y];
+  if (job.out == nullptr && job.outf == nullptr) return;
+  const int c = threadIdx.x & 31, pg = threadIdx.x >> 5;
+  const int n = blockIdx.x * 32 + c;
+  float a = 0.f;
+  if (n < N) {
+#pragma unroll 8
+    for (int p = pg; p < parts; p += 8) a += job.part[(int64_t)p * job.pstride + n];
+  }
+  red[pg][c] = a;
+  __syncthreads();
+  if (pg == 0 && n < N) {
+    float t = 0.f;
+#pragma unroll
+    for (int i = 0; i < 8; ++i) t += red[i][c];
+    if (job.outf) job.outf[n] = t;
+    else job.out[n] = (bf16_t)(t + (accumulate ? (float)job.out[n] : 0.f));
+  }
+}
+
+int ln_bwd_link_dispatch(const bf16_t* DY, const bf16_t* X, const bf16_t* W, const float* mean, const float* rstd, const bf16_t* ADD,
+                         bf16_t* DX, bf16_t* dw, bf16_t* db, float* ws, int64_t rows, int cols, int accumulate, LnLink L, float* const* g0,
+                         hipStream_t s) {
+  float* wsk = (dw || db) ? ws : nullptr;
+  const bool nt = (int64_t)rows * cols * (int64_t)sizeof(bf16_t) >= ((int64_t)64 << 20);
+  const int grid = ln_grid(rows, 1, g_ln_blocks_bwd);
+  L.g0ws = ws + (int64_t)grid * 2 * cols;
+  const size_t sh = (size_t)4 * L.nseg * cols * sizeof(float);
+#define LN_BL(CH)                                                                                                            \
+  do {                                                                                                                       \
+    if (nt) {                                                                                                                \
+      OP_ENSURE_LDS((ln_bwd_kernel<bf16_t, CH, 1, false, true, true>), 4 * LN_LINK_SEGS * 2048 * sizeof(float), "layernorm_bwd_link"); \
+      hipLaunchKernelGGL((ln_bwd_kernel<bf16_t, CH, 1, false, true, true>), dim3(grid), dim3(256), sh, s, DY, X, W, (const bf16_t*)nullptr, \
+                         mean, rstd, ADD, DX, wsk, rows, cols, (const int*)nullptr, L);                                     \
+    } else {                                                                                                                 \
+      OP_ENSURE_LDS((ln_bwd_kernel<bf16_t, CH, 1, false, false, true>), 4 * LN_LINK_SEGS * 2048 * sizeof(float), "layernorm_bwd_link"); \
+      hipLaunchKernelGGL((ln_bwd_kernel<bf16_t, CH, 1, false, false, true>), dim3(grid), dim3(256), sh, s, DY, X, W, (const bf16_t*)nullptr, \
+                         mean, rstd, ADD, DX, wsk, rows, cols, (const int*)nullptr, L);                                     \
+    }                                                                                                                        \
+  } while (0)
+  if (cols <= 512) LN_BL(1);
+  else if (cols <= 1024) LN_BL(2);
+  else if (cols <= 1536) LN_BL(3);
+  else LN_BL(4);
+#undef LN_BL
+  OP_LAUNCH_CHECK();
+  FoldJobs J = {};
+  if (wsk) {
+    J.j[0] = FoldJob{ws, dw, nullptr, (int64_t)2 * cols};
+    J.j[1] = FoldJob{ws + cols, db, nullptr, (int64_t)2 * cols};
+  }
+  for (int i = 0; i < L.nseg; ++i) J.j[2 + i] = FoldJob{L.g0ws + (int64_t)i * grid * cols, nullptr, g0[i], (int64_t)cols};
+  hipLaunchKernelGGL(partials_reduce_jobs_kernel, dim3(ceil_div(cols, 32), 2 + L.nseg), dim3(256), 0, s, J, grid, cols, accumulate);
+  OP_LAUNCH_CHECK();
+  return OP_OK;
+}
+
 }
 
 extern "C" {
@@ -680,6 +831,27 @@
                                                     (int)cols, accumulate, s, x_rows);
   op_set_error("layernorm_bwd: bad dtype %d", dtype);
   return OP_EINVAL;
+}
+
+int op_layernorm_bwd_link(const void* dy, const void* x, const void* w, const float* mean, const float* rstd, const void* add, void* dx,
+                          void* dw, void* db, void* workspace, int64_t rows, int64_t cols, int accumulate, void* u, int64_t n_seg,
+                          const int64_t* seg_end, const int64_t* seg_rps, const float* const* rowscale, float* const* g0, void* stream) {
+  OP_CHECK_ARG(dy && x && dx && mean && rstd && u && workspace && seg_end && seg_rps && rowscale && g0, "layernorm_bwd_link: null pointer");
+  OP_CHECK_ARG(rows > 0 && cols > 0 && cols % 8 == 0, "layernorm_bwd_link: cols=%lld must be a positive multiple of 8", (long long)cols);
+  if (cols > 2048) { op_set_error("layernorm_bwd_link: cols %lld > 2048 unsupported", (long long)cols); return OP_ENOTSUP; }
+  OP_CHECK_ARG(n_seg >= 1 && n_seg <= LN_LINK_SEGS, "layernorm_bwd_link: n_seg=%lld", (long long)n_seg);
+  LnLink L = {};
+  L.u = (bf16_t*)u;
+  L.nseg = (int)n_seg;
+  for (int i = 0; i < (int)n_seg; ++i) {
+    OP_CHECK_ARG(seg_end[i] > (i ? seg_end[i - 1] : 0) && seg_rps[i] > 0 && seg_rps[i] <= 0x7fffffff && g0[i], "layernorm_bwd_link: segment %d", i);
+    L.end[i] = seg_end[i];
+    L.rps[i] = (int)seg_rps[i];
+    L.rs[i] = rowscale[i];
+  }
+  OP_CHECK_ARG(seg_end[n_seg - 1] == rows, "layernorm_bwd_link: the segments must cover the %lld rows", (long long)rows);
+  return ln_bwd_link_dispatch((const bf16_t*)dy, (const bf16_t*)x, (const bf16_t*)w, mean, rstd, (const bf16_t*)add, (bf16_t*)dx, (bf16_t*)dw,
+                              (bf16_t*)db, (float*)workspace, rows, (int)cols, accumulate, L, g0, (hipStream_t)stream);
 }
 
 int op_ln_geglu_fwd(const void* h0, const void* h1, int64_t ldh, const void* w, const void* b, void* y, float* mean, float* rstd,
diff --git a/one-peace_amd/hip.py b/one-peace_amd/hip.py
--- a/one-peace_amd/hip.py
+++ b/one-peace_amd/hip.py
@@ -26,6 +26,7 @@
     "op_layernorm_bwd_workspace_bytes": (I64, [I64, I64]),
     "op_attn_bwd_dbias_slabs": (I64, [I64, I64, I64, I64]),
     "op_layernorm_bwd": (c_int, [P, P, P, P, P, P, P, P, P, P, P, I64, I64, c_int, c_int, c_int, P, P]),
+    "op_layernorm_bwd_link": (c_int, [P, P, P, P, P, P, P, P, P, P, I64, I64, c_int, P, I64, P, P, P, P, P]),
     "op_gemm_plan": (c_int, [c_int64, c_int64, c_int64, c_int, c_int, c_int64, I64, P]),
     "op_gemm_nt": (c_int, [P, I64, P, P, P, I64, I64, P, P, P, P, I64, P, P, P, I64, P, P, I64, P, I64, I64, I64,
                            c_int, P, I64, I64, P, I64, P]),
@@ -47,6 +48,7 @@
     "op_resid_bwd_workspace_bytes": (I64, [I64]),
     "op_resid_bwd": (c_int, [P, P, P, P, I64, P, P, P, P, P, I64, I64, c_int, P, P]),
     "op_gamma_grad_finish": (c_int, [P, I64, P, P, P, P, P, P, P, I64, c_int, P]),
+    "op_gamma_grad_finish_bias": (c_int, [P, I64, P, P, P, P, P, P, P, I64, c_int, P, P, P, P, P]),
     "op_ln_geglu_bwd": (c_int, [P, P, P, P, P, P, P, P, I64, I64, P, P, P, I64, I64, c_int, P]),
     "op_ln_geglu_fwd": (c_int, [P, P, I64, P, P, P, P, P, I64, I64, c_float, P]),
     "op_colsum": (c_int, [P, P, P, I64, P, P, P, I64, I64, c_int, c_int, P]),
@@ -314,6 +316,30 @@
     return dx, dw, db
 
 
+LN_LINK_MAX_COLS, LN_LINK_MAX_SEGS = 2048, 4
+
+
+def layernorm_bwd_link(dy, x, w, mean, rstd, segs, need_wgrad=True, dw=None, db=None, accumulate=False, add=None):
+    rows, cols = x.shape
+    assert x.dtype == torch.bfloat16 and cols <= LN_LINK_MAX_COLS and 1 <= len(segs) <= LN_LINK_MAX_SEGS and segs[-1][0] == rows
+    dx, u = torch.empty_like(x), torch.empty_like(x)
+    if need_wgrad and w is not None:
+        if dw is None:
+            dw, db, accumulate = torch.empty_like(w), torch.empty_like(w), False
+    else:
+        dw = db = None
+    ws = workspace(lib().op_layernorm_bwd_workspace_bytes(rows, cols), x.device, "ln")
+    n = len(segs)
+    g0 = torch.empty(n, cols, dtype=torch.float32, device=x.device)
+    for _, _, rs in segs:
+        assert rs is None or (rs.dtype == torch.float32 and rs.is_contiguous())
+    ends, rps = (c_int64 * n)(*[int(e) for e, _, _ in segs]), (c_int64 * n)(*[int(r) for _, r, _ in segs])
+    _check(lib().op_layernorm_bwd_link(ptr(dy), ptr(x), ptr(w), ptr(mean), ptr(rstd), ptr(add), ptr(dx), ptr(dw), ptr(db), ptr(ws), rows,
+                                       cols, int(accumulate), ptr(u), n, ends, rps, _ptr_array([rs for _, _, rs in segs], n),
+                                       _ptr_array([g0[i] for i in range(n)], n), stream()), "op_layernorm_bwd_link")
+    return dx, dw, db, u, [g0[i] for i in range(n)]
+
+
 SPLITK_WS_BYTES = 768 << 20
 GEMM_ALGO_BYTES = [0, 0]
 
@@ -597,12 +623,18 @@
     return out, dgamma, dbias
 
 
-def gamma_grad_finish(rowdot, pairs, dgamma, accumulate):
+def gamma_grad_finish(rowdot, pairs, dgamma, accumulate, gamma=None, dbias=None):
     assert rowdot.dtype == torch.float32 and rowdot.dim() == 2 and rowdot.is_contiguous() and len(pairs) <= 3 and dgamma.dtype == torch.bfloat16
     assert rowdot.shape[1] == dgamma.numel()
     flat = []
     for b, g0 in list(pairs) + [(None, None)] * (3 - len(pairs)):
         flat += [ptr(b), ptr(g0)]
+    if dbias is not None and any(d is not None for d in dbias):
+        assert len(dbias) == len(pairs) and all(d is None or (d.dtype == torch.bfloat16 and d.is_contiguous()) for d in dbias)
+        dbs = [ptr(d) for d in list(dbias) + [None] * (3 - len(dbias))]
+        _check(lib().op_gamma_grad_finish_bias(ptr(rowdot), rowdot.shape[0], *flat, ptr(dgamma), rowdot.shape[1], int(accumulate), ptr(gamma),
+                                               *dbs, stream()), "op_gamma_grad_finish_bias")
+        return dgamma
     _check(lib().op_gamma_grad_finish(ptr(rowdot), rowdot.shape[0], *flat, ptr(dgamma), rowdot.shape[1], int(accumulate), stream()),
            "op_gamma_grad_finish")
     return dgamma
diff --git a/one-peace_amd/ops.py b/one-peace_amd/ops.py
--- a/one-peace_amd/ops.py
+++ b/one-peace_amd/ops.py
@@ -725,6 +725,60 @@
     return out
 
 
+FUSED_BOOKKEEPING = os.environ.get("ONEPEACE_FUSED_BOOKKEEPING", "1") != "0"
+
+
+class BranchLink:
+    __slots__ = ("segs", "cols", "dx", "version", "u", "g0", "__weakref__")
+
+    def __init__(self, segs, cols):
+        self.segs, self.cols = segs, cols
+        self.dx = self.u = self.g0 = None
+        self.version = -1
+
+    def fill(self, dx, u, g0):
+        self.dx, self.u, self.g0, self.version = dx, u, g0, dx._version
+
+    def take(self, dout):
+        dx, u, g0, version = self.dx, self.u, self.g0, self.version
+        self.dx = self.u = self.g0 = None
+        if u is None or dout.data_ptr() != dx.data_ptr() or dout.shape != dx.shape or not dout.is_contiguous() or dx._version != version:
+            return None
+        return u, g0
+
+
+_open_links = {}
+
+
+def link_segments(segs, pss, rows):
+    out, at = [], 0
+    for sg, ps in zip(segs, pss):
+        if sg.row0 != at or sg.pad or (ps is not None and (ps.dtype != torch.float32 or not ps.is_contiguous())):
+            return None
+        at = sg.end
+        out.append((at, sg.S, ps))
+    return out if at == rows and 1 <= len(out) <= hip.LN_LINK_MAX_SEGS else None
+
+
+def offer_link(out, segs):
+    if len(_open_links) >= 16:
+        _open_links.clear()
+    link = BranchLink(segs, out.shape[1])
+    _open_links[id(out)] = (weakref.ref(out), link)
+    return link
+
+
+def find_link(x2):
+    hit = _open_links.pop(id(x2), None)
+    if hit is None or hit[0]() is not x2 or x2.dtype != torch.bfloat16 or x2.dim() != 2 or x2.shape[1] != hit[1].cols or not x2.is_contiguous():
+        return None
+    return hit[1]
+
+
+def _linkable(H):
+    return FUSED_BOOKKEEPING and H % 8 == 0 and H <= hip.LN_LINK_MAX_COLS
+
+
 def _resid_backward(dout, y, gamma, ps, S, gname, bname, direct, G, needs, g0=None, rows=None, fold=None):
     names = tuple(n for n, present in ((gname, gamma is not None and g0 is None), (bname, True)) if present and needs.get(n))
     tgt, acc = _targets(direct, *names) if names else ([], False)
@@ -770,9 +824,16 @@
     return weight_grad, direct
 
 
-def _gamma_finish_hook(rowdot, gamma_param, pairs, done):
+def _gamma_finish_hook(rowdot, gamma_param, pairs, done, bias_params=None):
     def run():
-        hip.gamma_grad_finish(rowdot, pairs, gamma_param.grad, True)
+        if bias_params is not None and any(q is not None for q in bias_params):
+            hip.gamma_grad_finish(rowdot, pairs, gamma_param.grad, True, gamma=gamma_param.detach(),
+                                  dbias=[q.grad if q is not None else None for q in bias_params])
+            for q in bias_params:
+                if q is not None:
+                    _direct_grad_done(q)
+        else:
+            hip.gamma_grad_finish(rowdot, pairs, gamma_param.grad, True)
         if done:
             _direct_grad_done(gamma_param)
     return run
@@ -806,6 +867,7 @@
         first_param = 7 + nseg
         needs = dict(zip(ATTN_PARAMS, ctx.needs_input_grad[first_param:]))
         x_full = x2
+        ctx.link_out = find_link(x2) if need_grad and keep and kept is None and _linkable(x2.shape[1]) else None
         mapped = _row_tables(kept)
         if kept is not None and not mapped:
             x2 = hip.rows_gather(x_full, kept)
@@ -838,6 +900,9 @@
             if P["aln_w"] is not None:
                 acts["aln"] = None
         _save(ctx, keep, acts, x2, rowscale, *params)
+        ctx.link_in = None
+        if ctx.dg_fused and keep and kept is None and _linkable(H) and (rowscale is None or (rowscale.dtype == torch.float32 and rowscale.is_contiguous())):
+            ctx.link_in = offer_link(x_mid, [(N, rps, rowscale)])
         return x_mid
 
     @staticmethod
@@ -871,11 +936,18 @@
         G = {}
         weight_grad, direct = _weight_grad_fn(ctx, G)
         if ctx.dg_fused:
-            g0 = torch.empty(H, dtype=torch.float32, device=dx_mid.device)
-            dy1 = _resid_backward(dx_mid, None, P["g1"], rowscale, rps, "g1", "bo", direct, G, needs, g0=g0, rows=xmap)
+            linked = ctx.link_in.take(dx_mid) if ctx.link_in is not None else None
+            bias_params = None
+            if linked is not None:
+                dy1, (g0,) = linked
+                if P["bo"] is not None:
+                    bias_params = [direct["bo"] if needs["bo"] else None]
+            else:
+                g0 = torch.empty(H, dtype=torch.float32, device=dx_mid.device)
+                dy1 = _resid_backward(dx_mid, None, P["g1"], rowscale, rps, "g1", "bo", direct, G, needs, g0=g0, rows=xmap)
             rowdot, (rd_wo,) = _rowdot_slots(dx_mid.device, [P["wo"]])
             weight_grad("wo", dy1, A["aln"], side=(P["wo"], rd_wo, P["g1"]),
-                        after=_gamma_finish_hook(rowdot, direct["g1"], [(P["bo"], g0)] if P["bo"] is not None else [], True))
+                        after=_gamma_finish_hook(rowdot, direct["g1"], [(P["bo"], g0)] if P["bo"] is not None else [], True, bias_params))
             wo_t = _transposed(P["wo"], scale=P["g1"])
         else:
             dy1 = _resid_backward(dx_mid, A["y1"], P["g1"], rowscale, rps, "g1", "bo", direct, G, needs, rows=xmap)
@@ -938,9 +1010,14 @@
                 dxln1 = hip.gemm_nt(dqkv, [_transposed(tuple(P[n] for n in cols))])
                 want = needs["ln1_w"] or needs["ln1_b"]
                 (tw, tb), acc = _targets(direct, "ln1_w", "ln1_b") if want else ((None, None), False)
-                dx, dw_, db_ = hip.layernorm_bwd(dxln1, x2, P["ln1_w"], P["ln1_b"], A["mean1"], A["rstd1"], add=dx_mid, dw=tw, db=tb,
-                                                 accumulate=acc, need_wgrad=want, dx=torch.empty_like(dx_full) if mapped else None,
-                                                 x_rows=xmap)
+                if ctx.link_out is not None and need_x:
+                    dx, dw_, db_, u, g0s = hip.layernorm_bwd_link(dxln1, x2, P["ln1_w"], A["mean1"], A["rstd1"], ctx.link_out.segs, add=dx_mid,
+                                                                  dw=tw, db=tb, accumulate=acc, need_wgrad=want)
+                    ctx.link_out.fill(dx, u, g0s)
+                else:
+                    dx, dw_, db_ = hip.layernorm_bwd(dxln1, x2, P["ln1_w"], P["ln1_b"], A["mean1"], A["rstd1"], add=dx_mid, dw=tw, db=tb,
+                                                     accumulate=acc, need_wgrad=want, dx=torch.empty_like(dx_full) if mapped else None,
+                                                     x_rows=xmap)
                 if want:
                     _finish(direct, G, ("ln1_w", "ln1_b"), (dw_, db_), acc)
         if dx is None and need_x:
@@ -1056,6 +1133,7 @@
         needs = ctx.needs_input_grad[5:]
         has_fln = params[5] is not None
         x_full = x2
+        ctx.link_out = find_link(x2) if need_grad and keep and kept is None and _linkable(x2.shape[1]) else None
         mapped = _row_tables(kept)
         if kept is not None and not mapped:
             x2 = hip.rows_gather(x_full, kept)
@@ -1090,6 +1168,11 @@
                 acts["gln"] = None
         _save(ctx, keep, acts or {}, x2, *[ps for ps in pss], *params)
         ctx.n_ps = len(pss)
+        ctx.link_in = None
+        if ctx.dg_fused and keep and kept is None and nseg <= 3 and _linkable(H):
+            lsegs = link_segments(segs, pss, N)
+            if lsegs is not None:
+                ctx.link_in = offer_link(out, lsegs)
         return out
 
     @staticmethod
@@ -1135,19 +1218,26 @@
         fused = ctx.dg_fused
         fp8b = FP8_FFN and FP8_FFN_DGRAD and H % 128 == 0 and Fd % 128 == 0
         (rowdot, rd_views), pairs = (_rowdot_slots(dev, [P["w2@%d" % i] for i in range(nseg)]), []) if fused else ((None, None), None)
+        linked = ctx.link_in.take(dout) if fused and ctx.link_in is not None else None
+        bias_params = [] if linked is not None else None
         for i, sg in enumerate(segs):
             r = slice(sg.row0, sg.end)
             k = lambda n: "%s@%d" % (n, i)
             g0 = None
             if fused:
-                g0 = torch.empty(H, dtype=torch.float32, device=dev)
+                g0 = linked[1][i] if linked is not None else torch.empty(H, dtype=torch.float32, device=dev)
                 if P[k("b2")] is not None:
                     pairs.append((P[k("b2")], g0))
-            dy2 = _resid_backward(dout_full if mapped else dout[r], A["y2"][r] if A["y2"] is not None else None, P["g2"], pss[i], sg.S,
-                                  "g2", k("b2"), direct, G, needs, g0=g0, rows=xmap[r] if mapped else None, fold=fold)
+                    if linked is not None:
+                        bias_params.append(direct[k("b2")] if needs[k("b2")] else None)
+            if linked is not None:
+                dy2 = linked[0][r]
+            else:
+                dy2 = _resid_backward(dout_full if mapped else dout[r], A["y2"][r] if A["y2"] is not None else None, P["g2"], pss[i], sg.S,
+                                      "g2", k("b2"), direct, G, needs, g0=g0, rows=xmap[r] if mapped else None, fold=fold)
             if fused:
                 weight_grad(k("w2"), dy2, A["gln"][r], side=(P[k("w2")], rd_views[i], P["g2"]),
-                            after=_gamma_finish_hook(rowdot, direct["g2"], pairs, True) if i == nseg - 1 else None)
+                            after=_gamma_finish_hook(rowdot, direct["g2"], pairs, True, bias_params) if i == nseg - 1 else None)
             elif needs[k("w2")]:
                 weight_grad(k("w2"), dy2, A["gln"][r])
             if not upstream:
@@ -1198,8 +1288,13 @@
                     hip.gemm_nt(dh[r], [wt], out=dxln2[r])
             want = needs["ln2_w"] or needs["ln2_b"]
             (tw, tb), acc = _targets(direct, "ln2_w", "ln2_b") if want else ((None, None), False)
-            dx, dw_, db_ = hip.layernorm_bwd(dxln2, x2, P["ln2_w"], P["ln2_b"], A["mean2"], A["rstd2"], add=dout, dw=tw, db=tb,
-                                             accumulate=acc, need_wgrad=want, dx=torch.empty_like(dout_full) if mapped else None, x_rows=xmap)
+            if ctx.link_out is not None and need_x:
+                dx, dw_, db_, u, g0s = hip.layernorm_bwd_link(dxln2, x2, P["ln2_w"], A["mean2"], A["rstd2"], ctx.link_out.segs, add=dout, dw=tw,
+                                                              db=tb, accumulate=acc, need_wgrad=want)
+                ctx.link_out.fill(dx, u, g0s)
+            else:
+                dx, dw_, db_ = hip.layernorm_bwd(dxln2, x2, P["ln2_w"], P["ln2_b"], A["mean2"], A["rstd2"], add=dout, dw=tw, db=tb,
+                                                 accumulate=acc, need_wgrad=want, dx=torch.empty_like(dout_full) if mapped else None, x_rows=xmap)
             if want:
                 _finish(direct, G, ("ln2_w", "ln2_b"), (dw_, db_), acc)
         if dx is None and need_x:
```
